# ymartin101/RTS

Hardware: AMD Instinct MI355X
Metric: Mrays/s (primary+bounces) & ms/pulse, 100k-tri scene (higher is better)
Workload: dtype f64

## Files before the change

### include/rts_amd.h

```cpp
#ifndef RTS_AMD_H
#define RTS_AMD_H

#include <stdint.h>
#include "rts_prd.h"

#ifdef __cplusplus
extern "C" {
#endif

typedef struct RtsContext* RtsHandle;

enum {
    RTS_OK = 0,
    RTS_ERR_INVALID = 1,
    RTS_ERR_NO_DEVICE = 2,
    RTS_ERR_HIP = 3,
    RTS_ERR_UNSUPPORTED = 4,
    RTS_ERR_CAPACITY = 5,
    RTS_ERR_IO = 6
};

typedef struct RtsParams {
    uint32_t width;
    uint32_t max_refl;
    uint32_t max_refr;
    uint32_t interpolate_smooth;
    int32_t device;
    uint32_t flags;
} RtsParams;

#define RTS_FLAG_KEEP_ALL_RAYS 1u
#define RTS_FLAG_DEVICE_BUILD 4u
#define RTS_FLAG_HOST_BUILD 16u
#define RTS_FLAG_NO_PREFILTER 8u
#define RTS_FLAG_COUNT_TRAVERSAL 2u

typedef struct RtsMesh {
    const uint32_t* triangles;
    const double* vertices;
    const double* normals;
    uint32_t n_triangles, n_vertices, n_normals;
    uint32_t reserved;
    double refl_coeff;
    double refr_index;
} RtsMesh;

typedef struct RtsTargetMotion {
    double position[3];
    double velocity[3];
    double rotation[9];
    int32_t has_rotation;
    int32_t reserved;
} RtsTargetMotion;

typedef struct RtsReceiverSphere {
    double centre[3];
    double radius;
    double min_theta, max_theta, min_phi, max_phi;
} RtsReceiverSphere;

typedef struct RtsPulse {
    double ray_origin[3];
    double tx_span[3];
    double tx_dir[2];
    uint64_t ray_first;
    uint64_t ray_count;
    const RtsTargetMotion* motion;
    uint32_t interleave_tile, interleave_parts, interleave_part, reserved;
} RtsPulse;
#define RTS_INTERLEAVE_LIST 0xffffffffu

typedef struct RtsStats {
    uint64_t rays;
    uint64_t segments;
    uint64_t shaded;
    uint64_t received;
    uint64_t node_visits;
    uint64_t tri_tests;
    uint32_t n_prims, n_nodes;
    float ms_scene;
    float ms_trace;
    float ms_compact;
    float ms_aggregate;
    uint32_t bvh_rebuilt;
    uint32_t stack_overflows;
    uint64_t walked_segments;
    uint32_t coop_tiles;
    uint32_t cost_records_dropped;
} RtsStats;

typedef struct RtsResponse {
    uint64_t ray;
    int32_t rx;
    uint32_t n;
    double power, delay, doppler, phase;
} RtsResponse;

#define RTS_MAX_DEPTH 16
typedef struct RtsGroup {
    int32_t rx;
    uint32_t direct;
    int32_t path[RTS_MAX_DEPTH];
    uint64_t min_ray;
    double n, sum_sqrt_power, sum_delay, sum_phase, sum_doppler;
} RtsGroup;

int rts_create(const RtsParams* params, RtsHandle* out);
int rts_destroy(RtsHandle h);
const char* rts_last_error(void);
const char* rts_build_id(void);
int rts_bind_host_to_device(int device, int* numa_node);
int rts_device_count(int* n);

int rts_set_scene(RtsHandle h, const RtsMesh* meshes, uint32_t n_targets);
int rts_set_receivers(RtsHandle h, const RtsReceiverSphere* rx, uint32_t n_rx);
int rts_share_scene(RtsHandle dst, RtsHandle src);
typedef struct RtsSceneInfo {
    uint32_t n_targets, n_prims, n_nodes, n_leaves;
    uint32_t handles_sharing;
    uint32_t builder;
    double build_ms;
    uint64_t shared_device_bytes;
    uint64_t handle_device_bytes;
    uint64_t version_bytes;
} RtsSceneInfo;
int rts_scene_info(RtsHandle h, RtsSceneInfo* out);

int rts_trace_pulse(RtsHandle h, const RtsPulse* pulse);

int rts_reserve(RtsHandle h, uint64_t n_rays);
int rts_trace_pulse_begin(RtsHandle h, const RtsPulse* pulse);
int rts_trace_pulse_end(RtsHandle h);
int rts_link_handles(RtsHandle a, RtsHandle b);
int rts_get_stats(RtsHandle h, RtsStats* out);
int rts_get_block_timeline(RtsHandle h, double* out, uint32_t n);

int rts_get_lane_stats(RtsHandle h, uint64_t* out3);
int rts_get_walk_stats(RtsHandle h, uint64_t* out, uint32_t n);
int rts_received_count(RtsHandle h, uint64_t* count);
int rts_get_received(RtsHandle h, struct PerRayData* rays, int32_t* paths, double* rcs_angles, uint64_t* slots,
                     uint64_t capacity);

int rts_received_prefetch(RtsHandle h);
int rts_received_view(RtsHandle h, const struct PerRayData** rays, const int32_t** paths, const double** rcs_angles, const uint64_t** slots,
                      uint64_t* count);
int rts_finalise_values(RtsHandle h, const double* power, const double* doppler, uint64_t count);
int rts_aggregated_view(RtsHandle h, const double** power, const double** doppler, const double** delay, const double** phase,
                        const int32_t** path_match, uint64_t* count);

int rts_get_all_rays(RtsHandle h, struct PerRayData* results, int32_t* targ_intersect, double* rcs_angle,
                     int32_t* hit_prim, float* hit_t, uint64_t capacity);

int rts_finalise_uniform(RtsHandle h, const double* rcs_per_target, double wavelength, double gt, double gr,
                         double carrier, double cspeed);

int rts_trace_pulse_end_uniform(RtsHandle h, const double* rcs_per_target, double wavelength, double gt, double gr,
                                double carrier, double cspeed, int32_t cube_pulse, uint64_t recv_index_base);

#define RTS_PATTERN_CONSTANT 0u
#define RTS_PATTERN_SEPARABLE 1u
#define RTS_PATTERN_GRID 2u
#define RTS_PATTERN_ABS_U 1u
#define RTS_PATTERN_ABS_V 2u
#define RTS_PATTERN_MAX_AXIS 65536u
#define RTS_PATTERN_MAX_GRID 4194304u
typedef struct RtsPattern {
    uint32_t kind;
    uint32_t flags;
    uint32_t n_u, n_v;
    double scale;
    const double* u_samples;
    const double* u_values;
    const double* v_samples;
    const double* v_values;
    double u0, du, v0, dv;
    const double* grid;
    uint64_t reserved[2];
} RtsPattern;
typedef struct RtsPatternPulse {
// ... 429 lines not shown
```

### rts_amd/_lib.py

```python
import ctypes as C
import os
import subprocess

import numpy as np

_HERE = os.path.dirname(os.path.abspath(__file__))
LIB_PATH = os.environ.get("RTS_AMD_LIB", os.path.join(_HERE, "librts_amd.so"))
CSRC = os.path.join(_HERE, "csrc")

RTS_OK, RTS_ERR_INVALID, RTS_ERR_NO_DEVICE, RTS_ERR_HIP, RTS_ERR_UNSUPPORTED, RTS_ERR_CAPACITY, RTS_ERR_IO = range(7)
RTS_FLAG_KEEP_ALL_RAYS = 1
RTS_FLAG_COUNT_TRAVERSAL = 2
RTS_FLAG_DEVICE_BUILD = 4
RTS_FLAG_HOST_BUILD = 16
RTS_FLAG_NO_PREFILTER = 8
RTS_MAX_DEPTH = 16
RTS_BASE_USE_ROWS = 0xffffffffffffffff

PRD_DTYPE = np.dtype({
    "names": ["rayLength", "refrIndex", "reflDepth", "refrDepth", "maxRayIndex", "rayDirection",
              "firstHitPoint", "prevHitPoint", "power", "doppler", "received", "end"],
    "formats": ["<f8", ("<f8", 2), "<u4", "<u4", "<u4", ("<f8", 3), ("<f8", 3), ("<f8", 3), "<f8", "<f8", "<i4", "u1"],
    "offsets": [0, 16, 32, 36, 40, 48, 72, 96, 120, 128, 136, 140],
    "itemsize": 144,
})


class RtsParams(C.Structure):
    _fields_ = [("width", C.c_uint32), ("max_refl", C.c_uint32), ("max_refr", C.c_uint32),
                ("interpolate_smooth", C.c_uint32), ("device", C.c_int32), ("flags", C.c_uint32)]


class RtsMesh(C.Structure):
    _fields_ = [("triangles", C.c_void_p), ("vertices", C.c_void_p), ("normals", C.c_void_p),
                ("n_triangles", C.c_uint32), ("n_vertices", C.c_uint32), ("n_normals", C.c_uint32),
                ("reserved", C.c_uint32), ("refl_coeff", C.c_double), ("refr_index", C.c_double)]


class RtsTargetMotion(C.Structure):
    _fields_ = [("position", C.c_double * 3), ("velocity", C.c_double * 3), ("rotation", C.c_double * 9),
                ("has_rotation", C.c_int32), ("reserved", C.c_int32)]


class RtsReceiverSphere(C.Structure):
    _fields_ = [("centre", C.c_double * 3), ("radius", C.c_double), ("min_theta", C.c_double),
                ("max_theta", C.c_double), ("min_phi", C.c_double), ("max_phi", C.c_double)]


class RtsPulse(C.Structure):
    _fields_ = [("ray_origin", C.c_double * 3), ("tx_span", C.c_double * 3), ("tx_dir", C.c_double * 2),
                ("ray_first", C.c_uint64), ("ray_count", C.c_uint64), ("motion", C.POINTER(RtsTargetMotion)),
                ("interleave_tile", C.c_uint32), ("interleave_parts", C.c_uint32), ("interleave_part", C.c_uint32), ("reserved", C.c_uint32)]


class RtsCubeParams(C.Structure):
    _fields_ = [("n_rx", C.c_uint32), ("n_pulses", C.c_uint32), ("n_bins", C.c_uint32), ("reserved", C.c_uint32),
                ("t0", C.c_double), ("dt", C.c_double)]


class RtsPlanItem(C.Structure):
    _fields_ = [("pulse", C.c_uint32), ("interleave_tile", C.c_uint32), ("interleave_parts", C.c_uint32), ("interleave_part", C.c_uint32),
                ("ray_first", C.c_uint64), ("ray_count", C.c_uint64)]


RTS_SHARD_PULSES, RTS_SHARD_RAYS, RTS_SHARD_PULSES_WHOLE = 0, 1, 2


RTS_PATTERN_CONSTANT, RTS_PATTERN_SEPARABLE, RTS_PATTERN_GRID = 0, 1, 2
# ... 168 lines not shown
class RtsCovParams(C.Structure):
    _fields_ = [("source", C.c_uint32), ("n_rows_in", C.c_uint32), ("first_row", C.c_uint32), ("n_rows", C.c_uint32),
                ("first_bin", C.c_uint32), ("n_bins", C.c_uint32), ("skip_first_bin", C.c_uint32), ("skip_n_bins", C.c_uint32),
                ("device_in", C.c_void_p), ("reserved", C.c_uint64 * 2)]


class RtsMvdrParams(C.Structure):
    _fields_ = [("n_beams", C.c_uint32), ("n_rx", C.c_uint32), ("loading", C.c_double), ("steering", C.c_void_p),
                ("device_cov", C.c_void_p), ("reserved", C.c_uint64 * 2)]


assert C.sizeof(RtsCovParams) == 56 and C.sizeof(RtsMvdrParams) == 48


RTS_ST_MAX_TAPS = 16


class RtsStCovParams(C.Structure):
    _fields_ = [("source", C.c_uint32), ("n_rows_in", C.c_uint32), ("first_row", C.c_uint32), ("n_rows", C.c_uint32),
                ("first_bin", C.c_uint32), ("n_bins", C.c_uint32), ("skip_first_bin", C.c_uint32), ("skip_n_bins", C.c_uint32),
                ("n_taps", C.c_uint32), ("reserved0", C.c_uint32), ("device_in", C.c_void_p), ("reserved", C.c_uint64 * 2)]


class RtsStApplyParams(C.Structure):
    _fields_ = [("n_filters", C.c_uint32), ("source", C.c_uint32), ("first_row", C.c_uint32), ("n_rows", C.c_uint32),
                ("n_rows_in", C.c_uint32), ("flags", C.c_uint32), ("n_taps", C.c_uint32), ("reserved0", C.c_uint32),
                ("weights", C.c_void_p), ("device_in", C.c_void_p), ("reserved", C.c_uint64 * 2)]


assert C.sizeof(RtsStCovParams) == 64 and C.sizeof(RtsStApplyParams) == 64


RTS_EIG_MAX_SWEEPS = 30
RTS_DOA_INVERSE = 1
RTS_DOA_BARTLETT, RTS_DOA_CAPON, RTS_DOA_MUSIC = 0, 1, 2
RTS_DOA_AIC, RTS_DOA_MDL = 0, 1


class RtsEigParams(C.Structure):
    _fields_ = [("n", C.c_uint32), ("reserved0", C.c_uint32), ("device_cov", C.c_void_p), ("reserved", C.c_uint64 * 2)]


class RtsDoaScanParams(C.Structure):
    _fields_ = [("n", C.c_uint32), ("first_vector", C.c_uint32), ("m", C.c_uint32), ("flags", C.c_uint32), ("n_dirs", C.c_uint64),
                ("g", C.c_void_p), ("device_steering", C.c_void_p), ("device_vectors", C.c_void_p), ("reserved", C.c_uint64 * 2)]


assert C.sizeof(RtsEigParams) == 32 and C.sizeof(RtsDoaScanParams) == 64


class RtsSceneInfo(C.Structure):
    _fields_ = [("n_targets", C.c_uint32), ("n_prims", C.c_uint32), ("n_nodes", C.c_uint32), ("n_leaves", C.c_uint32),
                ("handles_sharing", C.c_uint32), ("builder", C.c_uint32), ("build_ms", C.c_double),
                ("shared_device_bytes", C.c_uint64), ("handle_device_bytes", C.c_uint64), ("version_bytes", C.c_uint64)]


class RtsStats(C.Structure):
    _fields_ = [("rays", C.c_uint64), ("segments", C.c_uint64), ("shaded", C.c_uint64), ("received", C.c_uint64),
                ("node_visits", C.c_uint64), ("tri_tests", C.c_uint64), ("n_prims", C.c_uint32), ("n_nodes", C.c_uint32),
                ("ms_scene", C.c_float), ("ms_trace", C.c_float), ("ms_compact", C.c_float), ("ms_aggregate", C.c_float),
                ("bvh_rebuilt", C.c_uint32), ("stack_overflows", C.c_uint32), ("walked_segments", C.c_uint64), ("coop_tiles", C.c_uint32), ("cost_records_dropped", C.c_uint32)]


RESPONSE_DTYPE = np.dtype([("ray", "<u8"), ("rx", "<i4"), ("n", "<u4"), ("power", "<f8"), ("delay", "<f8"),
                           ("doppler", "<f8"), ("phase", "<f8")])
GROUP_DTYPE = np.dtype([("rx", "<i4"), ("direct", "<u4"), ("path", "<i4", (RTS_MAX_DEPTH,)), ("min_ray", "<u8"),
                        ("n", "<f8"), ("sum_sqrt_power", "<f8"), ("sum_delay", "<f8"), ("sum_phase", "<f8"),
                        ("sum_doppler", "<f8")])
assert RESPONSE_DTYPE.itemsize == 48 and GROUP_DTYPE.itemsize == 120


def is_stale():
    if not os.path.exists(LIB_PATH):
        return True
    try:
        return build_id() != source_hash()
    except (OSError, AttributeError):
        return True


def source_hash():
    import hashlib
    names = sorted(f for f in os.listdir(CSRC) if f.endswith((".hip", ".cpp", ".h")) and f != "rts_build_id.h")
    h = hashlib.sha256()
    for path in [os.path.join(CSRC, f) for f in names] + [os.path.join(_HERE, "..", "include", f) for f in ("rts_amd.h", "rts_prd.h")]:
        with open(path, "rb") as f:
            h.update(f.read())
    return h.hexdigest()[:16]


def build_id(path=None):
    L = C.CDLL(path or LIB_PATH)
    L.rts_build_id.restype = C.c_char_p
    return L.rts_build_id().decode()


def require_built():
    if not os.path.exists(LIB_PATH):
        raise SystemExit("librts_amd.so is not built: run `python __graft_entry__.py` (or make -C rts_amd/csrc) first")
    if "RTS_AMD_LIB" not in os.environ:
        have, want = build_id(), source_hash()
        if have != want:
            raise SystemExit("librts_amd.so is stale: built from sources %s, the tree is %s -- run `python __graft_entry__.py` first" % (have, want))


def build(force=False, verbose=False):
    if force or is_stale():
        cmd = ["make", "-C", CSRC, "-j", "5"] + ([] if verbose else ["-s"])
        subprocess.check_call(cmd)
    return LIB_PATH


_lib = None

EXPORTS = ["rts_create", "rts_destroy", "rts_last_error", "rts_device_count", "rts_set_scene", "rts_share_scene", "rts_scene_info", "rts_set_receivers",
           "rts_trace_pulse", "rts_reserve", "rts_trace_pulse_begin", "rts_trace_pulse_end", "rts_link_handles", "rts_get_stats", "rts_get_block_timeline", "rts_received_count", "rts_get_received", "rts_get_all_rays",
           "rts_finalise_uniform", "rts_trace_pulse_end_uniform", "rts_aggregate", "rts_group_count", "rts_get_groups", "rts_get_aggregated",
           "rts_merge_groups", "rts_groups_to_responses", "rts_kernel_wrapper", "rts_vertex_rotation",
           "rts_rotation_matrix", "rts_rect_mesh", "rts_sphere_mesh", "rts_file_mesh", "rts_rx_sphere", "rts_get_bvh",
           "rts_build_id", "rts_bind_host_to_device", "rts_get_lane_stats", "rts_get_walk_stats", "rts_self_test_math", "rts_cube_attach", "rts_cube_accumulate", "rts_cube_get", "rts_cube_accumulate_paths", "rts_cube_doppler", "rts_cube_doppler_get", "rts_plan_cpi", "rts_cube_reduce", "rts_kernel_wrapper_on",
           "rts_received_prefetch", "rts_received_view", "rts_finalise_values", "rts_aggregated_view", "rts_build_hierarchy_host",
           "rts_tile_records_get", "rts_tile_records_set", "rts_deal_tiles", "rts_set_tile_list",
           "rts_set_patterns", "rts_finalise_patterns", "rts_trace_pulse_end_patterns", "rts_pattern_eval",
           "rts_cube_set_waveform", "rts_cube_render", "rts_cube_compress", "rts_waveform_eval",
           "rts_cube_add_noise", "rts_noise_eval", "rts_cube_detect", "rts_cube_detections_get",
           "rts_cube_detect_os", "rts_cfar_os_alpha", "rts_cfar_os_eval",
           "rts_cube_plots", "rts_cube_plots_get", "rts_plots_eval",
           "rts_cube_track", "rts_cube_tracks_get", "rts_cube_tracks_set", "rts_cube_tracks_reset", "rts_cube_track_rounds", "rts_tracks_eval",
           "rts_cube_tbd_step", "rts_cube_tbd_extract", "rts_cube_tbd_tracks_get", "rts_cube_tbd_paths_get", "rts_cube_tbd_merit_get", "rts_cube_tbd_ring_get",
           "rts_cube_tbd_info", "rts_cube_tbd_reset", "rts_tbd_step_eval", "rts_tbd_extract_eval",
           "rts_cube_backproject", "rts_cube_image_get", "rts_backproject_eval",
           "rts_cube_spectrogram", "rts_cube_spectrogram_get", "rts_stft_eval", "rts_window_make",
           "rts_cube_render_beat", "rts_beat_eval", "rts_cube_range_transform", "rts_cube_range_get", "rts_range_eval",
           "rts_cube_beamform", "rts_cube_beam_get", "rts_beamform_eval", "rts_steering_make",
           "rts_cube_covariance", "rts_cube_covariance_get", "rts_covariance_eval", "rts_cube_mvdr", "rts_cube_mvdr_get", "rts_mvdr_eval",
           "rts_cube_st_covariance", "rts_st_covariance_eval", "rts_cube_st_apply", "rts_cube_st_get", "rts_st_apply_eval", "rts_st_steering_make",
           "rts_cube_eig", "rts_cube_eig_get", "rts_eig_eval", "rts_cube_doa_scan", "rts_cube_doa_get", "rts_doa_scan_eval", "rts_doa_weights", "rts_source_count"]


def lib():
    global _lib
    if _lib is not None:
        return _lib
    if not os.path.exists(LIB_PATH):
        raise RuntimeError("librts_amd.so is not built (run `make -C rts_amd/csrc` or __graft_entry__.build()); "
                           "there is no Python/CPU fallback for the RTS hot path")
    L = C.CDLL(LIB_PATH)
    vp, u32, u64, dbl, i32 = C.c_void_p, C.c_uint32, C.c_uint64, C.c_double, C.c_int32
    L.rts_last_error.restype = C.c_char_p
    sig = {
        "rts_create": [C.POINTER(RtsParams), C.POINTER(vp)],
        "rts_destroy": [vp],
        "rts_device_count": [C.POINTER(C.c_int)],
        "rts_set_scene": [vp, C.POINTER(RtsMesh), u32],
        "rts_share_scene": [vp, vp],
        "rts_scene_info": [vp, C.POINTER(RtsSceneInfo)],
        "rts_set_receivers": [vp, C.POINTER(RtsReceiverSphere), u32],
        "rts_trace_pulse": [vp, C.POINTER(RtsPulse)],
        "rts_reserve": [vp, u64],
        "rts_trace_pulse_begin": [vp, C.POINTER(RtsPulse)],
        "rts_get_block_timeline": [vp, vp, u32],
        "rts_trace_pulse_end": [vp],
        "rts_link_handles": [vp, vp],
        "rts_get_stats": [vp, C.POINTER(RtsStats)],
        "rts_received_count": [vp, C.POINTER(u64)],
        "rts_get_received": [vp, vp, vp, vp, vp, u64],
        "rts_get_all_rays": [vp, vp, vp, vp, vp, vp, u64],
        "rts_finalise_uniform": [vp, vp, dbl, dbl, dbl, dbl, dbl],
        "rts_build_hierarchy_host": [vp, vp, u32, dbl, vp, u32, vp, u32, C.POINTER(u32), C.POINTER(u32), C.POINTER(C.c_int32)],
        "rts_received_prefetch": [vp],
        "rts_received_view": [vp, C.POINTER(vp), C.POINTER(vp), C.POINTER(vp), C.POINTER(vp), C.POINTER(u64)],
        "rts_finalise_values": [vp, vp, vp, u64],
        "rts_aggregated_view": [vp, C.POINTER(vp), C.POINTER(vp), C.POINTER(vp), C.POINTER(vp), C.POINTER(vp), C.POINTER(u64)],
        "rts_aggregate": [vp, dbl, dbl, u64],
        "rts_trace_pulse_end_uniform": [vp, vp, dbl, dbl, dbl, dbl, dbl, C.c_int32, u64],
        "rts_group_count": [vp, C.POINTER(u32)],
        "rts_get_groups": [vp, vp, u32],
        "rts_get_aggregated": [vp, vp, vp, vp, vp, u64],
        "rts_merge_groups": [vp, u32, u32, vp, C.POINTER(u32)],
        "rts_groups_to_responses": [vp, u32, vp, u32, C.POINTER(u32)],
        "rts_kernel_wrapper": [vp, vp, C.c_uint, C.c_uint, C.c_uint, C.c_uint, dbl, dbl, vp, vp, vp, vp, vp, vp],
        "rts_kernel_wrapper_on": [vp, vp, vp, C.c_uint, C.c_uint, C.c_uint, C.c_uint, dbl, dbl, vp, vp, vp, vp, vp, vp],
        "rts_vertex_rotation": [vp, u32, C.c_float, C.c_float, C.c_float],
        "rts_rotation_matrix": [C.c_float, C.c_float, C.c_float, vp],
        "rts_rect_mesh": [C.c_float] * 6 + [vp, vp, vp],
        "rts_sphere_mesh": [u32, C.c_float, C.c_float, C.c_float, C.c_float, vp, C.POINTER(u32), vp, C.POINTER(u32), vp],
        "rts_file_mesh": [C.c_char_p, C.c_char_p, C.c_float, C.c_float, C.c_float, vp, vp, vp, C.POINTER(u32)],
        "rts_rx_sphere": [vp, dbl, dbl, dbl, dbl, dbl, C.POINTER(RtsReceiverSphere)],
        "rts_get_bvh": [vp, vp, vp, vp, u32, u32, vp],
        "rts_cube_attach": [vp, C.POINTER(RtsCubeParams), vp],
        "rts_cube_accumulate": [vp, u32, dbl, dbl],
        "rts_cube_get": [vp, vp, u64], "rts_get_lane_stats": [vp, vp], "rts_get_walk_stats": [vp, vp, C.c_uint32], "rts_bind_host_to_device": [C.c_int, C.POINTER(C.c_int)],
        "rts_cube_accumulate_paths": [vp, u32], "rts_cube_doppler": [vp, u32, vp], "rts_cube_doppler_get": [vp, vp, u64],
        "rts_plan_cpi": [u64, u32, u32, u32, u32, u32, u32, vp, u32, C.POINTER(u32)],
        "rts_cube_reduce": [vp, u32, C.c_int],
        "rts_tile_records_get": [vp, vp, u32], "rts_tile_records_set": [vp, vp, u32], "rts_deal_tiles": [vp, u32, u64, u32, u32, vp, vp], "rts_set_tile_list": [vp, u32, vp, u32],
        "rts_self_test_math": [vp, vp, vp, vp, vp, vp, vp, vp, u32],
        "rts_set_patterns": [vp, C.POINTER(RtsPattern), C.POINTER(RtsPattern), u32, C.POINTER(RtsPattern), u32],
        "rts_finalise_patterns": [vp, C.POINTER(RtsPatternPulse)],
        "rts_trace_pulse_end_patterns": [vp, C.POINTER(RtsPatternPulse), C.c_int32, u64],
        "rts_pattern_eval": [C.POINTER(RtsPattern), vp, vp, u32, vp],
        "rts_cube_set_waveform": [vp, C.POINTER(RtsWaveform)],
        "rts_cube_render": [vp, u32, u32, u32, C.c_double, C.c_double],
        "rts_cube_compress": [vp, u32, u32],
        "rts_waveform_eval": [C.POINTER(RtsWaveform), vp, u32, vp],
        "rts_cube_add_noise": [vp, u32, u32, C.c_double, u64],
        "rts_noise_eval": [u64, vp, u32, C.c_double, vp],
        "rts_cube_detect": [vp, C.POINTER(RtsCfarParams), vp, u32],
        "rts_cube_detections_get": [vp, vp, u32, C.POINTER(u32)],
        "rts_cube_detect_os": [vp, C.POINTER(RtsCfarOsParams), vp, u32],
        "rts_cfar_os_alpha": [u32, u32, C.c_double, C.POINTER(C.c_double)],
        "rts_cfar_os_eval": [C.POINTER(RtsCubeParams), vp, u32, C.POINTER(RtsCfarOsParams), vp, u32, C.POINTER(u32)],
        "rts_cube_plots": [vp, C.POINTER(RtsPlotParams)],
        "rts_cube_plots_get": [vp, vp, u32, C.POINTER(u32)],
        "rts_plots_eval": [C.POINTER(RtsCubeParams), vp, u32, u32, C.POINTER(RtsPlotParams), vp, u32, C.POINTER(u32)],
        "rts_cube_track": [vp, C.POINTER(RtsTrackParams), C.c_double],
        "rts_cube_tracks_get": [vp, vp, u32, C.POINTER(u32), C.POINTER(u64)],
        "rts_cube_tracks_set": [vp, vp, u32, u64, C.c_double],
        "rts_cube_tracks_reset": [vp],
        "rts_cube_track_rounds": [vp, C.POINTER(u32)],
        "rts_tracks_eval": [C.POINTER(RtsTrackParams), vp, u32, u64, C.c_double, vp, u32, vp, u32, C.POINTER(u32), C.POINTER(u64)],
        "rts_cube_tbd_step": [vp, C.POINTER(RtsTbdParams), C.c_double, vp, u32],
        "rts_cube_tbd_extract": [vp, C.POINTER(RtsTbdExtractParams)],
        "rts_cube_tbd_tracks_get": [vp, vp, u32, C.POINTER(u32)],
        "rts_cube_tbd_paths_get": [vp, vp, u32],
        "rts_cube_tbd_merit_get": [vp, vp, u64],
        "rts_cube_tbd_ring_get": [vp, vp, vp, u32, C.POINTER(u32)],
        "rts_cube_tbd_info": [vp, C.POINTER(u32 * 4), C.POINTER(u64)],
        "rts_cube_tbd_reset": [vp],
        "rts_tbd_step_eval": [C.POINTER(RtsCubeParams), vp, u32, vp, C.POINTER(RtsTbdParams), C.c_double, vp, vp, vp],
        "rts_tbd_extract_eval": [C.POINTER(RtsCubeParams), u32, C.POINTER(RtsTbdParams), vp, vp, vp, u32, C.POINTER(RtsTbdExtractParams), vp, vp, u32, C.POINTER(u32)],
        "rts_cube_backproject": [vp, C.POINTER(RtsImageParams), vp],
        "rts_cube_image_get": [vp, vp, u64],
        "rts_backproject_eval": [C.POINTER(RtsCubeParams), vp, C.POINTER(RtsImageParams), vp],
        "rts_cube_spectrogram": [vp, C.POINTER(RtsStftParams), vp, C.POINTER(u32)],
        "rts_cube_spectrogram_get": [vp, vp, u64],
        "rts_stft_eval": [C.POINTER(RtsCubeParams), vp, C.POINTER(RtsStftParams), vp, C.POINTER(u32)],
        "rts_window_make": [u32, u32, vp],
        "rts_cube_render_beat": [vp, u32, C.POINTER(RtsBeatParams), C.c_double, C.c_double],
        "rts_beat_eval": [C.POINTER(RtsCubeParams), C.POINTER(RtsBeatParams), vp, u32, u32, vp],
        "rts_cube_range_transform": [vp, C.POINTER(RtsRangeParams), vp],
        "rts_cube_range_get": [vp, vp, u64],
        "rts_range_eval": [C.POINTER(RtsCubeParams), vp, C.POINTER(RtsRangeParams), vp],
        "rts_cube_beamform": [vp, C.POINTER(RtsBeamParams), vp],
        "rts_cube_beam_get": [vp, vp, u64],
# ... 47 lines not shown
```

### rts_amd/api.py

```python
import ctypes as C

import numpy as np

from . import _lib as L
from ._lib import PRD_DTYPE, RESPONSE_DTYPE, GROUP_DTYPE, check, ptr


def rect_mesh(w, h, d, yaw=0.0, pitch=0.0, roll=0.0):
    v = np.zeros((8, 3)); t = np.zeros((12, 3), np.uint32); n = np.zeros((12, 3))
    check(L.lib().rts_rect_mesh(w, h, d, yaw, pitch, roll, ptr(v), ptr(t), ptr(n)))
    return v, t, n


def sphere_mesh(subdivisions, radius, yaw=0.0, pitch=0.0, roll=0.0):
    nv = C.c_uint32(); nt = C.c_uint32()
    check(L.lib().rts_sphere_mesh(subdivisions, radius, yaw, pitch, roll, None, C.byref(nv), None, C.byref(nt), None))
    v = np.zeros((nv.value, 3)); t = np.zeros((nt.value, 3), np.uint32); n = np.zeros((nv.value, 3))
    check(L.lib().rts_sphere_mesh(subdivisions, radius, yaw, pitch, roll, ptr(v), C.byref(nv), ptr(t), C.byref(nt), ptr(n)))
    return v, t, n


def file_mesh(v_file, n_file, yaw=0.0, pitch=0.0, roll=0.0):
    nt = C.c_uint32(0)
    check(L.lib().rts_file_mesh(v_file.encode(), n_file.encode(), yaw, pitch, roll, None, None, None, C.byref(nt)))
# ... 599 lines not shown
    p = _st_cov_params(taps, "cube", first, count, first_bin, n_bins, skip, None, 0)
    D = n_rx * max(int(taps), 0)
    out = np.zeros((D, D), np.complex128)
    check(L.lib().rts_st_covariance_eval(C.byref(q), ptr(inp.view(np.float64)), rows, C.byref(p), ptr(out.view(np.float64))))
    return out


def _st_apply_params(weights, taps, n_rx, source, first, count, power, device_in, n_rows_in):
    w = np.ascontiguousarray(np.asarray(weights, np.complex128))
    if w.ndim != 2 or w.shape[1] != int(taps) * n_rx:
        raise ValueError("st_apply: weights of shape %s for %d taps of %d receivers ([n_filters][taps n_rx])" % (w.shape, taps, n_rx))
    p = L.RtsStApplyParams()
    p.n_filters, p.source, p.n_taps = w.shape[0], _BEAM_SOURCES.get(source, source), int(taps)
    p.first_row, p.n_rows, p.n_rows_in = int(first), int(count or 0), int(n_rows_in)
    p.flags = L.RTS_BEAM_POWER if power else 0
    p.weights = ptr(w.view(np.float64))
    p.device_in = device_in if device_in else None
    return p, w


def st_apply_eval(inp, weights, taps, first=0, count=None, power=False):
    inp = np.ascontiguousarray(np.asarray(inp, np.complex128))
    n_rx, rows, nb = inp.shape
    q = L.RtsCubeParams(n_rx, rows, nb, 0, 0.0, 1.0)
    p, keep = _st_apply_params(weights, taps, n_rx, "cube", first, count, power, None, 0)
    out = _beam_out(p.n_filters, (p.n_rows if p.n_rows else rows - p.first_row) - p.n_taps + 1, nb, power, False)
    check(L.lib().rts_st_apply_eval(C.byref(q), ptr(inp.view(np.float64)), rows, C.byref(p), ptr(out.view(np.float64))))
    return out


def st_steering(spatial, dopplers, taps, tap_taper=None):
    a = np.ascontiguousarray(np.atleast_2d(np.asarray(spatial, np.complex128)))
    f = np.ascontiguousarray(np.asarray(dopplers, np.float64).ravel())
    t = None if tap_taper is None else np.ascontiguousarray(np.asarray(tap_taper, np.float64).ravel())
    if t is not None and len(t) != int(taps):
        raise ValueError("st_steering: a taper of %d values for %d taps" % (len(t), taps))
    out = np.zeros((a.shape[0] * len(f), max(int(taps), 0) * a.shape[1]), np.complex128)
    check(L.lib().rts_st_steering_make(ptr(a.view(np.float64)), a.shape[1], a.shape[0], ptr(f), len(f), int(taps), ptr(t), ptr(out.view(np.float64))))
    return out


def device_count():
    n = C.c_int(0)
    rc = L.lib().rts_device_count(C.byref(n))
    return n.value if rc == 0 else 0


import os as _os
_PY_LAP = {} if _os.environ.get("RTS_PY_LAP") == "1" else None


class Tracer:

    def __init__(self, width, max_refl, max_refr=0, smooth=True, device=0, keep_all=False, count_traversal=False, device_build=None, pre_filter=True):
        p = L.RtsParams(width, max_refl, max_refr, 1 if smooth else 0, device,
                        (L.RTS_FLAG_KEEP_ALL_RAYS if keep_all else 0) | (L.RTS_FLAG_COUNT_TRAVERSAL if count_traversal else 0) |
                        (0 if device_build is None else (L.RTS_FLAG_DEVICE_BUILD if device_build else L.RTS_FLAG_HOST_BUILD)) |
                         (0 if pre_filter else L.RTS_FLAG_NO_PREFILTER))
        self.h = C.c_void_p()
        check(L.lib().rts_create(C.byref(p), C.byref(self.h)))
        self.width = width; self.max_refl = max_refl; self.depth = max_refl + (2 if max_refr else 0)
        self.n_targets = 0; self.keep_all = keep_all; self.device = device
        self._keep = []

    def close(self):
        if self.h:
            L.lib().rts_destroy(self.h); self.h = C.c_void_p()

    def __del__(self):
        try:
            self.close()
        except Exception:
            pass

    def set_scene(self, meshes):
        arr = (L.RtsMesh * max(len(meshes), 1))()
        keep = []
        for i, m in enumerate(meshes):
            t = np.ascontiguousarray(m["tris"], np.uint32); v = np.ascontiguousarray(m["verts"], np.float64)
            n = np.ascontiguousarray(m["normals"], np.float64)
            keep += [t, v, n]
            arr[i] = L.RtsMesh(t.ctypes.data, v.ctypes.data, n.ctypes.data, t.shape[0], v.shape[0], n.shape[0], 0,
                               float(m.get("refl_coeff", 1.0)), float(m.get("refr_index", 1.0)))
        check(L.lib().rts_set_scene(self.h, arr, len(meshes)))
        self.n_targets = len(meshes)

    def share_scene(self, other):
        check(L.lib().rts_share_scene(self.h, other.h))
        self.n_targets = other.n_targets

    def scene_info(self):
        s = L.RtsSceneInfo()
        check(L.lib().rts_scene_info(self.h, C.byref(s)))
        return {k: getattr(s, k) for k, _ in L.RtsSceneInfo._fields_}

    def set_receivers(self, spheres):
        arr = (L.RtsReceiverSphere * max(len(spheres), 1))()
        for i, s in enumerate(spheres):
            arr[i] = L.RtsReceiverSphere((C.c_double * 3)(*s["centre"]), s["radius"], s["minTheta"], s["maxTheta"],
                                         s["minPhi"], s["maxPhi"])
        check(L.lib().rts_set_receivers(self.h, arr, len(spheres)))

    def trace(self, origin, tx_span, tx_dir, motion=None, ray_first=0, ray_count=0, want_stats=True, interleave=None):
        check(L.lib().rts_trace_pulse(self.h, C.byref(self._pulse(origin, tx_span, tx_dir, motion, ray_first, ray_count, interleave))))
        return self.stats() if want_stats else None

    def reserve(self, n_rays=0):
        check(L.lib().rts_reserve(self.h, n_rays))

    def trace_begin(self, origin, tx_span, tx_dir, motion=None, ray_first=0, ray_count=0, interleave=None):
        if _PY_LAP is None:
            check(L.lib().rts_trace_pulse_begin(self.h, C.byref(self._pulse(origin, tx_span, tx_dir, motion, ray_first, ray_count, interleave))))
            return
        import time
        t0 = time.perf_counter(); p = self._pulse(origin, tx_span, tx_dir, motion, ray_first, ray_count, interleave)
        t1 = time.perf_counter(); f = L.lib().rts_trace_pulse_begin
        t2 = time.perf_counter(); rc = f(self.h, C.byref(p))
        t3 = time.perf_counter(); check(rc)
        t4 = time.perf_counter()
        for k, v in zip(("marshal", "lookup", "call", "check"), (t1 - t0, t2 - t1, t3 - t2, t4 - t3)):
            _PY_LAP[k] = _PY_LAP.get(k, 0.0) + v
        _PY_LAP["n"] = _PY_LAP.get("n", 0) + 1

    def block_timeline(self):
        out = np.zeros(9, np.float64)
        check(L.lib().rts_get_block_timeline(self.h, ptr(out), 9))
        return dict(zip(("start_first", "start_p50", "start_last", "end_first", "end_p10", "end_p50", "end_p90", "end_last", "blocks"), out.tolist()))

    def trace_end(self):
        check(L.lib().rts_trace_pulse_end(self.h))

    def tile_records_get(self):
        n = (self.width ** 3 + 63) // 64
        out = np.zeros(n, np.uint32)
        check(L.lib().rts_tile_records_get(self.h, ptr(out), n))
        return out

    def tile_records_set(self, records):
# ... 493 lines not shown
```

### rts_amd/csrc/rts_api.hip

```cpp
#include <cmath>
#include <cstdarg>
#include <cstdio>
#include <cstring>
#include <cstdlib>
#include <dlfcn.h>
#include <algorithm>
#include <chrono>
#include <map>
#include <mutex>
#include <stdexcept>
#include <string>
#include "rts_internal.h"
#include "rts_raygen.h"
#include <atomic>

static thread_local char g_err[1024] = "";
void rts_set_error(const char* fmt, ...) { va_list ap; va_start(ap, fmt); vsnprintf(g_err, sizeof(g_err), fmt, ap); va_end(ap); }
extern "C" const char* rts_last_error(void) { return g_err; }
#include "rts_build_id.h"
extern "C" const char* rts_build_id(void) { return RTS_SOURCE_HASH; }

#include <dirent.h>
#include <sched.h>
extern "C" int rts_bind_host_to_device(int device, int* numa_node)
// ... 240 lines not shown
    for (int i = 0; i < 3; i++) for (int j = 0; j < 3; j++) a.rot1[3*i + j] = Rot1[i][j];
}

static void fill_mask_frame(RtsLaunchConsts& a, bool enable)
{
    RtsMaskFrame& f = a.mask; memset(&f, 0, sizeof(f));
    if (!enable || a.W < 2) return;
    dvec3 c[8]; dvec3 sum = mk3(0, 0, 0);
    for (int k = 0; k < 8; k++) {
        c[k] = rts_lattice_dir(a, (k & 1) ? a.W - 1 : 0, (k & 2) ? a.W - 1 : 0, (k & 4) ? a.W - 1 : 0);
        const double n = len3(c[k]); if (!(n > 0) || !std::isfinite(n)) return;
        c[k] = mk3(c[k].x / n, c[k].y / n, c[k].z / n); sum = add3(sum, c[k]);
    }
    const double sn = len3(sum); if (!(sn > 1e-6)) return;
    const dvec3 b = mk3(sum.x / sn, sum.y / sn, sum.z / sn);
    dvec3 ref = std::fabs(b.z) < 0.9 ? mk3(0, 0, 1) : mk3(1, 0, 0);
    dvec3 u = cross3(ref, b); const double un = len3(u); u = mk3(u.x / un, u.y / un, u.z / un);
    const dvec3 v = cross3(b, u);
    double u0 = 1e300, u1 = -1e300, v0 = 1e300, v1 = -1e300;
    for (int k = 0; k < 8; k++) {
        const double w = dot3(c[k], b); if (!(w > 0.5)) return;
        const double uu = dot3(c[k], u) / w, vv = dot3(c[k], v) / w;
        u0 = std::min(u0, uu); u1 = std::max(u1, uu); v0 = std::min(v0, vv); v1 = std::max(v1, vv);
    }
    const double du = std::max(u1 - u0, 1e-9), dv = std::max(v1 - v0, 1e-9);
    u0 -= 0.002 * du; u1 += 0.002 * du; v0 -= 0.002 * dv; v1 += 0.002 * dv;
    f.bx = (float)b.x; f.by = (float)b.y; f.bz = (float)b.z; f.ux = (float)u.x; f.uy = (float)u.y; f.uz = (float)u.z; f.vx = (float)v.x; f.vy = (float)v.y; f.vz = (float)v.z;
    const double n_fit = std::floor(std::min(u1 - u0, v1 - v0) / RTS_MASK_MIN_CELL);
    if (!(n_fit >= 32.0)) return;
    const uint32_t n = (uint32_t)std::min<double>(RTS_MASK_N, n_fit) & ~31u;
    f.u0 = (float)u0; f.v0 = (float)v0; f.inv_du = (float)(n / (u1 - u0)); f.inv_dv = (float)(n / (v1 - v0));
    f.n = n;
}

static int fill_target_placement(const RtsContext* c, uint32_t t, RtsTargetDev& td)
{
    const RtsTargetMotion& m = c->motion[t]; const RtsBlasInfo& b = c->scene->blas[t];
    double R[9] = {1, 0, 0, 0, 1, 0, 0, 0, 1};
    if (m.has_rotation) for (int k = 0; k < 9; k++) R[k] = m.rotation[k];
    for (int k = 0; k < 9; k++) if (!std::isfinite(R[k])) { rts_set_error("rts_trace_pulse: target %u has a non-finite rotation", t); return RTS_ERR_INVALID; }
    double dev = 0;
    for (int i = 0; i < 3; i++) for (int j = 0; j < 3; j++) {
        double g = 0; for (int k = 0; k < 3; k++) g += R[3*k + i] * R[3*k + j];
        dev = std::max(dev, std::fabs(g - (i == j ? 1.0 : 0.0)));
    }
    if (!(dev < 1e-3)) { rts_set_error("rts_trace_pulse: target %u: rotation is not orthonormal (|R^T R - I| = %.3g); only rigid placements are supported", t, dev); return RTS_ERR_UNSUPPORTED; }
    const double det = R[0]*(R[4]*R[8] - R[5]*R[7]) - R[1]*(R[3]*R[8] - R[5]*R[6]) + R[2]*(R[3]*R[7] - R[4]*R[6]);
    const double id = 1.0 / det;
    td.rinv[0] = (R[4]*R[8] - R[5]*R[7]) * id; td.rinv[1] = (R[2]*R[7] - R[1]*R[8]) * id; td.rinv[2] = (R[1]*R[5] - R[2]*R[4]) * id;
    td.rinv[3] = (R[5]*R[6] - R[3]*R[8]) * id; td.rinv[4] = (R[0]*R[8] - R[2]*R[6]) * id; td.rinv[5] = (R[2]*R[3] - R[0]*R[5]) * id;
    td.rinv[6] = (R[3]*R[7] - R[4]*R[6]) * id; td.rinv[7] = (R[1]*R[6] - R[0]*R[7]) * id; td.rinv[8] = (R[0]*R[4] - R[1]*R[3]) * id;
    td.px = m.position[0]; td.py = m.position[1]; td.pz = m.position[2];
    td.root = b.root;
    double cl[3], half2 = 0, wc[3], wmax = 0;
    for (int i = 0; i < 3; i++) { cl[i] = 0.5 * b.lo[i] + 0.5 * b.hi[i]; const double h = 0.5 * (b.hi[i] - b.lo[i]); half2 += h * h; }
    for (int i = 0; i < 3; i++) { wc[i] = R[3*i]*cl[0] + R[3*i + 1]*cl[1] + R[3*i + 2]*cl[2] + m.position[i]; wmax = std::max(wmax, std::fabs(wc[i])); }
    double rad = std::sqrt(half2) * (1.0 + 2.0 * dev); wmax += rad;
    rad = rad * (1.0 + 1e-6) + wmax * 1e-6 + 1e-30;
    td.cx = wc[0]; td.cy = wc[1]; td.cz = wc[2]; td.r2 = rad * rad;
    td.ew = (float)(wmax * c->tune.ew_rel) + 1.0e-30f;
    if (b.root < 0 || !std::isfinite(td.cx + td.cy + td.cz + td.r2)) td.root = -1;
    return RTS_OK;
}

static int rts_hist_ensure(RtsContext* c, uint32_t n_hist)
{
    if (c->hist->n == n_hist) return RTS_OK;
    std::lock_guard<std::mutex> lk(g_hist_mu);
    RTS_HIP(hipDeviceSynchronize()); RTS_HIP(c->hist->d.reserve(n_hist)); RTS_HIP(hipMemset(c->hist->d.p, 0, sizeof(uint32_t) * n_hist));
    c->hist->n = n_hist; c->hist->any = false; c->tile_cost_pending = false;
    return RTS_OK;
}

static int rts_zero_block_reserve(RtsContext* c)
{
    RTS_HIP(c->d_tile_ctr.reserve(RTS_ZERO_WORDS + RTS_MASK_WORDS + 64));
    c->p_counters = reinterpret_cast<unsigned long long*>(c->d_tile_ctr.p + RTS_OFF_COUNTERS);
    return RTS_OK;
}

static int rts_launch_buffers_reserve(RtsContext* c, const RtsLaunchSizes& s)
{
    RTS_HIP(c->d_recv.reserve(s.recv)); RTS_HIP(c->d_dir_hist.reserve(s.dir_hist)); RTS_HIP(c->d_child.reserve(s.child));
    RTS_HIP(c->d_stack_ovf.reserve(s.stack_ovf)); RTS_HIP(c->d_block_counters.reserve(s.block_counters));
    RTS_HIP(c->d_all.reserve(s.all)); RTS_HIP(c->d_hit_prim.reserve(s.hit_prim)); RTS_HIP(c->d_hit_t.reserve(s.hit_t));
    return RTS_OK;
}

static uint32_t rts_coop_threads(const RtsContext* c) { return c->tune.coop_frac > 0.0 ? c->tune.coop_grid_max * RTS_BLOCK : 0u; }

extern "C" int rts_reserve(RtsHandle c, uint64_t n_rays)
{
    CHECK_HANDLE(c);
    const uint64_t W3 = rts_lattice_size(c->params.width);
    const uint64_t n = std::min<uint64_t>(n_rays ? n_rays : W3, W3);
    if (n * rts_chains(c->params.max_refr) > 0xfffffff0ULL) { rts_set_error("rts_reserve: rays x chains exceeds 2^32"); return RTS_ERR_UNSUPPORTED; }
    const RtsLaunchSizes sz = rts_launch_sizes(n, (uint64_t)c->n_cu * 64 * RTS_BLOCK, (uint64_t)c->n_cu * 1024, rts_coop_threads(c), (uint64_t)c->n_cu * 64 + c->tune.coop_grid_max,
                                               c->params.max_refl, c->params.max_refr, (c->params.flags & RTS_FLAG_KEEP_ALL_RAYS) != 0);
    { int rc = rts_launch_buffers_reserve(c, sz); if (rc != RTS_OK) return rc; }
    { int rc = rts_zero_block_reserve(c); if (rc != RTS_OK) return rc; }
    const size_t n_tiles = (size_t)rts_wave_tiles(n);
    RTS_HIP(c->d_tile_cost.reserve(n_tiles)); RTS_HIP(c->d_tile_key.reserve(n_tiles)); RTS_HIP(c->d_tile_order.reserve(n_tiles));
    { int rc = rts_hist_ensure(c, (uint32_t)rts_wave_tiles(W3)); if (rc != RTS_OK) return rc; }
    RTS_HIP(hipMemsetAsync(c->d_recv.p, 0, sizeof(RtsEndRecord) * sz.recv, c->stream));
    RTS_HIP(hipMemsetAsync(c->d_dir_hist.p, 0, sizeof(float) * c->d_dir_hist.cap, c->stream));
    RTS_HIP(hipStreamSynchronize(c->stream));
// ... 76 lines not shown
    lc.ray_first = r.first; lc.W = W; lc.il_tile = r.il_tile; lc.il_parts = r.il_parts; lc.il_part = r.il_part; lc.il_list = r.il_list ? c->d_il_list.p : nullptr;
    const RtsDivMagic d = rts_div_magic(W); lc.w_magic = d.magic; lc.w_more = d.more;
    fill_mask_frame(lc, pre_filter && c->scene->n_prims > 0);
    for (int k = 0; k < 3; k++) { lc.f_bs[k] = (float)(&lc.bsx)[k]; lc.f_st[k] = (float)(&lc.stx)[k]; }
    for (int i = 0; i < 3; i++) for (int j = 0; j < 3; j++) lc.f_m[3 * i + j] = (float)(lc.rot1[3 * i] * lc.rot[j] + lc.rot1[3 * i + 1] * lc.rot[3 + j] + lc.rot1[3 * i + 2] * lc.rot[6 + j]);
}

static uint32_t* pulse_mask_words(const RtsContext* c) { return c->d_tile_ctr.p + RTS_ZERO_WORDS; }

static int pulse_upload_and_fill(RtsContext* c, bool moved)
{
    const uint32_t n_targets = (uint32_t)c->scene->meshes.size(); const RtsMaskFrame& mask = c->last_lc.mask;
    c->pin.p->lc = c->last_lc;
    RTS_HIP(hipMemcpyAsync(c->d_params.p, &c->pin.p->lc, moved && n_targets ? offsetof(RtsPinned, td) + sizeof(RtsTargetDev) * n_targets : sizeof(RtsLaunchConsts), hipMemcpyHostToDevice, c->stream));
    { int rc = rts_zero_block_reserve(c); if (rc != RTS_OK) return rc; }
    RTS_HIP(hipMemsetAsync(c->d_tile_ctr.p, 0, sizeof(uint32_t) * (((RTS_ZERO_WORDS + (mask.n ? (size_t)mask.n * mask.n / 32u + 1u : 0u)) + 63u) & ~(size_t)63u), c->stream));
    return RTS_OK;
}

static int pulse_scene_place(RtsContext* c, bool moved)
{
    { int rc = rts_scene_place(c, c->last_lc, moved, pulse_mask_words(c)); if (rc != RTS_OK) return rc; }
    if (moved) { RTS_STAGE(c, "scene_place"); c->bvh_valid = true; c->stats.bvh_rebuilt = 1; }
    RTS_HIP(hipEventRecord(c->ev[1], c->stream));
    return RTS_OK;
}

static int pulse_args_and_buffers(RtsContext* c, RtsPulseLaunch& L)
{
    RtsTraceArgs& a = L.a; memset(&a, 0, sizeof(a));
    const uint32_t n = L.n; const RtsLaunchConsts& lc = c->last_lc; hipStream_t st = c->stream;
    a.lc = c->p_lc;
    a.ray_first = L.r.first; a.n_rays = n; a.W = c->params.width; a.max_refl = c->params.max_refl; a.smooth = c->params.interpolate_smooth ? 1u : 0u;
    a.n_prims = c->scene->n_prims; a.n_targets = (uint32_t)c->scene->meshes.size(); a.n_rx = c->n_rx; a.keep_all = L.keep_all ? 1u : 0u;
    a.max_refr = c->params.max_refr; a.rows = a.max_refr ? c->params.max_refl + 3 : 1;
    if ((uint64_t)n * rts_chains(a.max_refr) > 0xfffffff0ULL) { rts_set_error("rts_trace_pulse: rays x chains exceeds 2^32"); return RTS_ERR_UNSUPPORTED; }
    a.total_threads = L.grid * RTS_BLOCK;
    a.coop_spread = c->tune.coop_spread;
    a.coop_walk_steps_lo = std::min(c->tune.coop_walk_steps_lo, c->tune.coop_walk_steps);
    a.coop_walk_steps = c->tune.coop_walk_steps; a.coop_min_cost = c->tune.coop_walk_steps ? std::min<uint32_t>(c->tune.coop_floor, 1875u) : 0u;
    a.slab_threads = a.total_threads + rts_coop_threads(c);
    const RtsLaunchSizes sz = rts_launch_sizes(n, a.total_threads, a.total_threads, rts_coop_threads(c), (uint64_t)L.grid + c->tune.coop_grid_max, a.max_refl, a.max_refr, L.keep_all);
    { int rc = rts_launch_buffers_reserve(c, sz); if (rc != RTS_OK) return rc; }
    if (L.keep_all) {
        rts_fill_i32(st, c->d_hit_prim.p, -2, sz.hit_prim - 1);
        RTS_HIP(hipMemsetAsync(c->d_hit_t.p, 0, sizeof(float) * (sz.hit_t - 1), st));
    }
    a.pmask = lc.mask.n ? pulse_mask_words(c) : nullptr; a.pre_filter = L.pre_filter ? 1u : 0u;
    a.nodes4 = c->scene->d_nodes4.p; a.nodes4v = c->tune.node_versions ? c->scene->d_nodes4v.p : nullptr; a.stack_lds = c->tune.stack_lds; a.leaves = c->d_leaves.p; a.tri_nidx = c->scene->d_tri_nidx.p; a.normals = c->d_normals_world.p;
    a.targets = c->p_targets; a.rx = c->d_rx.p;
    a.recv_records = c->d_recv.p; a.all_records = c->d_all.p; a.counters = c->p_counters; a.block_counters = c->d_block_counters.p; a.dir_hist = c->d_dir_hist.p;
    a.hit_prim = c->d_hit_prim.p; a.hit_t = c->d_hit_t.p; a.stack_ovf = c->d_stack_ovf.p; a.child = c->d_child.p;
    a.rx_window_screen = c->tune.rx_window_screen ? 1u : 0u;
    a.coop_versions = c->tune.coop_versions ? 1u : 0u;
    a.tile_ctr = c->d_tile_ctr.p;
    return RTS_OK;
}

static int pulse_tile_order(RtsContext* c, RtsPulseLaunch& L)
{
    RtsTraceArgs& a = L.a;
    const RtsLaunchShape s = rts_launch_shape(L.n, L.r.first, L.r.il_tile, L.r.il_parts, L.r.il_part, rts_lattice_size(c->params.width));
    const uint32_t n_tiles = s.n_tiles, resident_waves = L.grid * (RTS_BLOCK / RTS_WTILE);
    a.batch_dead = s.aligned ? (uint32_t)c->tune.batch_dead : 0u;
    if (!(c->tune.tile_lpt && s.aligned && n_tiles > resident_waves)) { c->tile_cost_pending = false; c->tile_last_valid = false; return RTS_OK; }
    { int rc = rts_hist_ensure(c, s.n_hist); if (rc != RTS_OK) return rc; }
    if (c->tile_cost_pending || c->hist->any) {
        c->coop_big_now = (L.r.il_parts > 1 && !L.shared_gpu && c->tune.coop_big_part > c->tune.coop_big) ? c->tune.coop_big_part : c->tune.coop_big;
        int rc = rts_tile_order_build(c, c->tile_cost_sig, c->tile_cost_pending, s.sig, n_tiles, resident_waves); if (rc != RTS_OK) return rc;
        a.tile_order = c->d_tile_order.p; a.tile_head = c->tune.coop_frac > 0.0 ? c->d_tile_ctr.p + RTS_OFF_HEAD + 2 : nullptr; a.tile_head_all = a.tile_head; c->hist->any = true;
        a.tile_live = c->d_tile_ctr.p + RTS_OFF_LIVE;
    }
    const bool merged_all = c->tile_cost_pending && rts_wave_tiles(c->tile_cost_sig[0]) >= n_tiles && c->d_tile_cost.cap >= n_tiles;
    RTS_HIP(c->d_tile_cost.reserve(n_tiles));
    if (!merged_all) RTS_HIP(hipMemsetAsync(c->d_tile_cost.p, 0, sizeof(uint32_t) * n_tiles, c->stream));
    a.tile_cost = c->d_tile_cost.p;
    c->tile_cost_pending = true; memcpy(c->tile_cost_sig, s.sig, sizeof(s.sig)); memcpy(c->tile_last_sig, s.sig, sizeof(s.sig)); c->tile_last_valid = true;
    return RTS_OK;
}

static int pulse_timelines(RtsContext* c, RtsPulseLaunch& L)
{
    const size_t blocks2 = (size_t)L.grid * 2;
    RtsLaunchTuning lt; if (L.count_trav) rts_tuning_read(&lt, rts_env);
    L.tl_path = lt.timeline;
    L.cnt_tl = blocks2 + 2 * (size_t)rts_wave_tiles(L.n);
    c->tl_blocks = 0;
    const size_t words = L.tl_path ? L.cnt_tl + 1 : (!L.count_trav && c->tune.timeline_blocks) ? blocks2 + 1 : 0;
    if (!words) return RTS_OK;
    RTS_HIP(c->d_timeline.reserve(words)); RTS_HIP(hipMemsetAsync(c->d_timeline.p, 0, sizeof(unsigned long long) * words, c->stream)); L.a.timeline = c->d_timeline.p;
    if (!L.tl_path) c->tl_blocks = L.grid;
    return RTS_OK;
}

static int pulse_launch(RtsContext* c, RtsPulseLaunch& L)
{
    RtsTraceArgs& a = L.a; hipStream_t st = c->stream;
    RTS_STAGE(c, "pre-trace");
    c->tstream_now = (c->tune.trace_own_stream && !L.shared_gpu && c->gate->refs.load() == 1) ? st : c->tstream;
    if (c->tstream_now != st) {
        RTS_HIP(hipEventRecord(c->ev[8], st));
        RTS_HIP(hipStreamWaitEvent(c->tstream_now, c->ev[8], 0));
    }
    RTS_HIP(hipEventRecord(c->ev[2], c->tstream_now));
    unsigned coop_grid = 0;
    if (a.tile_head) {
// ... 811 lines not shown
```

### rts_amd/csrc/rts_bvh.hip

```cpp
#include <cstring>
#include <hip/hip_runtime.h>
#include "rts_internal.h"
#include "rts_ray_ops.h"

__device__ __forceinline__ void place_one(const double* __restrict__ local, double* __restrict__ world, const uint32_t* __restrict__ targ_of,
                                          const RtsTargetMotion* __restrict__ motion, uint32_t i, bool add_position)
{
    const RtsTargetMotion m = motion[targ_of[i]];
    double x = local[3*i], y = local[3*i+1], z = local[3*i+2];
    if (m.has_rotation) {
        double rx = 0.0, ry = 0.0, rz = 0.0;
        rx += m.rotation[0] * x; rx += m.rotation[1] * y; rx += m.rotation[2] * z;
        ry += m.rotation[3] * x; ry += m.rotation[4] * y; ry += m.rotation[5] * z;
        rz += m.rotation[6] * x; rz += m.rotation[7] * y; rz += m.rotation[8] * z;
        x = rx; y = ry; z = rz;
    }
    if (add_position) { x += m.position[0]; y += m.position[1]; z += m.position[2]; }
    world[3*i] = x; world[3*i+1] = y; world[3*i+2] = z;
}
__global__ void k_place(const double* __restrict__ v_local, double* __restrict__ v_world, const uint32_t* __restrict__ v_targ, uint32_t n_verts,
                        const double* __restrict__ n_local, double* __restrict__ n_world, const uint32_t* __restrict__ n_targ, uint32_t n_normals,
                        const RtsTargetMotion* __restrict__ motion)
{
    const uint32_t i = blockIdx.x * blockDim.x + threadIdx.x;
// ... 34 lines not shown
    }
    const bool any = iu1 >= iu0 && iv1 >= iv0;
    {
        int b0 = any ? iu0 : 0x7fffffff, b1 = any ? iv0 : 0x7fffffff, b2 = any ? iu1 : -1, b3 = any ? iv1 : -1;
        for (int d = warpSize / 2; d > 0; d >>= 1) {
            b0 = min(b0, __shfl_xor(b0, d)); b1 = min(b1, __shfl_xor(b1, d)); b2 = max(b2, __shfl_xor(b2, d)); b3 = max(b3, __shfl_xor(b3, d));
        }
        if ((threadIdx.x & (warpSize - 1)) == 0 && b2 >= 0) { atomicMin(&S.box[0], b0); atomicMin(&S.box[1], b1); atomicMax(&S.box[2], b2); atomicMax(&S.box[3], b3); }
    }
    __syncthreads();
    if (S.box[2] < 0) return;
    const int W0 = S.box[0] >> 5, V0 = S.box[1], TW = (S.box[2] >> 5) - W0 + 1, TH = S.box[3] - V0 + 1;
    const int band = RTS_MASK_TILE_WORDS / TW;
    for (int b0 = 0; b0 < TH; b0 += band) {
        const int B0 = V0 + b0, bh = min(band, TH - b0), nw = TW * bh;
        if (b0) __syncthreads();
        for (int w = threadIdx.x; w < nw; w += blockDim.x) S.tile[w] = 0u;
        __syncthreads();
        if (any) {
            for (int iv = max(iv0, B0); iv <= min(iv1, B0 + bh - 1); iv++) {
                for (int w0 = iu0 >> 5; w0 <= (iu1 >> 5); w0++) {
                    const int lo = max(iu0, w0 << 5) & 31, hi = min(iu1, (w0 << 5) + 31) & 31;
                    const uint32_t bits = (hi == 31 ? 0xffffffffu : ((1u << (hi + 1)) - 1u)) & ~((1u << lo) - 1u);
                    atomicOr(&S.tile[(iv - B0) * TW + (w0 - W0)], bits);
                }
            }
        }
        __syncthreads();
        for (int w = threadIdx.x; w < nw; w += blockDim.x) {
            const uint32_t bits = S.tile[w];
            if (bits) atomicOr(&mask[((size_t)(B0 + w / TW) * f.n >> 5) + (size_t)(W0 + w % TW)], bits);
        }
    }
}

__device__ __forceinline__ void place_vertex(const double* __restrict__ local, const RtsTargetMotion& m, uint32_t i, double* __restrict__ out3)
{
    double x = local[3*(size_t)i], y = local[3*(size_t)i+1], z = local[3*(size_t)i+2];
    if (m.has_rotation) {
        double rx = 0.0, ry = 0.0, rz = 0.0;
        rx += m.rotation[0] * x; rx += m.rotation[1] * y; rx += m.rotation[2] * z;
        ry += m.rotation[3] * x; ry += m.rotation[4] * y; ry += m.rotation[5] * z;
        rz += m.rotation[6] * x; rz += m.rotation[7] * y; rz += m.rotation[8] * z;
        x = rx; y = ry; z = rz;
    }
    x += m.position[0]; y += m.position[1]; z += m.position[2];
    out3[0] = x; out3[1] = y; out3[2] = z;
}
template <bool LEAVES, bool MASK, bool PLACE = false>
__global__ void __launch_bounds__(256) k_leaves(const uint32_t* __restrict__ order, const uint32_t* __restrict__ tri_vidx, const double* __restrict__ verts,
                                                const uint32_t* __restrict__ prim_targ, RtsLeafTri* __restrict__ leaves, uint32_t n,
                                                double ox, double oy, double oz, RtsMaskFrame f, uint32_t* __restrict__ mask,
                                                const RtsTargetMotion* __restrict__ motion = nullptr, uint32_t prim_blocks = 0, const double* __restrict__ n_local = nullptr,
                                                double* __restrict__ n_world = nullptr, const uint32_t* __restrict__ n_targ = nullptr, uint32_t n_normals = 0)
{
    __shared__ __attribute__((aligned(16))) uint32_t s_raw[MASK ? sizeof(RtsMaskLds) / 4 : 1];
    if (PLACE && blockIdx.x >= prim_blocks) {
        const uint32_t q = (blockIdx.x - prim_blocks) * blockDim.x + threadIdx.x;
        if (q < n_normals) place_one(n_local, n_world, n_targ, motion, q, false);
        return;
    }
    const uint32_t i = blockIdx.x * blockDim.x + threadIdx.x;
    double p[9] = {0, 0, 0, 0, 0, 0, 0, 0, 0};
    if (i < n) {
        const uint32_t g = order[i];
        const uint32_t a = tri_vidx[3*(size_t)g], b = tri_vidx[3*(size_t)g+1], c = tri_vidx[3*(size_t)g+2];
        if (PLACE) {
            const RtsTargetMotion m = motion[prim_targ[g]];
            place_vertex(verts, m, a, p); place_vertex(verts, m, b, p + 3); place_vertex(verts, m, c, p + 6);
        } else {
        p[0] = verts[3*(size_t)a]; p[1] = verts[3*(size_t)a+1]; p[2] = verts[3*(size_t)a+2];
        p[3] = verts[3*(size_t)b]; p[4] = verts[3*(size_t)b+1]; p[5] = verts[3*(size_t)b+2];
        p[6] = verts[3*(size_t)c]; p[7] = verts[3*(size_t)c+1]; p[8] = verts[3*(size_t)c+2];
        }
        if (LEAVES) {
            dvec3 e0, e1, nn;
            tri_terms(mk3(p[0], p[1], p[2]), mk3(p[3], p[4], p[5]), mk3(p[6], p[7], p[8]), e0, e1, nn);
            RtsLeafTri L;
            L.p0x = p[0]; L.p0y = p[1]; L.p0z = p[2]; L.e0x = e0.x; L.e0y = e0.y; L.e0z = e0.z; L.e1x = e1.x; L.e1y = e1.y; L.e1z = e1.z;
            L.nx = nn.x; L.ny = nn.y; L.nz = nn.z;
            L.prim = g; L.targ = prim_targ[g]; L.pad[0] = 0u; L.pad[1] = 0u;
            leaves[g] = L;
        }
    }
    if (MASK) rts_mask_mark(*reinterpret_cast<RtsMaskLds*>(s_raw), i < n, p, ox, oy, oz, f, mask);
}

static inline unsigned blocks_for(size_t n, unsigned bs) { return (unsigned)((n + bs - 1) / bs); }

int rts_scene_place(RtsContext* c, const RtsLaunchConsts& lc, bool place, uint32_t* pmask)
{
    hipStream_t st = c->stream;
    const RtsMaskFrame& f = lc.mask;
    const bool mask = f.n != 0;
    const RtsScene* sc = c->scene;
    if (place && sc->n_prims) {
        const unsigned gp = blocks_for(sc->n_prims, 256), gn = blocks_for(sc->n_normals, 256);
        if (mask) k_leaves<true, true, true><<<gp + gn, 256, 0, st>>>(sc->d_prim_order.p, sc->d_tri_vidx.p, sc->d_verts_local.p, sc->d_prim_targ.p, c->d_leaves.p, sc->n_prims, lc.ox, lc.oy, lc.oz, f, pmask,
                                                                     c->p_motion, gp, sc->d_normals_local.p, c->d_normals_world.p, sc->d_norm_targ.p, sc->n_normals);
        else k_leaves<true, false, true><<<gp + gn, 256, 0, st>>>(sc->d_prim_order.p, sc->d_tri_vidx.p, sc->d_verts_local.p, sc->d_prim_targ.p, c->d_leaves.p, sc->n_prims, lc.ox, lc.oy, lc.oz, f, nullptr,
                                                                  c->p_motion, gp, sc->d_normals_local.p, c->d_normals_world.p, sc->d_norm_targ.p, sc->n_normals);
        c->verts_world_valid = false;
        RTS_HIP(hipGetLastError());
        return RTS_OK;
    }
    if (place) {
        if (sc->n_verts + sc->n_normals) k_place<<<blocks_for((size_t)sc->n_verts + sc->n_normals, 256), 256, 0, st>>>(sc->d_verts_local.p, c->d_verts_world.p, sc->d_vert_targ.p, sc->n_verts,
                                                                                                                         sc->d_normals_local.p, c->d_normals_world.p, sc->d_norm_targ.p, sc->n_normals, c->p_motion);
        c->verts_world_valid = true;
    } else if (mask) {
        if (!c->verts_world_valid && sc->n_verts) {
            k_place<<<blocks_for((size_t)sc->n_verts, 256), 256, 0, st>>>(sc->d_verts_local.p, c->d_verts_world.p, sc->d_vert_targ.p, sc->n_verts, sc->d_normals_local.p, c->d_normals_world.p, sc->d_norm_targ.p, 0u, c->p_motion);
            c->verts_world_valid = true;
        }
        if (sc->n_prims) k_leaves<false, true><<<blocks_for(sc->n_prims, 256), 256, 0, st>>>(sc->d_prim_order.p, sc->d_tri_vidx.p, c->d_verts_world.p, sc->d_prim_targ.p, nullptr, sc->n_prims, lc.ox, lc.oy, lc.oz, f, pmask);
    }
    RTS_HIP(hipGetLastError());
    return RTS_OK;
}
```

### rts_amd/csrc/rts_internal.h

```cpp
#pragma once
#include <hip/hip_runtime.h>
#include <stdint.h>
#include <stddef.h>
#include <atomic>
#include <string>
#include <vector>
#include "../../include/rts_amd.h"
#include "rts_device_math.h"
#include "rts_pattern.h"
#include "rts_waveform.h"
#include "rts_noise.h"
#include "rts_image.h"
#include "rts_cube_source.h"
#include "rts_stft.h"
#include "rts_beat.h"
#include "rts_beam.h"
#include "rts_adapt.h"
#include "rts_stap.h"
#include "rts_doa.h"
#include "rts_cfar_os.h"
#include "rts_track.h"
#include "rts_tbd.h"
#include "rts_plot.h"
#include "rts_owned.h"
#include "rts_launch_plan.h"
#include "rts_post_plan.h"
#include "rts_pulse_state.h"
#include "rts_scene_host.h"
#include "rts_tuning.h"
static_assert(RtsTuning().img_split_below == RTS_IMAGE_SPLIT_BELOW, "the default of RTS_IMAGE_SPLIT_BELOW is rts_image.h's");


struct __attribute__((aligned(16))) RtsLeafTri {
    double p0x, p0y, p0z, e0x, e0y, e0z, e1x, e1y, e1z, nx, ny, nz;
    uint32_t prim;
    uint32_t targ;
    uint32_t pad[2];
};
static_assert(sizeof(RtsLeafTri) == 112, "leaf size");
static_assert(offsetof(RtsLeafTri, p0x) == 0 && offsetof(RtsLeafTri, p0z) == 16 && offsetof(RtsLeafTri, e0y) == 32 && offsetof(RtsLeafTri, e1x) == 48 &&
              offsetof(RtsLeafTri, e1z) == 64 && offsetof(RtsLeafTri, ny) == 80 && offsetof(RtsLeafTri, prim) == 96 && offsetof(RtsLeafTri, targ) == 100,
              "leaf record offsets of the walk step's decode");

struct RtsTargetDev {
    double reflCoeff;
    double refrIndex;
    double vx, vy, vz;
    uint32_t tri_base;
    uint32_t perface_normals;
    double rinv[9];
    double px, py, pz;
    double cx, cy, cz, r2;
    float ew;
    int32_t root;
};

struct RtsRxDev { double cx, cy, cz, radius, minTheta, maxTheta, minPhi, maxPhi; };

struct __attribute__((aligned(16))) RtsEndRecord {
    double rayLength, power, doppler;
    double prevx, prevy, prevz;
    double firstx, firsty, firstz;
    uint64_t path_lo, path_hi;
    uint32_t slot;
    int32_t received;
    uint32_t reflDepth;
    uint32_t pad;
};
static_assert(sizeof(RtsEndRecord) == 112, "end record size");
static_assert(sizeof(RtsDetection) == 72 && sizeof(RtsCfarParams) == 72 && sizeof(RtsCfarOsParams) == 72, "CFAR ABI sizes (rts_amd/_lib.py mirrors them)");
static_assert(sizeof(RtsPlot) == 104 && sizeof(RtsPlotParams) == 56, "plot ABI sizes (rts_amd/_lib.py mirrors them)");
static_assert(sizeof(RtsTrack) == 88 && sizeof(RtsTrackParams) == 96, "track ABI sizes (rts_amd/_lib.py mirrors them)");
static_assert(sizeof(RtsTbdParams) == 72 && sizeof(RtsTbdExtractParams) == 40 && sizeof(RtsTbdTrack) == 48, "track-before-detect ABI sizes (rts_amd/_lib.py mirrors them)");
struct RtsTrackMeta { uint64_t next_id; uint32_t n, total, rounds, reserved; };

struct __attribute__((aligned(16))) RtsChildState {
    double prevx, prevy, prevz, firstx, firsty, firstz;
    double rayLength, power, doppler, refx, refy;
    float dx, dy, dz;
    uint32_t refrDepth, refr_code, end, pad0, pad1;
};
static_assert(sizeof(RtsChildState) == 128, "child state size");

#ifndef RTS_TILE_CTRS
#define RTS_TILE_CTRS 64
#endif
#define RTS_TILE_BUCKETS 1024
#define RTS_TILE_CTR_STRIDE 32
#define RTS_XCD 8
#define RTS_SEG_STRIPES 8
#define RTS_TILE_CTRS_LAYOUT ((RTS_XCD + 1) * RTS_SEG_STRIPES + 8)
#define RTS_OFF_CTR_COOP (RTS_TILE_CTRS_LAYOUT * RTS_TILE_CTR_STRIDE)
#define RTS_OFF_HEAD (2 * RTS_TILE_CTRS_LAYOUT * RTS_TILE_CTR_STRIDE)
#define RTS_OFF_LIVE (RTS_OFF_HEAD + 4)
#define RTS_OFF_COUNTERS (RTS_OFF_HEAD + 8)
#define RTS_OFF_BINS (RTS_OFF_COUNTERS + 32)
#define RTS_OFF_TAKEN (RTS_OFF_BINS + RTS_TILE_BUCKETS)
#define RTS_ZERO_WORDS (RTS_OFF_TAKEN + RTS_TILE_BUCKETS)
#ifndef RTS_RX_LDS
#define RTS_RX_LDS 16
#endif

#define RTS_MASK_MIN_CELL 1.0e-5
#define RTS_MASK_N 1024u
#define RTS_MASK_WORDS (RTS_MASK_N * RTS_MASK_N / 32u + 1u)
#define RTS_MASK_MAX_CELLS 4096
struct RtsMaskFrame { float bx, by, bz, ux, uy, uz, vx, vy, vz; float u0, v0, inv_du, inv_dv; uint32_t n, pad0, pad1; };

struct RtsLaunchConsts {
    double ox, oy, oz;
    double bsx, bsy, bsz;
    double stx, sty, stz;
    double rot[9];
    double rot1[9];
    double w1x, w1y, w1z;
    uint64_t ray_first;
    uint32_t W, pad;
    uint32_t w_magic, w_more;
    uint32_t il_tile, il_parts, il_part, pad2;
    const uint32_t* il_list;
    RtsMaskFrame mask;
    float f_bs[3], f_st[3], f_m[9], f_pad;
};
static_assert(sizeof(RtsLaunchConsts) % 8 == 0, "launch constants are copied to LDS dword by dword");

struct RtsTraceArgs {
    const RtsLaunchConsts* lc;
    uint64_t ray_first;
    uint32_t n_rays, W;
    uint32_t max_refl, smooth;
    uint32_t n_prims, n_targets, n_rx, keep_all;
    uint32_t max_refr, rows;
    RtsChildState* child;
    const RtsNode4* nodes4;
    const RtsNode4* nodes4v;
    const RtsLeafTri* leaves;
    const uint32_t* tri_nidx;
    const double* normals;
    const RtsTargetDev* targets;
    const RtsRxDev* rx;
    RtsEndRecord* recv_records;
    RtsEndRecord* all_records;
    unsigned long long* counters;
    unsigned long long* block_counters;
    float* dir_hist;
    int32_t* hit_prim;
    float* hit_t;
    int32_t* stack_ovf;
    uint32_t total_threads;
    uint32_t slab_threads;
    const uint32_t* tile_order;
    uint32_t* tile_cost;
    uint32_t* tile_ctr;
    uint32_t coop_spread;
    const uint32_t* tile_head;
    const uint32_t* tile_head_all;
    const uint32_t* tile_live;
    uint32_t rx_window_screen;
    uint32_t coop_versions;
    uint32_t batch_dead;
    uint32_t coop_walk_steps_lo;
    uint32_t coop_min_cost, coop_walk_steps;
    unsigned long long* timeline;
    uint32_t pre_filter;
    const uint32_t* pmask;
    uint32_t stack_lds;
};

#define RTS_PIN_GROUPS 4096
static inline uint32_t rts_agg_spec(uint32_t R) { return R < RTS_PIN_GROUPS ? R : RTS_PIN_GROUPS; }
struct RtsPinned {
    RtsLaunchConsts lc;
    RtsTargetMotion motion[256];
    RtsTargetDev td[256];
    unsigned long long cnt[16];
    uint32_t G, pad;
    double rcs[256];
    double gsum[5 * RTS_PIN_GROUPS]; uint64_t gkey[RTS_PIN_GROUPS]; uint64_t grow[RTS_PIN_GROUPS]; uint32_t gmin[RTS_PIN_GROUPS];
};

struct RtsGate { hipStream_t tstream = nullptr; std::atomic<int> refs{0}; int device = 0; };

struct RtsScene {
    std::atomic<int> refs{1}; int device = 0;
    std::vector<RtsMeshHost> meshes;
    uint32_t n_prims = 0, n_verts = 0, n_normals = 0;
    DevBuf<uint32_t> d_tri_vidx, d_tri_nidx, d_vert_targ, d_norm_targ, d_prim_targ;
    DevBuf<double> d_verts_local, d_normals_local;
    std::vector<RtsBlasInfo> blas; uint32_t n_nodes = 0, n_leaves = 0;
    DevBuf<RtsNode4> d_nodes4; DevBuf<uint32_t> d_leaf_prim;
    DevBuf<uint32_t> d_prim_order;
    DevBuf<RtsNode4> d_nodes4v;
    double build_ms = 0; uint32_t builder = 0;
    size_t device_bytes() const {
        return d_tri_vidx.cap * 4 + d_tri_nidx.cap * 4 + d_vert_targ.cap * 4 + d_norm_targ.cap * 4 + d_prim_targ.cap * 4 + d_verts_local.cap * 8 +
               d_normals_local.cap * 8 + (d_nodes4.cap + d_nodes4v.cap) * sizeof(RtsNode4) + d_leaf_prim.cap * 4 + d_prim_order.cap * 4;
    }
};

struct RtsTileHist { std::atomic<int> refs{1}; DevBuf<uint32_t> d; uint32_t n = 0; bool any = false; uint32_t head_hint = 0; bool head_hint_valid = false; };

struct RtsSpecParams { std::vector<double> rcs; double wl = 0, gt = 0, gr = 0, carrier = 0, cspeed = 0; int32_t cube_pulse = -1; uint64_t base = 0;
                       int mode = 0;
                       int fin = 0;
                       std::vector<double> pat_rx; double pat_org[3] = {0, 0, 0}, pat_dir[2] = {0, 0};
};
struct RtsPatArgs { const RtsPatView* pats; const double* rx; uint32_t n_rx, n_targets; double ox, oy, oz, tx_az, tx_el, wl, carrier, cspeed; };
struct RtsHostMirror {
    PinBuf<char> buf; uint32_t cap = 0, D = 0;
    size_t o_rays = 0, o_paths = 0, o_angles = 0, o_slots = 0, o_apower = 0, o_adoppler = 0, o_adelay = 0, o_aphase = 0, o_apm = 0, o_vpower = 0, o_vdoppler = 0;
    bool recv_valid = false, agg_valid = false;
    bool want = false;
};
struct RtsAggPending { bool valid = false, rows = false; uint32_t R = 0, D = 0, spec = 0; RtsKeyPlan key = {}; uint64_t base = 0; double* gsum = nullptr; };

struct RtsCubeProduct {
    DevBuf<double> own; double* p = nullptr; size_t doubles = 0; bool valid = false;
    hipError_t place(void* device_out, size_t n, double** out)
    {
        *out = (double*)device_out; if (*out) return hipSuccess;
        if (n > own.cap) { p = nullptr; doubles = 0; valid = false; }
        const hipError_t e = own.reserve(n); *out = own.p; return e;
    }
    void record(double* out, size_t n) { p = out; doubles = n; valid = true; }
};

struct RtsCubeState {
    RtsCubeParams params = {}; double* p = nullptr; DevBuf<double> own; bool set = false;
    DevBuf<double> d_wave; uint32_t wave_M = 0, wave_L = 0; bool wave_set = false;
    RtsCubeProduct doppler; uint32_t doppler_n = 0;
    DevBuf<uint32_t> d_det_cnt, d_det_off; DevBuf<uint8_t> d_det_tmp; DevBuf<RtsDetection> d_det; uint32_t det_nseg = 0, det_max = 0; bool det_valid = false;
    uint32_t det_nd = 0;
    DevBuf<uint64_t> d_plot_key; DevBuf<uint32_t> d_plot_parent, d_plot_idx, d_plot_lab_s, d_plot_idx_s, d_plot_len, d_plot_flag, d_plot_off; DevBuf<uint8_t> d_plot_tmp;
    DevBuf<RtsPlot> d_plot; uint32_t plot_cap = 0, plot_max = 0; bool plot_valid = false, plot_own_list = false;
    DevBuf<RtsTrack> d_trk[2]; DevBuf<RtsTrackMeta> d_trk_meta; DevBuf<RtsTrackPred> d_trk_pred;
    DevBuf<double> d_trk_zd, d_trk_zf, d_trk_pw, d_trk_cd, d_trk_md2; DevBuf<uint64_t> d_trk_best_d;
    DevBuf<uint32_t> d_trk_zrx, d_trk_cj, d_trk_cn, d_trk_of_track, d_trk_of_plot, d_trk_best_t, d_trk_rounds, d_trk_flag, d_trk_off; DevBuf<uint8_t> d_trk_tmp;
    uint32_t trk_cur = 0, trk_max = 0, trk_loaded = 0; bool trk_live = false; double trk_time = 0.0;
    DevBuf<double> d_tbd_merit[2]; DevBuf<uint8_t> d_tbd_ptr, d_tbd_tmp; DevBuf<int32_t> d_tbd_shift;
    DevBuf<uint32_t> d_tbd_cnt, d_tbd_off, d_tbd_paths; DevBuf<RtsTbdTrack> d_tbd_out;
    uint32_t tbd_rx = 0, tbd_nd = 0, tbd_nb = 0, tbd_depth = 0, tbd_hd = 0, tbd_hr = 0, tbd_cur = 0; uint64_t tbd_frames = 0;
    double tbd_time = 0.0, tbd_t0 = 0.0, tbd_dt = 0.0;
    uint32_t tbd_ext_nseg = 0, tbd_ext_max = 0, tbd_ext_depth = 0; bool tbd_ext_valid = false;
    StagedUpload<double> os_alpha; std::vector<double> os_tab; uint32_t os_tab_key[5] = {0, 0, 0, 0, 0}; double os_tab_pfa = 0.0; bool os_tab_sent = false;
    RtsCubeProduct image; uint32_t img_nx = 0, img_ny = 0;
    StagedUpload<double> img_geo; DevBuf<double> d_img_scratch;
    RtsCubeProduct stft;
    StagedUpload<double> stft_win; DevBuf<double> d_stft_part;
    DevBuf<double> d_beat_part;
// ... 51 lines not shown
    DevBuf<uint32_t> d_tile_cost, d_tile_key, d_tile_order, d_tile_ctr;
    RtsTileHist* hist = nullptr;
    double coop_big_now = 0.0;
    bool tile_cost_pending = false; uint64_t tile_cost_sig[4] = {0, 0, 0, 0};
    DevBuf<uint32_t> d_il_list; uint32_t il_list_n = 0, il_list_tile = 0, il_list_gen = 0; uint32_t il_list_last = 0;
    uint64_t tile_last_sig[4] = {0, 0, 0, 0}; bool tile_last_valid = false; DevBuf<uint32_t> d_rec_tmp;
    DevBuf<float> d_dir_hist; DevBuf<uint32_t> d_pmask; bool pre_dense = false;
    DevBuf<int32_t> d_hit_prim; DevBuf<float> d_hit_t; DevBuf<int32_t> d_stack_ovf; DevBuf<RtsChildState> d_child;
    DevBuf<uint64_t> d_rk64, d_rk64_sorted;
    RtsTraceArgs last_args; RtsLaunchConsts last_lc;
    DevBuf<uint32_t> d_rk, d_rk_sorted, d_ri, d_ri_sorted;
    DevBuf<PerRayData> d_rx_rays; DevBuf<int32_t> d_rx_paths; DevBuf<double> d_rx_angles; DevBuf<uint64_t> d_rx_slots;
    DevBuf<PerRayData> d_all_rays; DevBuf<int32_t> d_all_paths; DevBuf<double> d_all_angles;
    DevBuf<uint64_t> d_akeys, d_akeys_sorted; DevBuf<uint32_t> d_aidx, d_aidx_sorted; DevBuf<uint32_t> d_ghead, d_gid;
    DevBuf<double> d_gsum; DevBuf<uint32_t> d_gmin; DevBuf<uint64_t> d_gkey; DevBuf<uint32_t> d_gcount; DevBuf<uint64_t> d_grow; DevBuf<int32_t> d_gpath;
    DevBuf<double> d_delay, d_phase; DevBuf<int32_t> d_pathmatch; DevBuf<double> d_rcs;
    double tl_summary[9] = {0, 0, 0, 0, 0, 0, 0, 0, 0};
    uint32_t tl_blocks = 0;
    bool order_sum_valid = false; DevBuf<unsigned long long> d_order_sum;
    bool verts_world_valid = false;
    hipStream_t tstream_now = nullptr;
    uint32_t spec_cap = RTS_SMALL_CAP64;
    RtsSpecParams spec;
    uint64_t recv_hint = 0; bool recv_hint_valid = false;
    RtsPulseResults res;
    PinBuf<RtsRxDev> pin_rx; std::vector<RtsRxDev> rx_host;
    RtsCubeState cube;
    PinBuf<RtsPinned> pin;
    bool rcs_uploaded = false; DevBuf<double> d_rcsval; int n_cu = 0; bool stats_pending = false;
    RtsStats stats;
    DevBuf<char> d_pat; uint32_t pat_n_rx = 0, pat_n_targets = 0; bool pat_set = false;
    StagedUpload<double> pat_rx;
    double pulse_org[3] = {0, 0, 0}, pulse_dir[2] = {0, 0}; bool pulse_traced = false;
    double lap_s[8] = {0, 0, 0, 0, 0, 0, 0, 0}; uint64_t lap_n[8] = {0, 0, 0, 0, 0, 0, 0, 0};
    RtsGate* gate = nullptr;
    RtsPulseState pulse;
    ~RtsContext();
};
static inline RtsKeyPlan rts_key_plan_for(uint32_t D, uint32_t n_targets, uint32_t n_rx) { return rts_key_plan(D, (int64_t)n_targets - 1, (int64_t)(n_rx ? n_rx : 1u) - 1); }
static inline RtsKeyPlan rts_handle_key_plan(const RtsContext* c) { return rts_key_plan_for(c->depth, (uint32_t)c->scene->meshes.size(), c->n_rx); }
static inline RtsCubeSource rts_cube_source(const RtsContext* c, bool paths, double cspeed, double carrier, int64_t base)
{
    RtsCubeSource s;
    s.rays = c->d_rx_rays.p; s.delay = c->d_delay.p; s.phase = c->d_phase.p; s.pm = c->d_pathmatch.p; s.base = base;
    s.R = (uint32_t)c->res.n_recv; s.paths = paths ? 1 : 0; s.cspeed = cspeed; s.carrier = carrier;
    return s;
}
void rts_scene_unref(RtsScene* s);
void rts_hist_unref(RtsTileHist* h);
void rts_gate_unref(RtsGate* g);

int rts_sah_build(const double* verts, const uint32_t* tris, uint32_t n_tris, double split_budget, std::vector<RtsNode4>& nodes, std::vector<uint32_t>& leaf_prim, RtsBlasInfo& out);
int rts_lbvh_build_device(RtsContext* c, RtsScene* ns, const RtsSceneFlat& flat, const RtsSceneTuning& tune);
int rts_scene_place(RtsContext* c, const RtsLaunchConsts& lc, bool place, uint32_t* pmask);
int rts_tile_costs_flush(RtsContext* c);
int rts_tile_records_masked(RtsContext* c, uint32_t* d_out, uint32_t n);
int rts_tile_order_build(RtsContext* c, const uint64_t* prev_sig, bool prev_valid, const uint64_t* cur_sig, uint32_t n_tiles_cur, uint32_t resident_waves);
int rts_trace_launch(RtsContext* c, const RtsTraceArgs& a, bool count_traversal, unsigned coop_grid);
void rts_trace_preload();
int rts_post_order_and_expand(RtsContext* c);
int rts_mirror_reserve(RtsContext* c, uint32_t rows);
int rts_post_mirror_received(RtsContext* c);
int rts_post_mirror_aggregated(RtsContext* c);
int rts_post_set_values(RtsContext* c, const double* power, const double* doppler);
int rts_post_expand_all(RtsContext* c);
int rts_post_all_small(RtsContext* c, uint32_t cap, const RtsSpecParams& sp, bool want_groups);
int rts_cube_accumulate_device(RtsContext* c, uint32_t pulse_index, double cspeed, double carrier);
int rts_cube_accumulate_paths_device(RtsContext* c, uint32_t pulse_index, int64_t base);
int rts_cube_render_device(RtsContext* c, uint32_t pulse_index, bool paths, bool doppler, double cspeed, double carrier, int64_t base);
int rts_cube_compress_device(RtsContext* c, uint32_t first_pulse, uint32_t n_pulses);
int rts_cube_noise_device(RtsContext* c, uint32_t first_pulse, uint32_t n_pulses, double sigma, uint64_t seed);
int rts_cube_detect_device(RtsContext* c, const RtsCfarParams& p, const double* map, uint32_t n_doppler, uint32_t max_det);
int rts_cube_detect_os_device(RtsContext* c, const RtsCfarOsParams& p, const double* alpha_tab, const double* map, uint32_t n_doppler, uint32_t max_det);
int rts_cube_plots_device(RtsContext* c, const RtsPlotParams& p, const RtsDetection* list, const uint32_t* n_dev, uint32_t n_cap, uint32_t n_doppler, uint32_t max_plots);
int rts_cube_track_tables(RtsContext* c);
int rts_cube_track_device(RtsContext* c, const RtsTrackParams& p, double T, const RtsPlot* list, const uint32_t* n_dev, uint32_t pcap, uint32_t tcap);
int rts_cube_tbd_step_device(RtsContext* c, const RtsTbdParams& p, const double* map, bool first, double T, double dt, uint32_t slot);
int rts_cube_tbd_extract_device(RtsContext* c, const RtsTbdExtractParams& e, uint32_t max_tracks);
int rts_cube_doppler_device(RtsContext* c, uint32_t n_fft, double* out);
int rts_cube_stft_device(RtsContext* c, const RtsStftParams& p, const RtsStftPlan& plan, const double* window, double* out);
int rts_cube_beat_device(RtsContext* c, uint32_t pulse_index, const RtsBeatParams& p, const RtsBeatPlan& plan, double cspeed, double carrier, int64_t base);
int rts_cube_range_device(RtsContext* c, const RtsRangeParams& p, const RtsRangePlan& plan, const double* window, double* out);
int rts_cube_beam_device(RtsContext* c, const RtsBeamParams& p, const RtsBeamPlan& plan, const double* in, uint64_t rx_stride, const double* weights, void* out);
int rts_cube_cov_device(RtsContext* c, const RtsCovSet& set, const RtsCovPlan& plan, uint32_t n_taps, const double* in, uint64_t rx_stride, double* part, double* out);
int rts_cube_mvdr_device(RtsContext* c, const RtsMvdrPlan& plan, uint32_t n_rx, uint32_t n_beams, double loading, const double* cov, const double* steering, uint32_t* status, double* out);
int rts_cube_st_apply_device(RtsContext* c, const RtsStApplyParams& p, const RtsStApplyPlan& plan, const double* in, uint64_t rx_stride, const double* weights, void* out);
int rts_cube_eig_device(RtsContext* c, const RtsEigPlan& plan, uint32_t n, const double* cov, uint32_t* status, double* values, double* vectors);
int rts_cube_doa_scan_device(RtsContext* c, const RtsDoaScanPlan& plan, uint32_t n, uint32_t m, uint64_t n_dirs, uint32_t flags, const double* steering, const double* vectors,
                             const double* g, double* out);
int rts_cube_backproject_device(RtsContext* c, const RtsImageParams& p, const RtsImagePlan& plan, const double* geo, double* out);
int rts_post_finalise(RtsContext* c, const double* rcs_host, double wl, double gt, double gr, double carrier, double cspeed);
int rts_pattern_pulse_upload(RtsContext* c, const RtsSpecParams& q, RtsPatArgs* out);
int rts_post_finalise_patterns(RtsContext* c, const RtsSpecParams& q);
hipError_t rts_stream_wait(RtsContext* c, hipStream_t st);
int rts_aggregate_fetch(RtsContext* c, std::vector<RtsGroup>* groups);
int rts_aggregate_device(RtsContext* c, int32_t max_path, int32_t max_rx, const int32_t* d_paths, uint64_t R, uint32_t D,
                         double cspeed, double carrier, uint64_t base, PerRayData* d_rays, double* d_delay,
                         double* d_phase, int32_t* d_pm, std::vector<RtsGroup>* groups, double* d_npath,
                         double* d_power_sum, double* d_doppler_sum, int32_t pm_init, const uint64_t* d_rows);
const char* rts_env(const char* name);
int check_key_width(uint32_t depth, uint32_t n_targets, uint32_t n_rx, const char* who);
int rts_attach_scene(RtsContext* c);
int rts_debug_stage(RtsContext* c, const char* name);
#define RTS_STAGE(c, name) do { int rc_ = rts_debug_stage((c), (name)); if (rc_ != RTS_OK) return rc_; } while (0)

#define RTS_HIP(call) do { hipError_t e_ = (call); if (e_ != hipSuccess) { \
// ... 15 lines not shown
```

### rts_amd/csrc/rts_results_api.hip

```cpp
#include <cstring>
#include "rts_internal.h"

template <class T> static hipError_t rts_copy_home(T* dst, const T* src, size_t n) { return dst && n ? hipMemcpy(dst, src, sizeof(T) * n, hipMemcpyDeviceToHost) : hipSuccess; }

template <class T> static hipError_t rts_view_fill(RtsPulseResults& r, unsigned bit, std::vector<T>& v, const T* src, size_t n, const T** out)
{
    if (!(r.v_recv_have & bit)) { v.resize(n); const hipError_t e = hipMemcpy(v.data(), src, sizeof(T) * n, hipMemcpyDeviceToHost); if (e != hipSuccess) return e; r.v_recv_have |= bit; }
    if (out) *out = v.data();
    return hipSuccess;
}

extern "C" int rts_get_stats(RtsHandle c, RtsStats* out)
{
    if (!c || !out) { rts_set_error("rts_get_stats: null argument"); return RTS_ERR_INVALID; }
    CHECK_CLOSED(c);
    if (c->stats_pending) {
        RTS_HIP(hipSetDevice(c->device));
        RTS_HIP(hipStreamSynchronize(c->stream));
        RtsStats& s = c->stats; float ms = 0;
        RTS_HIP(hipEventElapsedTime(&s.ms_scene, c->ev[0], c->ev[1]));
        RTS_HIP(hipEventElapsedTime(&s.ms_trace, c->ev[2], c->ev[3]));
        RTS_HIP(hipEventElapsedTime(&s.ms_compact, c->ev[4], c->ev[5]));
        s.ms_aggregate = 0;
        if (c->res.fin_timed || c->res.agg_timed) { RTS_HIP(hipEventElapsedTime(&ms, c->ev[6], c->ev[7])); s.ms_aggregate = ms; }
        c->stats_pending = false;
    }
    *out = c->stats; return RTS_OK;
}

extern "C" int rts_get_block_timeline(RtsHandle c, double* out, uint32_t n)
{
    if (!c || !out) { rts_set_error("rts_get_block_timeline: null argument"); return RTS_ERR_INVALID; }
    CHECK_CLOSED(c);
    if (!c->tune.timeline_blocks || c->tl_summary[8] == 0.0) { rts_set_error("rts_get_block_timeline: the handle records no block timeline (create it with RTS_TIMELINE_BLOCKS=1, product build) or has not traced yet"); return RTS_ERR_INVALID; }
    for (uint32_t k = 0; k < n && k < 9; k++) out[k] = c->tl_summary[k];
    return RTS_OK;
}

static int rts_walk_counters(RtsContext* c, const char* who, uint64_t* out, uint32_t n)
{
    if (!c || !out) { rts_set_error("%s: null argument", who); return RTS_ERR_INVALID; }
    CHECK_CLOSED(c);
    const int src[5] = {8, 9, 10, 11, 15};
    for (uint32_t k = 0; k < n && k < 5u; k++) out[k] = c->pin.p->cnt[src[k]];
    return RTS_OK;
}
extern "C" int rts_get_lane_stats(RtsHandle c, uint64_t* out3) { return rts_walk_counters(c, "rts_get_lane_stats", out3, 3); }
extern "C" int rts_get_walk_stats(RtsHandle c, uint64_t* out, uint32_t n) { return rts_walk_counters(c, "rts_get_walk_stats", out, n); }

extern "C" int rts_received_count(RtsHandle c, uint64_t* count)
{
    if (!c || !count) { rts_set_error("rts_received_count: null argument"); return RTS_ERR_INVALID; }
    CHECK_CLOSED(c);
    *count = c->res.n_recv; return RTS_OK;
}

extern "C" int rts_get_received(RtsHandle c, PerRayData* rays, int32_t* paths, double* rcs_angles, uint64_t* slots, uint64_t capacity)
{
    CHECK_HANDLE(c);
    CHECK_CLOSED(c);
    const uint64_t R = c->res.n_recv; const uint32_t D = c->depth;
    if (capacity < R) { rts_set_error("rts_get_received: capacity %llu < %llu received rays", (unsigned long long)capacity, (unsigned long long)R); return RTS_ERR_CAPACITY; }
    if (R == 0) return RTS_OK;
    RTS_HIP(hipStreamSynchronize(c->stream));
    RTS_HIP(rts_copy_home(rays, c->d_rx_rays.p, R)); RTS_HIP(rts_copy_home(paths, c->d_rx_paths.p, R * D));
    RTS_HIP(rts_copy_home(rcs_angles, c->d_rx_angles.p, 2 * R * D)); RTS_HIP(rts_copy_home(slots, c->d_rx_slots.p, R));
    return RTS_OK;
}

extern "C" int rts_get_all_rays(RtsHandle c, PerRayData* results, int32_t* targ_intersect, double* rcs_angle, int32_t* hit_prim, float* hit_t, uint64_t capacity)
{
    CHECK_HANDLE(c);
    CHECK_CLOSED(c);
    if (!(c->params.flags & RTS_FLAG_KEEP_ALL_RAYS)) { rts_set_error("rts_get_all_rays: handle was not created with RTS_FLAG_KEEP_ALL_RAYS"); return RTS_ERR_INVALID; }
    const uint64_t n1 = c->n_rays, n = n1 * c->last_args.rows; const uint32_t D = c->depth, H = rts_hit_rows(c->params.max_refl);
    if (capacity < n) { rts_set_error("rts_get_all_rays: capacity too small (%llu rows)", (unsigned long long)n); return RTS_ERR_CAPACITY; }
    if (n == 0) return RTS_OK;
    RTS_HIP(hipStreamSynchronize(c->stream));
    RTS_HIP(rts_copy_home(results, c->d_all_rays.p, n)); RTS_HIP(rts_copy_home(targ_intersect, c->d_all_paths.p, n * D)); RTS_HIP(rts_copy_home(rcs_angle, c->d_all_angles.p, 2 * n * D));
    RTS_HIP(rts_copy_home(hit_prim, c->d_hit_prim.p, n1 * H)); RTS_HIP(rts_copy_home(hit_t, c->d_hit_t.p, n1 * H));
    return RTS_OK;
}

extern "C" int rts_received_view(RtsHandle c, const PerRayData** rays, const int32_t** paths, const double** rcs_angles, const uint64_t** slots, uint64_t* count)
{
    CHECK_HANDLE(c);
    if (!count) { rts_set_error("rts_received_view: null count"); return RTS_ERR_INVALID; }
    CHECK_CLOSED(c);
    RtsPulseResults& r = c->res; const uint64_t R = r.n_recv; const uint32_t D = c->depth;
    *count = R;
    if (rays) *rays = nullptr; if (paths) *paths = nullptr; if (rcs_angles) *rcs_angles = nullptr; if (slots) *slots = nullptr;
    if (R == 0) return RTS_OK;
    RTS_HIP(rts_stream_wait(c, c->stream));
    const RtsHostMirror& m = r.mirror;
    if (m.recv_valid && R <= m.cap) {
        if (rays) *rays = (const PerRayData*)(m.buf.p + m.o_rays); if (paths) *paths = (const int32_t*)(m.buf.p + m.o_paths);
        if (rcs_angles) *rcs_angles = (const double*)(m.buf.p + m.o_angles); if (slots) *slots = (const uint64_t*)(m.buf.p + m.o_slots);
// ... 94 lines not shown
```

### rts_amd/csrc/rts_scene.hip

```cpp
#include <cstdio>
#include <cstring>
#include <algorithm>
#include <chrono>
#include <memory>
#include <thread>
#include "rts_internal.h"
#include "rts_prim_order.h"

__global__ void k_children_to_prims(RtsNode4* __restrict__ nodes, uint32_t n, const uint32_t* __restrict__ leaf_prim)
{
    const uint32_t i = blockIdx.x * blockDim.x + threadIdx.x;
    if (i >= n) return;
    for (int k = 0; k < 4; k++) { const int32_t ch = nodes[i].child[k]; nodes[i].pad[k] = ch; if (ch < 0) nodes[i].child[k] = ~(int32_t)leaf_prim[~ch]; }
}

__global__ void k_node_versions(const RtsNode4* __restrict__ nodes, uint32_t n, RtsNode4* __restrict__ out, int key_mode)
{
    const uint32_t g = blockIdx.x * blockDim.x + threadIdx.x;
    if (g >= n * 8u) return;
    const uint32_t i = g >> 3, o = g & 7u;
    const RtsNode4 nd = nodes[i];
    const bool mx = (o & 1u) != 0u, my = (o & 2u) != 0u, mz = (o & 4u) != 0u;
    float key[4]; int ord[4];
    for (int k = 0; k < 4; k++) {
// ... 88 lines not shown
    const bool want = st.node_versions;
    const int key_mode = st.version_key_centre ? 1 : 0;
    size_t free_b = 0, total_b = 0; (void)hipMemGetInfo(&free_b, &total_b);
    const size_t need = (size_t)ns->n_nodes * 8 * sizeof(RtsNode4);
    if (want && ns->n_nodes && ns->n_nodes < (1u << 28) && need < free_b / 4) {
        if (ns->d_nodes4v.reserve((size_t)ns->n_nodes * 8) == hipSuccess) {
            k_node_versions<<<(ns->n_nodes * 8u + 255u) / 256u, 256, 0, c->stream>>>(ns->d_nodes4.p, ns->n_nodes, ns->d_nodes4v.p, key_mode);
            RTS_HIP(hipGetLastError()); RTS_HIP(hipStreamSynchronize(c->stream));
        } else (void)hipGetLastError();
    }
    return RTS_OK;
}

int rts_attach_scene(RtsContext* c)
{
    const RtsScene* sc = c->scene; const uint32_t n_targets = (uint32_t)sc->meshes.size();
    RTS_HIP(c->d_leaves.reserve((size_t)sc->n_prims + 1));
    RTS_HIP(c->d_verts_world.reserve(3*(size_t)sc->n_verts + 1)); RTS_HIP(c->d_normals_world.reserve(3*(size_t)sc->n_normals + 1));
    {
        const size_t span = offsetof(RtsPinned, cnt);
        RTS_HIP(c->d_params.reserve(span));
        c->p_lc = reinterpret_cast<RtsLaunchConsts*>(c->d_params.p + offsetof(RtsPinned, lc));
        c->p_motion = reinterpret_cast<RtsTargetMotion*>(c->d_params.p + offsetof(RtsPinned, motion));
        c->p_targets = reinterpret_cast<RtsTargetDev*>(c->d_params.p + offsetof(RtsPinned, td));
        c->rcs_uploaded = false;
    }
    c->verts_world_valid = false; c->order_sum_valid = false;
    if (c->hist->refs.load() > 1) { rts_hist_unref(c->hist); c->hist = new RtsTileHist(); }
    c->motion.assign(n_targets, RtsTargetMotion{}); c->motion_valid = false; c->bvh_valid = false; c->hist->n = 0; c->hist->any = false; c->hist->head_hint_valid = false; c->tile_cost_pending = false; c->tile_last_valid = false;
    return RTS_OK;
}

static int scene_swap(RtsContext* c, RtsScene* ns)
{
    rts_scene_unref(c->scene);
    c->scene = ns;
    return rts_attach_scene(c);
}

extern "C" int rts_set_scene(RtsHandle c, const RtsMesh* meshes, uint32_t n_targets)
{
    CHECK_HANDLE(c);
    CHECK_CLOSED(c);
    { int rc = check_key_width(c->depth, n_targets, c->n_rx, "rts_set_scene"); if (rc != RTS_OK) return rc; }
    RtsSceneFlat flat;
    { int rc = rts_scene_flatten(meshes, n_targets, c->params.interpolate_smooth, &flat); if (rc != RTS_OK) return rc; }
    std::unique_ptr<RtsScene> ns(new RtsScene()); ns->device = c->device;
    { int rc = scene_upload(c, ns.get(), flat); if (rc != RTS_OK) return rc; }
    const auto t_build0 = std::chrono::steady_clock::now();
    RtsSceneTuning st; st.device_build = (c->params.flags & RTS_FLAG_HOST_BUILD) == 0;
    rts_tuning_read(&st, rts_env);
    { int rc = scene_build(c, ns.get(), meshes, flat, st); if (rc != RTS_OK) return rc; }
    { int rc = scene_finish(c, ns.get(), st); if (rc != RTS_OK) return rc; }
    ns->build_ms = std::chrono::duration<double, std::milli>(std::chrono::steady_clock::now() - t_build0).count();
    return scene_swap(c, ns.release());
}

extern "C" int rts_share_scene(RtsHandle dst, RtsHandle src)
{
    if (!dst || !src || dst == src) { rts_set_error("rts_share_scene: needs two distinct handles"); return RTS_ERR_INVALID; }
    if (dst->device != src->device) { rts_set_error("rts_share_scene: handles live on different devices (%d, %d)", dst->device, src->device); return RTS_ERR_INVALID; }
    if (dst->params.interpolate_smooth && !src->params.interpolate_smooth) {
        for (const RtsMeshHost& m : src->scene->meshes) if (m.n_tris && m.n_normals == 0) { rts_set_error("rts_share_scene: the scene has a mesh without normals but the receiving handle interpolates normals"); return RTS_ERR_INVALID; }
    }
    RtsContext* c = dst;
    CHECK_HANDLE(c);
    CHECK_CLOSED(c);
    RTS_HIP(hipStreamSynchronize(c->stream));
    if (dst->scene == src->scene) return RTS_OK;
    rts_scene_unref(dst->scene);
    dst->scene = src->scene; dst->scene->refs++;
    { int rc = rts_attach_scene(dst); if (rc != RTS_OK) return rc; }
    if (dst->tune.share_history && src->tune.share_history && dst->params.width == src->params.width) {
        rts_hist_unref(dst->hist);
        dst->hist = src->hist; dst->hist->refs++;
    }
    return RTS_OK;
}

extern "C" int rts_scene_info(RtsHandle c, RtsSceneInfo* out)
{
    if (!c || !out) { rts_set_error("rts_scene_info: null argument"); return RTS_ERR_INVALID; }
    const RtsScene* sc = c->scene;
    memset(out, 0, sizeof(*out));
    out->n_targets = (uint32_t)sc->meshes.size(); out->n_prims = sc->n_prims; out->n_nodes = sc->n_nodes; out->n_leaves = sc->n_leaves;
    out->handles_sharing = (uint32_t)sc->refs.load(); out->builder = sc->builder; out->build_ms = sc->build_ms;
    out->shared_device_bytes = sc->device_bytes(); out->version_bytes = sc->d_nodes4v.cap * sizeof(RtsNode4);
    out->handle_device_bytes = c->d_leaves.cap * sizeof(RtsLeafTri) + c->d_verts_world.cap * 8 + c->d_normals_world.cap * 8 + c->d_params.cap;
    return RTS_OK;
}

extern "C" int rts_get_bvh(RtsHandle c, void* nodes128, uint32_t* leaf_prim, int32_t* roots, uint32_t node_capacity, uint32_t leaf_capacity, uint32_t* n_leaves)
{
    CHECK_HANDLE(c);
    if (n_leaves) *n_leaves = c->scene->n_leaves;
    if ((nodes128 && node_capacity < c->scene->n_nodes) || (leaf_prim && leaf_capacity < c->scene->n_leaves)) { rts_set_error("rts_get_bvh: capacity too small (%u nodes, %u leaves)", c->scene->n_nodes, c->scene->n_leaves); return RTS_ERR_CAPACITY; }
    RTS_HIP(hipStreamSynchronize(c->stream));
    if (nodes128 && c->scene->n_nodes) {
        RTS_HIP(hipMemcpy(nodes128, c->scene->d_nodes4.p, sizeof(RtsNode4)*c->scene->n_nodes, hipMemcpyDeviceToHost));
        RtsNode4* nd = static_cast<RtsNode4*>(nodes128);
        for (uint32_t i = 0; i < c->scene->n_nodes; i++) for (int k = 0; k < 4; k++) { nd[i].child[k] = nd[i].pad[k]; nd[i].pad[k] = 0; }
    }
    if (leaf_prim && c->scene->n_leaves) RTS_HIP(hipMemcpy(leaf_prim, c->scene->d_leaf_prim.p, sizeof(uint32_t)*c->scene->n_leaves, hipMemcpyDeviceToHost));
    if (roots) for (size_t t = 0; t < c->scene->blas.size(); t++) roots[t] = c->scene->blas[t].root;
    return RTS_OK;
}
```

### rts_amd/csrc/rts_trace.hip

```cpp
#include "rts_internal.h"
#include "rts_raygen.h"
#include "rts_ray_ops.h"

struct RtsSlabRay { float iNx, cNx, iFx, cFx, iNy, cNy, iFy, cFy, iNz, cNz, iFz, cFz; };
__device__ __forceinline__ void rts_slab_axis(float o, float d, float E, float& iN_, float& cN_, float& iF_, float& cF_)
{
    const float iv = 1.0f / d;
    const bool pos = !(iv < 0.0f);
    const float oN = o + (pos ? E : -E), oF = o - (pos ? E : -E);
    const float iN = iv * 0.9999994f, iF = iv * 1.0000006f;
    const float cN = -(oN * iN), cF = -(oF * iF);
    const bool drop = !(fabsf(iv) < 1.0e30f);
    const float NINF = -__builtin_inff(), PINF = __builtin_inff();
    iN_ = drop ? 0.0f : iN; cN_ = drop ? NINF : cN;
    iF_ = drop ? 0.0f : iF; cF_ = drop ? PINF : cF;
}
__device__ __forceinline__ RtsSlabRay rts_slab_setup(const dvec3& o, const dvec3& d, float extra)
{
    RtsSlabRay r;
    const float ox = (float)o.x, oy = (float)o.y, oz = (float)o.z;
    const float E = fmaxf(fmaxf(fabsf(ox), fabsf(oy)), fabsf(oz)) * 4.5e-7f + extra + 1.0e-30f;
    rts_slab_axis(ox, (float)d.x, E, r.iNx, r.cNx, r.iFx, r.cFx);
    rts_slab_axis(oy, (float)d.y, E, r.iNy, r.cNy, r.iFy, r.cFy);
    rts_slab_axis(oz, (float)d.z, E, r.iNz, r.cNz, r.iFz, r.cFz);
// ... 208 lines not shown
        const bool busy = node != SENTINEL;
        const unsigned long long busy_m = __ballot(busy);
        if (busy_m == 0ULL) break;
        if (++steps > (1u << 24)) { hard_overflow = true; break; }
        const unsigned long long idle_m = __ballot(true) & ~busy_m;
        if (idle_m != 0ULL) {
            const bool can = busy && sp > bot && bot < lds_cap;
            const unsigned long long can_m = __ballot(can);
            if (can_m != 0ULL) {
                const unsigned long long idle_g = idle_m & gmask, can_g = can_m & gmask;
                const uint32_t n_give = min((uint32_t)__popcll(idle_g), (uint32_t)__popcll(can_g));
                const uint32_t r_can = (uint32_t)__popcll(can_g & below_me), r_idle = (uint32_t)__popcll(idle_g & below_me);
                if (can && r_can < n_give) { row[r_can] = s_stack[bot * RTS_BLOCK + tid]; s_stack[bot * RTS_BLOCK + tid] = SENTINEL; bot++; }
                __builtin_amdgcn_wave_barrier();
                if (!busy && r_idle < n_give) { node = row[r_idle]; sp = 1; bot = 1; }
                __builtin_amdgcn_wave_barrier();
            }
        }
        bool improved = false;
        if (node != SENTINEL) {
            const float before = t_prune;
            rts_walk_step<COUNT, VERS ? RTS_WALK_VERSIONS : RTS_WALK_PLANES>(a, s_stack, tid, gtid, lds_cap, n_spill_lds, node, sp, lp, prev, dir, tmin, best_t, best_leaf, best_prim, t_prune, n_nodes, n_tris, hard_overflow);
            improved = t_prune != before;
        }
        if (__any(improved)) { for (int o = (int)CG / 2; o > 0; o >>= 1) t_prune = fminf(t_prune, __shfl_xor(t_prune, o)); }
    }
    const unsigned long long key = best_leaf >= 0 ? (((unsigned long long)__float_as_uint(best_t) << 32) | best_prim) : ~0ULL;
    unsigned long long kmin = key;
    for (int o = (int)CG / 2; o > 0; o >>= 1) { const unsigned long long w = __shfl_xor(kmin, o); kmin = w < kmin ? w : kmin; }
    const unsigned long long has_m = __ballot(key == kmin) & gmask;
    const int win = has_m ? __ffsll((long long)has_m) - 1 : (int)lane;
    const int leaf_w = __shfl(best_leaf, win);
    if (kmin != ~0ULL) {
        best_leaf = leaf_w; best_t = __uint_as_float((uint32_t)(kmin >> 32)); best_prim = (uint32_t)kmin;
        t_prune = f32_next_up_pos(best_t);
    }
}

#define RTS_RXP_QQW 3
#define RTS_RXP_R2W 4
#define RTS_RXP_QN 5
#define RTS_RXP_QQ 6
#define RTS_RXP_R2 7
#define RTS_RXP_E2 8
#define RTS_RXP_CT 9
#define RTS_RXP_ST 10
#define RTS_RXP_CH 11
#define RTS_RXP_SLO 12
#define RTS_RXP_SHI 13
#define RTS_RXP_OK 14
#define RTS_RXP_RW 15
#define RTS_RXP_N 16
struct RtsUnitLds { int32_t* stack; int32_t* exch; double* first; unsigned long long* path; uint32_t* n; const RtsRxDev* rx; const float (*rxp)[RTS_RXP_N]; uint32_t* lane_scratch; uint32_t* walk; };
struct RtsRay { dvec3 dir, prev; double rayLength, power, doppler, refx, refy; uint32_t reflDepth, refrDepth; int received; bool end, chain_start; };

template <bool KEEP_ALL, bool REFR, bool COOP, uint32_t CG = 64u>
__device__ __forceinline__ bool rts_shade(const RtsTraceArgs& a, const RtsUnitLds& L_, const uint32_t tid, const uint32_t gtid, const uint32_t lane, const uint32_t slot,
                                          const uint32_t chain, const uint32_t D, const uint32_t max_refr, const dvec3& origin, const bool primary, const bool may_rx,
                                          const float best_t, const int best_leaf, const uint32_t best_prim, const float tmin, RtsRay& S, uint32_t& pending, uint32_t& refr_code0)
{
    double* const s_first = L_.first; unsigned long long* const s_path = L_.path; uint32_t* const s_n = L_.n; const RtsRxDev* const s_rx = L_.rx;
    dvec3& dir = S.dir; dvec3& prev = S.prev;
    double& rayLength = S.rayLength; double& power = S.power; double& doppler = S.doppler; double& refx = S.refx; double& refy = S.refy;
    uint32_t& reflDepth = S.reflDepth; uint32_t& refrDepth = S.refrDepth; int& received = S.received; bool& end = S.end; bool& chain_start = S.chain_start;
        if (KEEP_ALL && chain == 0 && (!COOP || (lane & (CG - 1u)) == 0u)) {
            const size_t hidx = (size_t)slot * (a.max_refl + 1) + reflDepth;
            a.hit_prim[hidx] = (best_leaf >= 0) ? (int32_t)best_prim : -1;
            a.hit_t[hidx] = (best_leaf >= 0) ? best_t : 0.0f;
        }

        if (best_leaf < 0) {
            if (end == false && (!primary || may_rx)) {
                for (uint32_t Rx_i = 0; Rx_i < a.n_rx; Rx_i++) {
                    const RtsRxDev rx = Rx_i < RTS_RX_LDS ? s_rx[Rx_i] : a.rx[Rx_i];
                    double t[2] = {0, 0};
                    const double A = (dir.x)*(dir.x) + (dir.y)*(dir.y) + (dir.z)*(dir.z);
                    const double B = 2*(((prev.x - rx.cx)*dir.x) + ((prev.y - rx.cy)*dir.y) + ((prev.z - rx.cz)*dir.z));
                    const double C = prev.x*prev.x + prev.y*prev.y + prev.z*prev.z + (rx.cx*rx.cx) + (rx.cy*rx.cy) + (rx.cz*rx.cz) -
                                     2*((rx.cx*prev.x) + (rx.cy*prev.y) + (rx.cz*prev.z)) - rx.radius*rx.radius;
                    double discriminant = B*B - 4*A*C;
                    if (discriminant > 0.f) {
                        discriminant = sqrt(discriminant);
                        t[0] = (-B - discriminant)/(2*A);
                        t[1] = (-B + discriminant)/(2*A);
                        unsigned int received_root = 2;
    #pragma unroll
                        for (int i = 0; i < 2; i++) {
                            if ((t[i] >= 0) && ((rayLength + t[i]) > SCENE_EPS) && ((rayLength + t[i]) > SCENE_EPS_R)) {
                                const dvec3 ep = mk3(prev.x + t[i]*dir.x, prev.y + t[i]*dir.y, prev.z + t[i]*dir.z);
                                double theta = rts_atan2f((float)(ep.y - rx.cy), (float)(ep.x - rx.cx));
                                double phi = rts_atan2f((float)(ep.z - rx.cz), (float)sqrt(((ep.y - rx.cy) * (ep.y - rx.cy)) + ((ep.x - rx.cx) * (ep.x - rx.cx))));
                                if ((phi < -RTS_PI/2)) { theta += RTS_PI; phi = -RTS_PI - phi; }
                                if ((phi > RTS_PI/2)) { theta += RTS_PI; phi = RTS_PI - phi; }
                                double maxTheta1 = rx.maxTheta, minTheta1 = rx.minTheta, maxTheta2 = maxTheta1, minTheta2 = minTheta1;
                                double maxPhi1 = rx.maxPhi, minPhi1 = rx.minPhi, maxPhi2 = maxPhi1, minPhi2 = minPhi1;
                                if ((minPhi1 < -RTS_PI/2)) { maxTheta2 += RTS_PI; minTheta2 += RTS_PI; maxPhi2 = -RTS_PI - minPhi1; minPhi2 = -RTS_PI/2; minPhi1 = -RTS_PI/2; }
                                if ((maxPhi1 > RTS_PI/2)) { maxTheta2 += RTS_PI; minTheta2 += RTS_PI; minPhi2 = RTS_PI - maxPhi1; maxPhi2 = RTS_PI/2; maxPhi1 = RTS_PI/2; }
                                if (((rts_angle_in_range(theta, minTheta1, maxTheta1)) && (rts_angle_in_range(phi, minPhi1, maxPhi1))) ||
                                    ((rts_angle_in_range(theta, minTheta2, maxTheta2)) && (rts_angle_in_range(phi, minPhi2, maxPhi2)))) {
                                    if (received_root == 2) received_root = i;
                                    else if (t[received_root] > t[i]) received_root = i;
                                }
                            }
                        }
                        if (received_root < 2) {
                            end = true;
// ... 71 lines not shown
                normal = mk3(n[0], n[1], n[2]);
            } else {
                const double* n0 = a.normals + 3*(size_t)ni[0]; const double* n1 = a.normals + 3*(size_t)ni[1]; const double* n2 = a.normals + 3*(size_t)ni[2];
                const double w = 1.0f - h.beta - h.gamma;
                normal = mk3(n1[0]*h.beta + n2[0]*h.gamma + n0[0]*w, n1[1]*h.beta + n2[1]*h.gamma + n0[1]*w, n1[2]*h.beta + n2[2]*h.gamma + n0[2]*w);
            }
            normal = unit3(normal);
        } else {
            normal = unit3(h.n);
        }
        const fvec3 dirf = (chain == 0 && chain_start) ? unit3_to_f32(dir) : mk3f((float)dir.x, (float)dir.y, (float)dir.z);
        const fvec3 nf = unit3_to_f32(normal);

        const double rrefx = refy;
        if (REFR) {
            if ((fabs(T.reflCoeff) != 1.00000f) && (refrDepth < max_refr) && (reflDepth == 0)) {
                const double rrefy = (rrefx == 1) ? T.refrIndex : 1.0;
                const float ratio = (float)(rrefy / rrefx);
                fvec3 rd;
                if (refract3f(rd, dirf, nf, ratio)) {
                    RtsChildState cs;
                    cs.prevx = prev.x; cs.prevy = prev.y; cs.prevz = prev.z; cs.firstx = s_first[tid]; cs.firsty = s_first[RTS_BLOCK + tid]; cs.firstz = s_first[2 * RTS_BLOCK + tid];
                    cs.rayLength = rayLength; cs.refx = rrefx; cs.refy = rrefy; cs.end = end ? 1u : 0u;
                    double cpower = power;
                    if ((reflDepth + 1) < (a.max_refl + 1)) cpower *= (1 - fabs(T.reflCoeff));
                    cs.power = cpower;
                    cs.refrDepth = refrDepth + 1;
                    const dvec3 k0 = unit3(dir);
                    const dvec3 nd3 = widen3(rd);
                    const dvec3 k1 = unit3(nd3);
                    cs.doppler = doppler + dot3(mk3(T.vx, T.vy, T.vz), sub3(k1, k0));
                    cs.dx = rd.x; cs.dy = rd.y; cs.dz = rd.z;
                    cs.refr_code = (chain == 0) ? (L.targ + 1) : (uint32_t)(s_path[tid] & 0xff);
                    if (chain == 0) refr_code0 = L.targ + 1;
                    a.child[(size_t)chain * a.slab_threads + gtid] = cs;
                    pending |= 1u << (chain + 1);
                    float* dh = a.dir_hist + (size_t)((chain + 1) * (a.max_refl + 1)) * 3 * a.n_rays;
                    if (!COOP || (lane & (CG - 1u)) == 0u) { dh[slot] = rd.x; dh[(size_t)a.n_rays + slot] = rd.y; dh[2*(size_t)a.n_rays + slot] = rd.z; }
                }
            }
        }
        reflDepth++;
        refy = rrefx; refx = rrefx;
        chain_start = false;
        if (!(reflDepth < a.max_refl + 1)) return false;
        const fvec3 nd = reflect3f(dirf, nf);
        power *= T.reflCoeff;
        if (KEEP_ALL || REFR) {
            const dvec3 k0 = unit3(dir);
            const dvec3 k1 = unit3(widen3(nd));
            doppler += dot3(mk3(T.vx, T.vy, T.vz), sub3(k1, k0));
        }
        dir = widen3(nd);
        {
            const size_t plane = REFR ? (size_t)chain * (a.max_refl + 1) + reflDepth : (size_t)(reflDepth - 1);
            float* dh = a.dir_hist + plane * 3 * a.n_rays;
            if (!COOP || (lane & (CG - 1u)) == 0u) { dh[slot] = nd.x; dh[(size_t)a.n_rays + slot] = nd.y; dh[2*(size_t)a.n_rays + slot] = nd.z; }
        }
    return true;
}


template <bool KEEP_ALL, bool REFR, bool COOP, uint32_t CG = 64u>
__device__ __forceinline__ void rts_write_back(const RtsTraceArgs& a, const RtsUnitLds& L_, const uint32_t tid, const uint32_t lane, const uint32_t slot, const uint32_t chain,
                                               const RtsRay& S, const uint32_t pending, const uint32_t refr_code0)
{
    const double* const s_first = L_.first; const unsigned long long* const s_path = L_.path;
    const dvec3& prev = S.prev; const double rayLength = S.rayLength, power = S.power, doppler = S.doppler;
    const uint32_t reflDepth = S.reflDepth, refrDepth = S.refrDepth; const int received = S.received;
    const bool recv = received >= 0;
    if ((recv || KEEP_ALL) && (!COOP || (lane & (CG - 1u)) == 0u)) {
        RtsEndRecord r;
        r.rayLength = rayLength; r.power = power; r.doppler = (KEEP_ALL || REFR) ? doppler : 0.0;
        r.prevx = prev.x; r.prevy = prev.y; r.prevz = prev.z;
        r.firstx = s_first[tid]; r.firsty = s_first[RTS_BLOCK + tid]; r.firstz = s_first[2 * RTS_BLOCK + tid];
        r.path_lo = s_path[tid]; r.path_hi = s_path[RTS_BLOCK + tid]; r.slot = slot; r.received = received; r.reflDepth = reflDepth;
        r.pad = chain | (refrDepth << 2) | ((chain == 0 ? refr_code0 : 0u) << 8) | ((pending & 6u) << 15);
        if (KEEP_ALL) a.all_records[(size_t)chain * a.n_rays + slot] = r;
        if (recv) {
            unsigned long long idx = atomicAdd(&a.counters[0], 1ULL);
            a.recv_records[idx] = r;
        }
    }
}

__device__ __forceinline__ bool rts_rx_maybe(const float* K, const float dx, const float dy, const float dz, const float dd, const float delta)
{
    const float qx = K[0], qy = K[1], qz = K[2], qn = K[RTS_RXP_QN];
    const float b = qx*dx + qy*dy + qz*dz;
    const float R = K[RTS_RXP_RW] + qn * delta, r2w = delta > 0.0f ? R * R : K[RTS_RXP_R2W];
    const bool inside = K[RTS_RXP_QQW] <= K[RTS_RXP_R2W] * 1.01f;
    const bool ahead = b > -(1.0e-3f + delta) * qn && (b*b - (K[RTS_RXP_QQW] - r2w) * dd) >= 0.0f;
    if (!(inside || ahead)) return false;
    if (K[RTS_RXP_OK] == 0.0f) return true;
    const float e2 = K[RTS_RXP_E2], s2 = b*b - (K[RTS_RXP_QQ] - K[RTS_RXP_R2]);
    if (!(s2 >= 16.0f * e2)) return true;
    const float s = __builtin_sqrtf(s2);
    float dt = 0.0f;
    if (delta > 0.0f) {
        const float qd = qn * delta;
        if (!(s2 - qd * (2.2f * fabsf(b) + qd) >= 0.5f * s2)) return true;
        dt = qd * (1.0f + (2.0f * fabsf(b) + qd) / (1.7f * s));
    }
    const float et = 0.75f * e2 / s + 1.0e-6f * qn;
    const float tl_min = fabsf(b >= 0.0f ? b + s : b - s) - et - dt;
    const bool small_gone = tl_min > 0.0f && (fabsf(K[RTS_RXP_QQ] - K[RTS_RXP_R2]) + e2) / tl_min + et < 0.004999f;
// ... 52 lines not shown
        const float iwa = __builtin_amdgcn_rcpf(wa), iwb = __builtin_amdgcn_rcpf(wb);
        const float fua = ((ax * mf.ux + ay * mf.uy + az * mf.uz) * iwa - mf.u0) * mf.inv_du, fva = ((ax * mf.vx + ay * mf.vy + az * mf.vz) * iwa - mf.v0) * mf.inv_dv;
        const float fub = ((bx * mf.ux + by * mf.uy + bz * mf.uz) * iwb - mf.u0) * mf.inv_du, fvb = ((bx * mf.vx + by * mf.vy + bz * mf.vz) * iwb - mf.v0) * mf.inv_dv;
        const float ulo = fminf(fua, fub), uhi = fmaxf(fua, fub), vlo = fminf(fva, fvb), vhi = fmaxf(fva, fvb);
        if (!(ulo >= 0.0f && vlo >= 0.0f && uhi < (float)mf.n && vhi < (float)mf.n)) return true;
        const bool major_u = (uhi - ulo) >= (vhi - vlo);
        float a0 = major_u ? fua : fva, a1 = major_u ? fub : fvb, b0 = major_u ? fva : fua, b1 = major_u ? fvb : fub;
        if (a0 > a1) { const float t0 = a0; a0 = a1; a1 = t0; const float t1 = b0; b0 = b1; b1 = t1; }
        const uint32_t c0 = (uint32_t)a0, c1 = (uint32_t)a1;
        if (c1 - c0 > 96u) return true;
        const float slope = (a1 - a0) > 1.0e-6f ? (b1 - b0) / (a1 - a0) : 0.0f;
        const float nmax = (float)(mf.n - 1u);
        uint32_t found = 0u;
        for (uint32_t c = c0; c <= c1; c++) {
            const float la = fmaxf(a0, (float)c), ha = fminf(a1, (float)(c + 1u));
            const float bl = b0 + slope * (la - a0), bh = b0 + slope * (ha - a0);
            const uint32_t r0 = (uint32_t)fminf(fmaxf(fminf(bl, bh) - 0.03125f, 0.0f), nmax), r1 = (uint32_t)fminf(fmaxf(fmaxf(bl, bh) + 0.03125f, 0.0f), nmax);
            for (uint32_t r = r0; r <= r1; r++) { const uint32_t cell = major_u ? r * mf.n + c : c * mf.n + r; found |= pmask[cell >> 5] >> (cell & 31u); }
        }
        if (found & 1u) return true;
    }
    const float ex = ax - bx, ey = ay - by, ez = az - bz;
    const float delta = 1.6f * __builtin_sqrtf(ex*ex + ey*ey + ez*ez) + 4.0e-6f;
    const float dd = ax*ax + ay*ay + az*az;
    for (uint32_t Rx_i = 0; Rx_i < n_rx; Rx_i++) if (rts_rx_maybe(rxp[Rx_i], ax, ay, az, dd, delta)) return true;
    return false;
}
__device__ __forceinline__ bool rts_tile_maybe(const RtsLaunchConsts& lc, const uint32_t tile, const uint32_t n_rays, const bool has_prims, const bool mask_on, const uint32_t* __restrict__ pmask,
                                               const uint32_t n_rx, const float (*rxp)[RTS_RXP_N])
{
    const uint32_t s0 = tile * 64u, s1 = min(s0 + 63u, n_rays - 1u);
    uint32_t lx, ly, lz;
    rts_lattice_coords(lc, s0, lx, ly, lz);
    uint32_t left = s1 - s0 + 1u;
    bool maybe = false;
    while (left != 0u && !maybe) {
        const uint32_t n = min(left, lc.W - lx);
        maybe = rts_segment_maybe(lc, lx, lx + n - 1u, ly, lz, has_prims, mask_on, pmask, n_rx, rxp);
        left -= n; lx = 0u;
        if (++ly == lc.W) { ly = 0u; lz++; }
    }
    return maybe;
}

__device__ __forceinline__ void rts_primary_setup(const RtsTraceArgs& a, const RtsLaunchConsts& lc, const RtsUnitLds& L_, const uint32_t tid, const uint32_t slot, const bool pre_on,
                                                  const bool mask_on, const dvec3& origin, RtsRay& S, bool& may_target, bool& may_rx, const bool pre_done = false)
{
    double* const s_first = L_.first; unsigned long long* const s_path = L_.path; const float (*const s_rxp)[RTS_RXP_N] = L_.rxp;
    dvec3& dir = S.dir; dvec3& prev = S.prev; double& rayLength = S.rayLength; double& power = S.power; double& doppler = S.doppler;
    if (pre_on && !pre_done) rts_prefilter(lc, slot, mask_on, a.pmask, a.n_rx, s_rxp, may_target, may_rx);
    dir = (may_target || may_rx) ? rts_primary_dir(lc, slot) : mk3(0.0, 0.0, 0.0);
    prev = origin;
    s_first[tid] = 0.0; s_first[RTS_BLOCK + tid] = 0.0; s_first[2 * RTS_BLOCK + tid] = 0.0;
    s_path[tid] = 0ULL; s_path[RTS_BLOCK + tid] = 0ULL;
    rayLength = 0; power = 0; doppler = 0;
}

template <bool COUNT, bool KEEP_ALL, bool REFR, bool COOP, bool VERS = false>
__device__ __forceinline__ void rts_trace_unit(const RtsTraceArgs& a, const RtsLaunchConsts& lc, const RtsUnitLds& L_, const uint32_t tid, const uint32_t gtid, const uint32_t lane,
                                               const uint32_t slot, const bool pre_on, const bool mask_on, const uint32_t D, const uint32_t max_refr, const dvec3& origin,
                                               uint32_t& n_nodes, uint32_t& n_tris, bool& hard_overflow, unsigned long long (&lane_stats)[5],
                                               const uint32_t pre = 0u)
{
      int32_t* const s_stack = L_.stack; int32_t* const s_exch = L_.exch; double* const s_first = L_.first; unsigned long long* const s_path = L_.path; uint32_t* const s_n = L_.n;
      constexpr uint32_t CG = (COOP && VERS) ? (uint32_t)RTS_COOP_GROUP : 64u;

      uint32_t pending = 0;
      uint32_t refr_code0 = 0;
      for (uint32_t chain = 0; chain < (REFR ? 3u : 1u); chain++) {
        RtsRay S;
        dvec3& dir = S.dir; dvec3& prev = S.prev;
        double& rayLength = S.rayLength; double& power = S.power; double& doppler = S.doppler; double& refx = S.refx; double& refy = S.refy;
        uint32_t& reflDepth = S.reflDepth; uint32_t& refrDepth = S.refrDepth; bool& end = S.end; bool& chain_start = S.chain_start;
        refx = 1; refy = 1; reflDepth = 0; refrDepth = 0; S.received = -1; end = false;
        bool may_target = a.n_prims > 0, may_rx = a.n_rx > 0;
        if (pre & 1u) { may_target = (pre & 2u) != 0u; may_rx = (pre & 4u) != 0u; }
        if (chain == 0) {
            rts_primary_setup(a, lc, L_, tid, slot, pre_on, mask_on, origin, S, may_target, may_rx, (pre & 1u) != 0u);
        } else {
            if (!REFR || !(pending & (1u << chain))) continue;
            const RtsChildState cs = a.child[(size_t)(chain - 1) * a.slab_threads + gtid];
            dir = mk3((double)cs.dx, (double)cs.dy, (double)cs.dz);
            prev = mk3(cs.prevx, cs.prevy, cs.prevz);
            s_first[tid] = cs.firstx; s_first[RTS_BLOCK + tid] = cs.firsty; s_first[2 * RTS_BLOCK + tid] = cs.firstz;
            rayLength = cs.rayLength; power = cs.power; doppler = cs.doppler; refx = cs.refx; refy = cs.refy;
            refrDepth = cs.refrDepth; end = cs.end != 0;
            const uint64_t code = cs.refr_code;
            uint64_t path_lo = 0, path_hi = 0;
            for (uint32_t col = 0; col < (chain == 1 ? D : 2u); col++) { if (col < 8) path_lo |= code << (8 * col); else path_hi |= code << (8 * (col - 8)); }
            s_path[tid] = path_lo; s_path[RTS_BLOCK + tid] = path_hi;
        }
        chain_start = true;

        for (;;) {
            if (!COOP || (lane & (CG - 1u)) == 0u) atomicAdd(&s_n[tid], RTS_SEG_ONE);
            if (!COOP) { const unsigned long long ex_ = __ballot(true);
                         if (__builtin_amdgcn_mbcnt_hi((uint32_t)(ex_ >> 32), __builtin_amdgcn_mbcnt_lo((uint32_t)ex_, 0u)) == 0u) atomicAdd(&L_.walk[2u * __builtin_amdgcn_readfirstlane(tid >> 6) + 1u], 1u); }
            const float tmin = chain_start ? SCENE_EPS : SCENE_EPS_R;
            float best_t = RTS_DEFAULT_TMAX;
            int best_leaf = -1; uint32_t best_prim = 0xffffffffu;
            const bool primary = chain == 0 && chain_start;
            const bool may_hit = primary ? may_target : a.n_prims > 0;
            uint32_t steps = 0;
            if (may_hit) {
                float t_prune = RTS_DEFAULT_TMAX;
                for (uint32_t targ = 0; targ < a.n_targets; targ++) {
                    const RtsTargetDev& TG = a.targets[targ];
                    if (TG.root < 0) continue;
                    {
                        const dvec3 q = mk3(TG.cx - prev.x, TG.cy - prev.y, TG.cz - prev.z);
                        const double qq = q.x*q.x + q.y*q.y + q.z*q.z, b = q.x*dir.x + q.y*dir.y + q.z*dir.z;
                        if (qq > TG.r2) {
                            const double dd = dir.x*dir.x + dir.y*dir.y + dir.z*dir.z;
                            if (!(b > 0.0) || !(b*b >= (qq - TG.r2) * dd * 0.999999)) continue;
                        }
                    }
                    const dvec3 q = mk3(prev.x - TG.px, prev.y - TG.py, prev.z - TG.pz);
                    const dvec3 ol = mk3(TG.rinv[0]*q.x + TG.rinv[1]*q.y + TG.rinv[2]*q.z, TG.rinv[3]*q.x + TG.rinv[4]*q.y + TG.rinv[5]*q.z, TG.rinv[6]*q.x + TG.rinv[7]*q.y + TG.rinv[8]*q.z);
                    const dvec3 dl = mk3(TG.rinv[0]*dir.x + TG.rinv[1]*dir.y + TG.rinv[2]*dir.z, TG.rinv[3]*dir.x + TG.rinv[4]*dir.y + TG.rinv[5]*dir.z, TG.rinv[6]*dir.x + TG.rinv[7]*dir.y + TG.rinv[8]*dir.z);
                    const RtsSlabRay lr = rts_slab_setup(ol, dl, TG.ew);
                    const uint32_t oct = VERS ? ((__float_as_uint(lr.iNx) >> 31) | ((__float_as_uint(lr.iNy) >> 31) << 1) | ((__float_as_uint(lr.iNz) >> 31) << 2)) : 0u;
                    const int SENTINEL = RTS_STACK_SENTINEL;
                    const int lds_cap = (int)a.stack_lds;
                    if (COOP) {
                        rts_walk_coop<COUNT, VERS, CG>(a, s_stack, s_exch, tid, gtid, lane, lds_cap, &s_n[2 * RTS_BLOCK + tid], VERS ? (int)(((uint32_t)TG.root << 3) | oct) : TG.root, lr, prev, dir, tmin, best_t, best_leaf, best_prim, t_prune,
                                             n_nodes, n_tris, hard_overflow);
                        if (COUNT) steps = 1u;
                    } else {
                        s_stack[tid] = SENTINEL;
                        int sp = 1;
                        int node = VERS ? (int)(((uint32_t)TG.root << 3) | oct) : TG.root;
                        uint32_t wave_steps = 0;
                        while (node != SENTINEL) {
                            wave_steps = __builtin_amdgcn_readfirstlane(wave_steps) + 1u;
                            if (wave_steps > (1u << 24)) { hard_overflow = true; break; }
                            if (COUNT) steps++;
                            rts_walk_step<COUNT, VERS ? RTS_WALK_VERSIONS : RTS_WALK_ROLES>(a, s_stack, tid, gtid, lds_cap, &s_n[2 * RTS_BLOCK + tid], node, sp, lr, prev, dir, tmin, best_t, best_leaf, best_prim, t_prune,
                                                 n_nodes, n_tris, hard_overflow);
                        }
                        { const unsigned long long ex_ = __ballot(true);
                          if (__builtin_amdgcn_mbcnt_hi((uint32_t)(ex_ >> 32), __builtin_amdgcn_mbcnt_lo((uint32_t)ex_, 0u)) == 0u) { atomicAdd(&L_.walk[2u * __builtin_amdgcn_readfirstlane(tid >> 6)], wave_steps); } }
                    }
                }
            }
            if (COUNT && !COOP) {
                uint32_t* ls = L_.lane_scratch + 2u * (tid >> 6);
                const unsigned long long act = __ballot(true);
                if (lane == (uint32_t)(__ffsll((long long)act) - 1)) { ls[0] = 0u; ls[1] = 0u; }
                atomicMax(&ls[0], steps); atomicAdd(&ls[1], steps);
                const uint32_t smax = ls[0], ssum = ls[1];
                lane_stats[0] += 64ull * smax; lane_stats[1] += (unsigned long long)__popcll(act) * smax; lane_stats[2] += ssum;
                lane_stats[3] += (unsigned long long)__popcll(__ballot(steps > 0u));
                lane_stats[4] += (unsigned long long)__popcll(__ballot(steps == 0u)) * smax;
            }
            if (COUNT && COOP && steps) lane_stats[3] += 1ull;
            {
                const bool go_on_ = rts_shade<KEEP_ALL, REFR, COOP, CG>(a, L_, tid, gtid, lane, slot, chain, D, max_refr, origin, primary, may_rx, best_t, best_leaf, best_prim, tmin, S, pending, refr_code0);
                if (!go_on_) break;
            }
        }

        rts_write_back<KEEP_ALL, REFR, COOP, CG>(a, L_, tid, lane, slot, chain, S, pending, refr_code0);
      }
}

#define RTS_COST_UNITS(ticks) (((unsigned long long)(ticks) * 3ULL) >> 3)

template <bool COUNT, bool KEEP_ALL, bool REFR, bool COOP, bool VERS = false>
__global__ void __launch_bounds__(RTS_BLOCK, (REFR && COOP) ? 2 : ((REFR || COOP) ? 3 : 4)) k_trace(const RtsTraceArgs a)
{
    __shared__ __attribute__((aligned(16))) int32_t s_stack[RTS_STACK_LDS * RTS_BLOCK];
    const uint32_t tid = threadIdx.x;
    const uint32_t gtid = (COOP ? a.total_threads : 0u) + blockIdx.x * RTS_BLOCK + tid;
    __shared__ __attribute__((aligned(16))) RtsLaunchConsts s_lc;
    __shared__ __attribute__((aligned(16))) RtsRxDev s_rx[RTS_RX_LDS];
    __shared__ __attribute__((aligned(16))) double s_first[3 * RTS_BLOCK];
    __shared__ __attribute__((aligned(16))) unsigned long long s_path[2 * RTS_BLOCK];
    __shared__ uint32_t s_n[3 * RTS_BLOCK];
    s_n[threadIdx.x] = 0; s_n[RTS_BLOCK + threadIdx.x] = 0; s_n[2 * RTS_BLOCK + threadIdx.x] = 0;
    {
        const uint32_t* src = reinterpret_cast<const uint32_t*>(a.lc); uint32_t* dst = reinterpret_cast<uint32_t*>(&s_lc);
        for (uint32_t i = threadIdx.x; i < sizeof(RtsLaunchConsts) / 4; i += RTS_BLOCK) dst[i] = src[i];
        const uint32_t n_rx_lds = a.n_rx < RTS_RX_LDS ? a.n_rx : RTS_RX_LDS;
        const uint32_t* rsrc = reinterpret_cast<const uint32_t*>(a.rx); uint32_t* rdst = reinterpret_cast<uint32_t*>(s_rx);
        for (uint32_t i = threadIdx.x; i < n_rx_lds * (sizeof(RtsRxDev) / 4); i += RTS_BLOCK) rdst[i] = rsrc[i];
    }
    __syncthreads();
    const RtsLaunchConsts& lc = s_lc;
    const dvec3 origin = mk3(lc.ox, lc.oy, lc.oz);
    __shared__ float s_rxp[RTS_RX_LDS][RTS_RXP_N];
    if (tid < RTS_RX_LDS && tid < a.n_rx) {
        const RtsRxDev r = s_rx[tid];
        const double qx = r.cx - lc.ox, qy = r.cy - lc.oy, qz = r.cz - lc.oz, qq = qx*qx + qy*qy + qz*qz;
        const double w2 = lc.ox*lc.ox + lc.oy*lc.oy + lc.oz*lc.oz + r.cx*r.cx + r.cy*r.cy + r.cz*r.cz;
        const double r2wd = r.radius * r.radius * 1.001 + 1.0e-5 * qq + 1.0e-6 + 1.0e-14 * w2;
        s_rxp[tid][0] = (float)qx; s_rxp[tid][1] = (float)qy; s_rxp[tid][2] = (float)qz; s_rxp[tid][RTS_RXP_QQW] = (float)qq * 1.000001f;
        s_rxp[tid][RTS_RXP_R2W] = (float)r2wd;
        s_rxp[tid][RTS_RXP_QN] = (float)sqrt(qq);
        const double th_c = 0.5 * (r.minTheta + r.maxTheta), th_h = 0.5 * (r.maxTheta - r.minTheta);
        const bool ok = r.minPhi >= -RTS_PI / 2 && r.maxPhi <= RTS_PI / 2 && r.minPhi < r.maxPhi && th_h > 0.0 && th_h < 1.5 && r.radius > 0.0 && isfinite(th_c) && isfinite(qq);
        s_rxp[tid][RTS_RXP_QQ] = (float)qq; s_rxp[tid][RTS_RXP_R2] = (float)(r.radius * r.radius);
        s_rxp[tid][RTS_RXP_E2] = (float)(2.0e-6 * qq + 1.0e-6 * r.radius * r.radius + 1.0e-14 * w2 + 1.0e-12);
        s_rxp[tid][RTS_RXP_CT] = (float)cos(th_c); s_rxp[tid][RTS_RXP_ST] = (float)sin(th_c); s_rxp[tid][RTS_RXP_CH] = (float)cos(th_h);
        s_rxp[tid][RTS_RXP_SLO] = (float)(r.radius * sin(r.minPhi)); s_rxp[tid][RTS_RXP_SHI] = (float)(r.radius * sin(r.maxPhi));
        s_rxp[tid][RTS_RXP_OK] = (ok && a.rx_window_screen) ? 1.0f : 0.0f;
        s_rxp[tid][RTS_RXP_RW] = (float)(sqrt(r2wd) * 1.000001);
    }
    __syncthreads();
    uint32_t n_nodes = 0, n_tris = 0;
    bool hard_overflow = false;
    const bool mask_on = a.pmask != nullptr && lc.mask.n != 0 && a.pmask[(size_t)lc.mask.n * lc.mask.n / 32u] == 0u;
    const bool pre_on = lc.W > 1 && a.n_rx <= RTS_RX_LDS && (mask_on || a.n_prims == 0) && a.pre_filter;
    const uint32_t max_refr = REFR ? 2u : 0u;
    const uint32_t D = a.max_refl + max_refr;

    unsigned long long tl_t0 = 0;
    if (!COOP && a.timeline && tid == 0) { tl_t0 = wall_clock64(); a.timeline[(size_t)blockIdx.x * 2] = tl_t0; }
    const uint32_t n_tiles = (a.n_rays + 63u) / 64u;
    const uint32_t lane = tid & 63u;
    const uint32_t wave_u = __builtin_amdgcn_readfirstlane(tid >> 6);
    const uint32_t stripe = __builtin_amdgcn_readfirstlane((blockIdx.x * (RTS_BLOCK / 64u) + (tid >> 6)) % RTS_TILE_CTRS);
    const uint32_t n_head = (a.tile_head && a.tile_order) ? min(min(__builtin_amdgcn_readfirstlane(a.tile_head[0]), n_tiles), 16384u) : 0u;
    constexpr uint32_t CG = (COOP && VERS) ? (uint32_t)RTS_COOP_GROUP : 64u;
    constexpr uint32_t RPU = 64u / CG;
    const uint32_t n_units = COOP ? CG * n_head : n_tiles - n_head;
    __shared__ int32_t s_exch[COOP ? RTS_BLOCK : 1];
    __shared__ uint32_t s_lane_scratch[COUNT ? 2 * (RTS_BLOCK / 64) : 1];
    __shared__ uint32_t s_walk[2 * (RTS_BLOCK / 64)];
    const RtsUnitLds ul = {s_stack, s_exch, s_first, s_path, s_n, s_rx, s_rxp, s_lane_scratch, s_walk};
    unsigned long long lane_stats[5] = {0ull, 0ull, 0ull, 0ull, 0ull};
#define RTS_OPAQUE_S(x) ({ uint32_t o_ = (x); asm volatile("" : "+s"(o_)); o_; })
    uint32_t coop_x = 0, coop_sweep = 0, coop_len = 0;
    const uint32_t coop_P = COOP ? a.coop_spread : 1u, coop_G = RTS_XCD / coop_P;
#define RTS_COOP_LEN(x) (n_head > ((x) % coop_G) ? (n_head - ((x) % coop_G) + coop_G - 1u) / coop_G : 0u)
    if (COOP) {
        asm volatile("s_getreg_b32 %0, hwreg(HW_REG_XCC_ID)" : "=s"(coop_x));
        coop_x &= (RTS_XCD - 1u);
        coop_len = RTS_COOP_LEN(coop_x);
    }
    const uint32_t S = COOP ? (uint32_t)RTS_SEG_STRIPES : (uint32_t)RTS_TILE_CTRS;
#define RTS_LSTRIPE (COOP ? (stripe & (RTS_SEG_STRIPES - 1u)) : RTS_OPAQUE_S(stripe))
    const uint32_t per_stripe_all = (n_units + RTS_TILE_CTRS - 1u) / RTS_TILE_CTRS;
    constexpr bool BATCHABLE = !COOP && !KEEP_ALL;
    __shared__ uint32_t s_sched[(RTS_BLOCK / 64) * 8];
#define RTS_SCHED(k) s_sched[RTS_OPAQUE_S(wave_u) * 8u + (k)]
    const uint32_t single_draws_nobatch = per_stripe_all >= 1024u ? per_stripe_all / 4u : per_stripe_all;
    if (BATCHABLE) {
        uint32_t k_dead = per_stripe_all;
        if (a.batch_dead != 0u && pre_on) {
            if (a.batch_dead == 2u) k_dead = 0u;
            else if (a.tile_live && a.tile_order) {
                const uint32_t lv = __builtin_amdgcn_readfirstlane(a.tile_live[0]);
                if (lv) { const uint32_t v_dead = lv - 1u > n_head ? lv - 1u - n_head : 0u; k_dead = min(per_stripe_all, v_dead > stripe ? (v_dead - stripe + RTS_TILE_CTRS - 1u) / RTS_TILE_CTRS : 0u); }
            }
        }
        const uint32_t s1 = min(single_draws_nobatch, k_dead);
        if (lane == 0) { RTS_SCHED(0) = s1; RTS_SCHED(1) = (k_dead - s1 + 3u) / 4u; RTS_SCHED(2) = k_dead; }
    }
    const uint32_t single_draws_all = single_draws_nobatch;
    __shared__ uint32_t s_draw[RTS_BLOCK / 64];
    uint32_t draw_next = 0;
#define RTS_DRAW() { const uint32_t dv_ = atomicAdd(&a.tile_ctr[(COOP ? RTS_OFF_CTR_COOP : 0) + ((COOP ? coop_x * S : 0u) + RTS_LSTRIPE) * RTS_TILE_CTR_STRIDE], 1u); if (COUNT || KEEP_ALL) s_draw[wave_u] = dv_; else draw_next = dv_; }
    if (lane == 0) RTS_DRAW()
    for (;;) {
      const uint32_t draw = __builtin_amdgcn_readfirstlane((COUNT || KEEP_ALL) ? s_draw[wave_u] : draw_next);
      const uint32_t per_stripe = COOP ? (coop_len * (CG / coop_P) + RTS_SEG_STRIPES - 1u) / RTS_SEG_STRIPES : per_stripe_all;
      const uint32_t single_draws = COOP ? per_stripe : (BATCHABLE ? __builtin_amdgcn_readfirstlane(RTS_SCHED(0)) : single_draws_all);
      const uint32_t four_draws = BATCHABLE ? __builtin_amdgcn_readfirstlane(RTS_SCHED(1)) : 0u, k_dead = BATCHABLE ? __builtin_amdgcn_readfirstlane(RTS_SCHED(2)) : 0u;
      const bool batch = BATCHABLE && draw >= single_draws + four_draws;
      const uint32_t k0 = draw < single_draws ? draw : (batch ? k_dead + 64u * (draw - single_draws - four_draws) : single_draws + 4u * (draw - single_draws));
      const uint32_t kn = draw < single_draws ? 1u : (batch ? 64u : (BATCHABLE ? min(4u, k_dead - k0) : 4u));
      if (k0 >= per_stripe) {
          if (COOP) {
              if (++coop_sweep >= RTS_XCD) break;
              coop_x = (coop_x + 1u) & (RTS_XCD - 1u);
              coop_len = RTS_COOP_LEN(coop_x);
              if (lane == 0) RTS_DRAW()
              continue;
          }
          break;
      }
      const uint32_t seg_len = COOP ? coop_len * (CG / coop_P) : n_units;
      const bool ahead = draw >= single_draws;
// ... 29 lines not shown
          const uint32_t per = CG / coop_P, j = (uint32_t)vloc64 / per, i = (uint32_t)vloc64 - j * per, h = (coop_x % coop_G) + coop_G * j;
          vpos = (h << 6) | ((((coop_x - h) & (RTS_XCD - 1u)) / coop_G) + coop_P * i);
      }
      const bool coop_unit = COOP;
      const uint32_t tpos = COOP ? (vpos >> 6) : vpos + n_head;
      const uint32_t tile = a.tile_order ? a.tile_order[tpos] : ((tpos & 1u) ? (n_tiles - 1u) / 2u + (tpos + 1u) / 2u : (n_tiles - 1u) / 2u - tpos / 2u);
      const uint32_t slot = coop_unit ? tile * 64u + (vpos & 63u) * RPU + lane / CG : tile * 64u + lane;
      uint32_t pre = 0u;
      if (!COOP && !KEEP_ALL && pre_on) {
          bool pre_target = a.n_prims > 0, pre_rx = a.n_rx > 0;
          if (slot < a.n_rays) rts_prefilter(lc, slot, mask_on, a.pmask, a.n_rx, s_rxp, pre_target, pre_rx);
          if (!__any(slot < a.n_rays && (pre_target || pre_rx))) {
              if (slot < a.n_rays) atomicAdd(&s_n[tid], 1u);
              if (lane == 0 && a.tile_cost) a.tile_cost[tile] = 1u;
              continue;
          }
          pre = 1u | (pre_target ? 2u : 0u) | (pre_rx ? 4u : 0u);
      }
      const long long tile_t0 = wall_clock64();
      const long long tile_s0 = COUNT ? clock64() : 0;
      if (!COOP) atomicAnd(&s_n[tid], 0x003fffffu);
      if (!COOP && lane == 0) { const uint32_t z_ = RTS_OPAQUE_S(0u); s_walk[2u * wave_u] = z_; s_walk[2u * wave_u + 1u] = z_; }
      const unsigned long long tl_tile = (COUNT && a.timeline && lane == 0) ? wall_clock64() : 0ULL;
      if (slot < a.n_rays) {
          rts_trace_unit<COUNT, KEEP_ALL, REFR, COOP, VERS>(a, lc, ul, tid, gtid, lane, slot, pre_on, mask_on, D, max_refr, origin, n_nodes, n_tris, hard_overflow, lane_stats, pre);
      }
      const unsigned long long dt = RTS_COST_UNITS(wall_clock64() - tile_t0);
      if (COUNT && !COOP && lane == 0 && clock64() - tile_s0 < 0) {
          uint32_t xcc; asm volatile("s_getreg_b32 %0, hwreg(HW_REG_XCC_ID)" : "=s"(xcc));
          atomicAdd(&a.counters[14], 1ULL); atomicOr(&a.counters[14], 1ULL << (56u + (xcc & 7u)));
      }
      bool long_walks = false, longish_walks = false;
      if (!COOP && a.tile_cost && dt >= a.coop_min_cost) {
          const uint32_t wsteps = __builtin_amdgcn_readfirstlane(s_walk[2u * wave_u]), walks = __builtin_amdgcn_readfirstlane(s_walk[2u * wave_u + 1u]);
          long_walks = walks != 0u && (unsigned long long)wsteps >= (unsigned long long)a.coop_walk_steps * walks;
          longish_walks = walks != 0u && (unsigned long long)wsteps >= (unsigned long long)a.coop_walk_steps_lo * walks;
      }
      if (lane == 0) {
          if (a.tile_cost && dt >= (1ULL << 26)) atomicAdd(&a.counters[12], 1ULL);
          if (a.tile_cost && dt < (1ULL << 26)) {
              if (COOP) { atomicAdd(&a.tile_cost[tile], ((unsigned int)(dt > 0x00fffffeULL ? 0x00fffffeULL : dt) + 1u) * RPU); if ((vpos & 63u) == 0u) atomicOr(&a.tile_cost[tile], 0x80000000u); }
              else a.tile_cost[tile] = ((unsigned int)(dt > 0x3ffffffeULL ? 0x3ffffffeULL : dt) + 1u) | (long_walks ? 0x80000000u : 0u) | (longish_walks ? 0x40000000u : 0u);
          }
          if (COUNT && a.timeline && !coop_unit) { a.timeline[(size_t)gridDim.x * 2 + tile] = wall_clock64() - tl_tile; a.timeline[(size_t)gridDim.x * 2 + n_tiles + tile] = tl_tile; }
      }
     }
      if (!ahead && lane == 0) RTS_DRAW()
    }
    if (!COOP && a.timeline && tid == 0) a.timeline[(size_t)blockIdx.x * 2 + 1] = wall_clock64();

    if (COUNT && !COOP && lane == 0 && lane_stats[0]) { atomicAdd(&a.counters[8], lane_stats[0]); atomicAdd(&a.counters[9], lane_stats[1]); atomicAdd(&a.counters[10], lane_stats[2]); }
    if (COUNT && (lane & (CG - 1u)) == 0u && lane_stats[3]) atomicAdd(&a.counters[11], lane_stats[3]);
    if (COUNT && !COOP && lane == 0 && lane_stats[4]) atomicAdd(&a.counters[15], lane_stats[4]);
    const uint32_t tid_e = (wave_u << 6) | __builtin_amdgcn_mbcnt_hi(~0u, __builtin_amdgcn_mbcnt_lo(~0u, 0u));
    unsigned long long n_seg = s_n[tid_e] & 0x003fffffu, n_shaded = s_n[RTS_BLOCK + tid_e], n_spill = s_n[2 * RTS_BLOCK + tid_e], n_nodes_w = n_nodes, n_tris_w = n_tris;
    for (int off = 32; off > 0; off >>= 1) {
        n_seg += __shfl_down(n_seg, off); n_shaded += __shfl_down(n_shaded, off);
        if (COUNT) { n_nodes_w += __shfl_down(n_nodes_w, off); n_tris_w += __shfl_down(n_tris_w, off); }
        n_spill += __shfl_down(n_spill, off);
    }
    __syncthreads();
    unsigned long long* s_cnt = reinterpret_cast<unsigned long long*>(s_stack);
    const int wave = (int)wave_u;
    if ((tid_e & 63) == 0) {
        s_cnt[wave * 8 + 1] = n_seg; s_cnt[wave * 8 + 2] = n_shaded; s_cnt[wave * 8 + 3] = COUNT ? n_nodes_w : 0ULL;
        s_cnt[wave * 8 + 4] = COUNT ? n_tris_w : 0ULL; s_cnt[wave * 8 + 5] = n_spill;
    }
    const bool any_overflow = __syncthreads_or(hard_overflow ? 1 : 0) != 0;
    if (tid_e >= 1 && tid_e <= 6) {
        unsigned long long v = 0;
        if (tid_e <= 5) { for (int w = 0; w < RTS_BLOCK / 64; w++) v += s_cnt[w * 8 + tid_e]; }
        else v = any_overflow ? 1ULL : 0ULL;
        a.block_counters[((size_t)(COOP ? a.total_threads / RTS_BLOCK : 0u) + blockIdx.x) * 8 + tid_e] = v;
    }
}

__global__ void k_sum_counters(const unsigned long long* __restrict__ block_counters, unsigned int n_blocks, unsigned long long* __restrict__ counters, const uint32_t* __restrict__ head_count,
                               unsigned long long* __restrict__ host_cnt)
{
    __shared__ unsigned long long s[256];
    const uint32_t t = threadIdx.x;
#define RTS_LD64(p) __hip_atomic_load((p), __ATOMIC_RELAXED, __HIP_MEMORY_SCOPE_AGENT)
    if (t == 7) { const unsigned long long h = head_count ? (unsigned long long)__hip_atomic_load(head_count, __ATOMIC_RELAXED, __HIP_MEMORY_SCOPE_AGENT) : 0ULL; counters[7] = h; host_cnt[7] = h; }
    if (t == 0) host_cnt[0] = RTS_LD64(&counters[0]);
    if ((t >= 8 && t <= 12) || t == 14 || t == 15) host_cnt[t] = RTS_LD64(&counters[t]);
    const unsigned int k = t & 7u, lane = t >> 3;
    unsigned long long v = 0;
    unsigned long long poisoned = 0;
    if (k >= 1 && k <= 6) for (unsigned int b = lane; b < n_blocks; b += 32) { const unsigned long long x = RTS_LD64(&block_counters[(size_t)b * 8 + k]); if (x == ~0ULL) poisoned++; else v += x; }
    s[t] = v;
    if (k == 1 && poisoned) { atomicAdd(&counters[13], poisoned); __threadfence(); }
    __syncthreads();
    if (t >= 1 && t <= 6) {
        unsigned long long sum = 0;
        for (unsigned int l = 0; l < 32; l++) sum += s[l * 8 + t];
        counters[t] = sum; host_cnt[t] = sum;
    }
    if (t == 13) host_cnt[13] = RTS_LD64(&counters[13]);
#undef RTS_LD64
}

template <bool COOP>
static void rts_trace_dispatch(const RtsTraceArgs& a, bool count_traversal, unsigned grid, hipStream_t st)
{
    const int sel = (a.max_refr ? 4 : 0) | (a.keep_all ? 2 : 0) | (count_traversal ? 1 : 0);
    if (!COOP && a.nodes4v) {
        switch (sel) {
            case 0: k_trace<false, false, false, false, true><<<grid, RTS_BLOCK, 0, st>>>(a); break;
            case 1: k_trace<true, false, false, false, true><<<grid, RTS_BLOCK, 0, st>>>(a); break;
            case 2: k_trace<false, true, false, false, true><<<grid, RTS_BLOCK, 0, st>>>(a); break;
            case 3: k_trace<true, true, false, false, true><<<grid, RTS_BLOCK, 0, st>>>(a); break;
            case 4: k_trace<false, false, true, false, true><<<grid, RTS_BLOCK, 0, st>>>(a); break;
            case 5: k_trace<true, false, true, false, true><<<grid, RTS_BLOCK, 0, st>>>(a); break;
            case 6: k_trace<false, true, true, false, true><<<grid, RTS_BLOCK, 0, st>>>(a); break;
            default: k_trace<true, true, true, false, true><<<grid, RTS_BLOCK, 0, st>>>(a); break;
        }
        return;
    }
    if (COOP && a.nodes4v && a.coop_versions && sel < 2) {
        if (sel == 0) k_trace<false, false, false, true, true><<<grid, RTS_BLOCK, 0, st>>>(a);
        else k_trace<true, false, false, true, true><<<grid, RTS_BLOCK, 0, st>>>(a);
        return;
    }
    switch (sel) {
        case 0: k_trace<false, false, false, COOP><<<grid, RTS_BLOCK, 0, st>>>(a); break;
        case 1: k_trace<true, false, false, COOP><<<grid, RTS_BLOCK, 0, st>>>(a); break;
        case 2: k_trace<false, true, false, COOP><<<grid, RTS_BLOCK, 0, st>>>(a); break;
        case 3: k_trace<true, true, false, COOP><<<grid, RTS_BLOCK, 0, st>>>(a); break;
        case 4: k_trace<false, false, true, COOP><<<grid, RTS_BLOCK, 0, st>>>(a); break;
        case 5: k_trace<true, false, true, COOP><<<grid, RTS_BLOCK, 0, st>>>(a); break;
        case 6: k_trace<false, true, true, COOP><<<grid, RTS_BLOCK, 0, st>>>(a); break;
        default: k_trace<true, true, true, COOP><<<grid, RTS_BLOCK, 0, st>>>(a); break;
    }
}

int rts_trace_launch(RtsContext* c, const RtsTraceArgs& a, bool count_traversal, unsigned coop_grid)
{
    if (a.n_rays == 0) {
// ... 28 lines not shown
```

Baseline: 24720.

## Skip self-target traversal after reflection using precomputed per-triangle horizon bounds

```diff
diff --git a/include/rts_amd.h b/include/rts_amd.h
--- a/include/rts_amd.h
+++ b/include/rts_amd.h
@@ -33,6 +33,7 @@
 #define RTS_FLAG_DEVICE_BUILD 4u
 #define RTS_FLAG_HOST_BUILD 16u
 #define RTS_FLAG_NO_PREFILTER 8u
+#define RTS_FLAG_NO_HORIZON 32u
 #define RTS_FLAG_COUNT_TRAVERSAL 2u
 
 typedef struct RtsMesh {
@@ -123,8 +124,10 @@
     uint64_t shared_device_bytes;
     uint64_t handle_device_bytes;
     uint64_t version_bytes;
+    uint64_t horizon_bytes;
 } RtsSceneInfo;
 int rts_scene_info(RtsHandle h, RtsSceneInfo* out);
+int rts_get_horizon(RtsHandle h, float* out, uint32_t capacity_prims);
 
 int rts_trace_pulse(RtsHandle h, const RtsPulse* pulse);
 
diff --git a/rts_amd/_lib.py b/rts_amd/_lib.py
--- a/rts_amd/_lib.py
+++ b/rts_amd/_lib.py
@@ -14,6 +14,7 @@
 RTS_FLAG_DEVICE_BUILD = 4
 RTS_FLAG_HOST_BUILD = 16
 RTS_FLAG_NO_PREFILTER = 8
+RTS_FLAG_NO_HORIZON = 32
 RTS_MAX_DEPTH = 16
 RTS_BASE_USE_ROWS = 0xffffffffffffffff
 
@@ -288,7 +289,8 @@
 class RtsSceneInfo(C.Structure):
     _fields_ = [("n_targets", C.c_uint32), ("n_prims", C.c_uint32), ("n_nodes", C.c_uint32), ("n_leaves", C.c_uint32),
                 ("handles_sharing", C.c_uint32), ("builder", C.c_uint32), ("build_ms", C.c_double),
-                ("shared_device_bytes", C.c_uint64), ("handle_device_bytes", C.c_uint64), ("version_bytes", C.c_uint64)]
+                ("shared_device_bytes", C.c_uint64), ("handle_device_bytes", C.c_uint64), ("version_bytes", C.c_uint64),
+                ("horizon_bytes", C.c_uint64)]
 
 
 class RtsStats(C.Structure):
@@ -354,7 +356,7 @@
            "rts_finalise_uniform", "rts_trace_pulse_end_uniform", "rts_aggregate", "rts_group_count", "rts_get_groups", "rts_get_aggregated",
            "rts_merge_groups", "rts_groups_to_responses", "rts_kernel_wrapper", "rts_vertex_rotation",
            "rts_rotation_matrix", "rts_rect_mesh", "rts_sphere_mesh", "rts_file_mesh", "rts_rx_sphere", "rts_get_bvh",
-           "rts_build_id", "rts_bind_host_to_device", "rts_get_lane_stats", "rts_get_walk_stats", "rts_self_test_math", "rts_cube_attach", "rts_cube_accumulate", "rts_cube_get", "rts_cube_accumulate_paths", "rts_cube_doppler", "rts_cube_doppler_get", "rts_plan_cpi", "rts_cube_reduce", "rts_kernel_wrapper_on",
+           "rts_build_id", "rts_bind_host_to_device", "rts_get_lane_stats", "rts_get_walk_stats", "rts_get_horizon", "rts_self_test_math", "rts_cube_attach", "rts_cube_accumulate", "rts_cube_get", "rts_cube_accumulate_paths", "rts_cube_doppler", "rts_cube_doppler_get", "rts_plan_cpi", "rts_cube_reduce", "rts_kernel_wrapper_on",
            "rts_received_prefetch", "rts_received_view", "rts_finalise_values", "rts_aggregated_view", "rts_build_hierarchy_host",
            "rts_tile_records_get", "rts_tile_records_set", "rts_deal_tiles", "rts_set_tile_list",
            "rts_set_patterns", "rts_finalise_patterns", "rts_trace_pulse_end_patterns", "rts_pattern_eval",
@@ -426,7 +428,7 @@
         "rts_get_bvh": [vp, vp, vp, vp, u32, u32, vp],
         "rts_cube_attach": [vp, C.POINTER(RtsCubeParams), vp],
         "rts_cube_accumulate": [vp, u32, dbl, dbl],
-        "rts_cube_get": [vp, vp, u64], "rts_get_lane_stats": [vp, vp], "rts_get_walk_stats": [vp, vp, C.c_uint32], "rts_bind_host_to_device": [C.c_int, C.POINTER(C.c_int)],
+        "rts_cube_get": [vp, vp, u64], "rts_get_lane_stats": [vp, vp], "rts_get_walk_stats": [vp, vp, C.c_uint32], "rts_get_horizon": [vp, vp, u32], "rts_bind_host_to_device": [C.c_int, C.POINTER(C.c_int)],
         "rts_cube_accumulate_paths": [vp, u32], "rts_cube_doppler": [vp, u32, vp], "rts_cube_doppler_get": [vp, vp, u64],
         "rts_plan_cpi": [u64, u32, u32, u32, u32, u32, u32, vp, u32, C.POINTER(u32)],
         "rts_cube_reduce": [vp, u32, C.c_int],
diff --git a/rts_amd/api.py b/rts_amd/api.py
--- a/rts_amd/api.py
+++ b/rts_amd/api.py
@@ -675,11 +675,11 @@
 
 class Tracer:
 
-    def __init__(self, width, max_refl, max_refr=0, smooth=True, device=0, keep_all=False, count_traversal=False, device_build=None, pre_filter=True):
+    def __init__(self, width, max_refl, max_refr=0, smooth=True, device=0, keep_all=False, count_traversal=False, device_build=None, pre_filter=True, horizon=True):
         p = L.RtsParams(width, max_refl, max_refr, 1 if smooth else 0, device,
                         (L.RTS_FLAG_KEEP_ALL_RAYS if keep_all else 0) | (L.RTS_FLAG_COUNT_TRAVERSAL if count_traversal else 0) |
                         (0 if device_build is None else (L.RTS_FLAG_DEVICE_BUILD if device_build else L.RTS_FLAG_HOST_BUILD)) |
-                         (0 if pre_filter else L.RTS_FLAG_NO_PREFILTER))
+                         (0 if pre_filter else L.RTS_FLAG_NO_PREFILTER) | (0 if horizon else L.RTS_FLAG_NO_HORIZON))
         self.h = C.c_void_p()
         check(L.lib().rts_create(C.byref(p), C.byref(self.h)))
         self.width = width; self.max_refl = max_refl; self.depth = max_refl + (2 if max_refr else 0)
@@ -707,6 +707,16 @@
                                float(m.get("refl_coeff", 1.0)), float(m.get("refr_index", 1.0)))
         check(L.lib().rts_set_scene(self.h, arr, len(meshes)))
         self.n_targets = len(meshes)
+
+    def horizon(self, n_prims):
+        out = np.zeros((int(n_prims), 2), np.float32)
+        check(L.lib().rts_get_horizon(self.h, ptr(out), int(n_prims)))
+        return out
+
+    def walk_stats(self):
+        ls = (C.c_uint64 * 11)()
+        check(L.lib().rts_get_walk_stats(self.h, ls, 11))
+        return [int(v) for v in ls]
 
     def share_scene(self, other):
         check(L.lib().rts_share_scene(self.h, other.h))
diff --git a/rts_amd/csrc/rts_api.hip b/rts_amd/csrc/rts_api.hip
--- a/rts_amd/csrc/rts_api.hip
+++ b/rts_amd/csrc/rts_api.hip
@@ -316,6 +316,7 @@
     td.rinv[6] = (R[3]*R[7] - R[4]*R[6]) * id; td.rinv[7] = (R[1]*R[6] - R[0]*R[7]) * id; td.rinv[8] = (R[0]*R[4] - R[1]*R[3]) * id;
     td.px = m.position[0]; td.py = m.position[1]; td.pz = m.position[2];
     td.root = b.root;
+    { const RtsHorizonMesh& hz = c->scene->hz[t]; td.hz_h0 = (float)hz.h0 * 1.000001f; td.hz_rho = det > 0.0 ? (float)hz.rho * 0.999999f : 0.0f; }
     double cl[3], half2 = 0, wc[3], wmax = 0;
     for (int i = 0; i < 3; i++) { cl[i] = 0.5 * b.lo[i] + 0.5 * b.hi[i]; const double h = 0.5 * (b.hi[i] - b.lo[i]); half2 += h * h; }
     for (int i = 0; i < 3; i++) { wc[i] = R[3*i]*cl[0] + R[3*i + 1]*cl[1] + R[3*i + 2]*cl[2] + m.position[i]; wmax = std::max(wmax, std::fabs(wc[i])); }
@@ -498,6 +499,7 @@
     a.recv_records = c->d_recv.p; a.all_records = c->d_all.p; a.counters = c->p_counters; a.block_counters = c->d_block_counters.p; a.dir_hist = c->d_dir_hist.p;
     a.hit_prim = c->d_hit_prim.p; a.hit_t = c->d_hit_t.p; a.stack_ovf = c->d_stack_ovf.p; a.child = c->d_child.p;
     a.rx_window_screen = c->tune.rx_window_screen ? 1u : 0u;
+    a.horizon = (c->params.flags & RTS_FLAG_NO_HORIZON) ? 0u : 1u;
     a.coop_versions = c->tune.coop_versions ? 1u : 0u;
     a.tile_ctr = c->d_tile_ctr.p;
     return RTS_OK;
diff --git a/rts_amd/csrc/rts_bvh.hip b/rts_amd/csrc/rts_bvh.hip
--- a/rts_amd/csrc/rts_bvh.hip
+++ b/rts_amd/csrc/rts_bvh.hip
@@ -110,7 +110,8 @@
                                                 const uint32_t* __restrict__ prim_targ, RtsLeafTri* __restrict__ leaves, uint32_t n,
                                                 double ox, double oy, double oz, RtsMaskFrame f, uint32_t* __restrict__ mask,
                                                 const RtsTargetMotion* __restrict__ motion = nullptr, uint32_t prim_blocks = 0, const double* __restrict__ n_local = nullptr,
-                                                double* __restrict__ n_world = nullptr, const uint32_t* __restrict__ n_targ = nullptr, uint32_t n_normals = 0)
+                                                double* __restrict__ n_world = nullptr, const uint32_t* __restrict__ n_targ = nullptr, uint32_t n_normals = 0,
+                                                const float* __restrict__ horizon = nullptr)
 {
     __shared__ __attribute__((aligned(16))) uint32_t s_raw[MASK ? sizeof(RtsMaskLds) / 4 : 1];
     if (PLACE && blockIdx.x >= prim_blocks) {
@@ -137,7 +138,7 @@
             RtsLeafTri L;
             L.p0x = p[0]; L.p0y = p[1]; L.p0z = p[2]; L.e0x = e0.x; L.e0y = e0.y; L.e0z = e0.z; L.e1x = e1.x; L.e1y = e1.y; L.e1z = e1.z;
             L.nx = nn.x; L.ny = nn.y; L.nz = nn.z;
-            L.prim = g; L.targ = prim_targ[g]; L.pad[0] = 0u; L.pad[1] = 0u;
+            L.prim = g; L.targ = prim_targ[g]; L.hz[0] = horizon ? horizon[2*(size_t)g] : 1.0f; L.hz[1] = horizon ? horizon[2*(size_t)g+1] : 1.0f;
             leaves[g] = L;
         }
     }
@@ -155,9 +156,9 @@
     if (place && sc->n_prims) {
         const unsigned gp = blocks_for(sc->n_prims, 256), gn = blocks_for(sc->n_normals, 256);
         if (mask) k_leaves<true, true, true><<<gp + gn, 256, 0, st>>>(sc->d_prim_order.p, sc->d_tri_vidx.p, sc->d_verts_local.p, sc->d_prim_targ.p, c->d_leaves.p, sc->n_prims, lc.ox, lc.oy, lc.oz, f, pmask,
-                                                                     c->p_motion, gp, sc->d_normals_local.p, c->d_normals_world.p, sc->d_norm_targ.p, sc->n_normals);
+                                                                     c->p_motion, gp, sc->d_normals_local.p, c->d_normals_world.p, sc->d_norm_targ.p, sc->n_normals, sc->d_horizon.p);
         else k_leaves<true, false, true><<<gp + gn, 256, 0, st>>>(sc->d_prim_order.p, sc->d_tri_vidx.p, sc->d_verts_local.p, sc->d_prim_targ.p, c->d_leaves.p, sc->n_prims, lc.ox, lc.oy, lc.oz, f, nullptr,
-                                                                  c->p_motion, gp, sc->d_normals_local.p, c->d_normals_world.p, sc->d_norm_targ.p, sc->n_normals);
+                                                                  c->p_motion, gp, sc->d_normals_local.p, c->d_normals_world.p, sc->d_norm_targ.p, sc->n_normals, sc->d_horizon.p);
         c->verts_world_valid = false;
         RTS_HIP(hipGetLastError());
         return RTS_OK;
diff --git a/rts_amd/csrc/rts_horizon.hip b/rts_amd/csrc/rts_horizon.hip
--- /dev/null
+++ b/rts_amd/csrc/rts_horizon.hip
@@ -0,0 +1,137 @@
+#include <cmath>
+#include "rts_internal.h"
+#include "rts_ray_ops.h"
+
+#define RTS_HZ_BLOCK 64u
+#define RTS_HZ_WORK_CAP (1ull << 31)
+#define RTS_HZ_SLICES 8u
+
+struct RtsHzPrim { double cx, cy, cz, r, nx, ny, nz, d; };
+struct RtsHzBlk { double cx, cy, cz, r; uint32_t tlo, thi; };
+
+__global__ void k_hz_prims(const uint32_t* __restrict__ order, const uint32_t* __restrict__ tri_vidx, const double* __restrict__ verts, const uint32_t* __restrict__ prim_targ,
+                           uint32_t n, const RtsHorizonMesh* __restrict__ mesh, uint32_t* __restrict__ mesh_off, RtsHzPrim* __restrict__ hp, double* __restrict__ pv)
+{
+    const uint32_t i = blockIdx.x * blockDim.x + threadIdx.x;
+    if (i >= n) return;
+    const uint32_t g = order[i], t = prim_targ[g];
+    double p[9];
+    for (int k = 0; k < 3; k++) { const uint32_t v = tri_vidx[3 * (size_t)g + k]; for (int a = 0; a < 3; a++) p[3 * k + a] = verts[3 * (size_t)v + a]; }
+    for (int k = 0; k < 9; k++) pv[(size_t)i * 9 + k] = p[k];
+    dvec3 e0, e1, nn;
+    tri_terms(mk3(p[0], p[1], p[2]), mk3(p[3], p[4], p[5]), mk3(p[6], p[7], p[8]), e0, e1, nn);
+    const double nl = sqrt(nn.x * nn.x + nn.y * nn.y + nn.z * nn.z);
+    const double l0 = sqrt(e0.x * e0.x + e0.y * e0.y + e0.z * e0.z), l1 = sqrt(e1.x * e1.x + e1.y * e1.y + e1.z * e1.z);
+    const double e2x = p[6] - p[3], e2y = p[7] - p[4], e2z = p[8] - p[5], l2 = sqrt(e2x * e2x + e2y * e2y + e2z * e2z);
+    const double longest = fmax(l0, fmax(l1, l2));
+    const bool good = isfinite(nl) && isfinite(longest) && longest > 0.0 && nl / longest >= RTS_HZ_DEGEN * mesh[t].extent;
+    if (!good) atomicOr(&mesh_off[t], 1u);
+    RtsHzPrim q;
+    q.cx = (p[0] + p[3] + p[6]) / 3.0; q.cy = (p[1] + p[4] + p[7]) / 3.0; q.cz = (p[2] + p[5] + p[8]) / 3.0;
+    double r2 = 0.0;
+    for (int k = 0; k < 3; k++) { const double dx = p[3 * k] - q.cx, dy = p[3 * k + 1] - q.cy, dz = p[3 * k + 2] - q.cz; r2 = fmax(r2, dx * dx + dy * dy + dz * dz); }
+    q.r = sqrt(r2) * (1.0 + 1e-12);
+    const double inv = good ? 1.0 / nl : 0.0;
+    q.nx = nn.x * inv; q.ny = nn.y * inv; q.nz = nn.z * inv; q.d = q.nx * p[0] + q.ny * p[1] + q.nz * p[2];
+    hp[i] = q;
+}
+
+__global__ void k_hz_blocks(const uint32_t* __restrict__ order, const uint32_t* __restrict__ prim_targ, uint32_t n, uint32_t n_blocks, const RtsHzPrim* __restrict__ hp, RtsHzBlk* __restrict__ hb)
+{
+    const uint32_t b = blockIdx.x * blockDim.x + threadIdx.x;
+    if (b >= n_blocks) return;
+    const uint32_t i0 = b * RTS_HZ_BLOCK, i1 = min(n, i0 + RTS_HZ_BLOCK);
+    double cx = 0, cy = 0, cz = 0; uint32_t tlo = 0xffffffffu, thi = 0u;
+    for (uint32_t i = i0; i < i1; i++) { cx += hp[i].cx; cy += hp[i].cy; cz += hp[i].cz; const uint32_t t = prim_targ[order[i]]; tlo = min(tlo, t); thi = max(thi, t); }
+    const double m = 1.0 / (double)(i1 - i0); cx *= m; cy *= m; cz *= m;
+    double r = 0.0;
+    for (uint32_t i = i0; i < i1; i++) { const double dx = hp[i].cx - cx, dy = hp[i].cy - cy, dz = hp[i].cz - cz; r = fmax(r, sqrt(dx * dx + dy * dy + dz * dz) + hp[i].r); }
+    RtsHzBlk o; o.cx = cx; o.cy = cy; o.cz = cz; o.r = isfinite(r) ? r * (1.0 + 1e-12) : INFINITY; o.tlo = tlo; o.thi = thi;
+    hb[b] = o;
+}
+
+__device__ __forceinline__ double hz_raise(double s, double hmax, double gap, double h0)
+{
+    if (!(hmax <= h0)) s = (gap > 0.0) ? fmax(s, fmin(1.0, hmax / gap)) : 1.0;
+    return s;
+}
+
+__global__ void __launch_bounds__(256) k_hz_main(const uint32_t* __restrict__ order, const uint32_t* __restrict__ prim_targ, uint32_t n, uint32_t n_blocks, const RtsHorizonMesh* __restrict__ mesh,
+                                                 const uint32_t* __restrict__ mesh_off, const RtsHzPrim* __restrict__ hp, const RtsHzBlk* __restrict__ hb, const double* __restrict__ pv,
+                                                 uint32_t* __restrict__ horizon)
+{
+    const uint32_t i = blockIdx.x * blockDim.x + threadIdx.x, slice = blockIdx.y;
+    if (i >= n) return;
+    const uint32_t g = order[i], t = prim_targ[g];
+    double sp = 0.0, sm = 0.0;
+    if (mesh_off[t]) { sp = 1.0; sm = 1.0; }
+    else {
+        const RtsHzPrim T = hp[i];
+        const double h0 = RTS_HZ_H0 * mesh[t].extent, rho = RTS_HZ_RHO * mesh[t].extent;
+        for (uint32_t b = slice; b < n_blocks && !(sp >= 1.0 && sm >= 1.0); b += RTS_HZ_SLICES) {
+            const RtsHzBlk B = hb[b];
+            if (t < B.tlo || t > B.thi) continue;
+            const double hc = T.nx * B.cx + T.ny * B.cy + T.nz * B.cz - T.d;
+            const double dx = B.cx - T.cx, dy = B.cy - T.cy, dz = B.cz - T.cz;
+            const double gap = sqrt(dx * dx + dy * dy + dz * dz) - B.r - T.r - rho;
+            if (hz_raise(sp, hc + B.r, gap, h0) <= sp && hz_raise(sm, -hc + B.r, gap, h0) <= sm) continue;
+            const uint32_t j0 = b * RTS_HZ_BLOCK, j1 = min(n, j0 + RTS_HZ_BLOCK);
+            for (uint32_t j = j0; j < j1; j++) {
+                if (j == i || prim_targ[order[j]] != t) continue;
+                const RtsHzPrim U = hp[j];
+                const double* u = pv + (size_t)j * 9;
+                const double a0 = T.nx * u[0] + T.ny * u[1] + T.nz * u[2] - T.d, a1 = T.nx * u[3] + T.ny * u[4] + T.nz * u[5] - T.d, a2 = T.nx * u[6] + T.ny * u[7] + T.nz * u[8] - T.d;
+                const double ex = U.cx - T.cx, ey = U.cy - T.cy, ez = U.cz - T.cz;
+                const double pg = sqrt(ex * ex + ey * ey + ez * ez) - U.r - T.r - rho;
+                sp = hz_raise(sp, fmax(a0, fmax(a1, a2)), pg, h0);
+                sm = hz_raise(sm, fmax(-a0, fmax(-a1, -a2)), pg, h0);
+            }
+        }
+    }
+    float fp = (float)sp, fm = (float)sm;
+    if ((double)fp < sp) fp = __uint_as_float(__float_as_uint(fp) + 1u);
+    if ((double)fm < sm) fm = __uint_as_float(__float_as_uint(fm) + 1u);
+    atomicMax(&horizon[2 * (size_t)g], __float_as_uint(fminf(fp, 1.0f))); atomicMax(&horizon[2 * (size_t)g + 1], __float_as_uint(fminf(fm, 1.0f)));
+}
+
+int rts_horizon_build(RtsContext* c, RtsScene* ns, const RtsSceneFlat& flat)
+{
+    const uint32_t n = ns->n_prims, n_targets = (uint32_t)ns->meshes.size();
+    ns->hz.assign(n_targets, RtsHorizonMesh{0.0, 0.0, 0.0});
+    if (!n) return RTS_OK;
+    const uint32_t n_blocks = (n + RTS_HZ_BLOCK - 1u) / RTS_HZ_BLOCK;
+    std::vector<uint32_t> off(n_targets, 0u);
+    for (uint32_t t = 0; t < n_targets; t++) {
+        RtsBlasInfo b; rts_mesh_bounds(flat, t, &b);
+        double e2 = 0; for (int a = 0; a < 3; a++) e2 += (b.hi[a] - b.lo[a]) * (b.hi[a] - b.lo[a]);
+        const double E = std::sqrt(e2);
+        ns->hz[t].extent = E; ns->hz[t].h0 = RTS_HZ_H0 * E; ns->hz[t].rho = RTS_HZ_RHO * E;
+        if (!(E > 0.0) || !std::isfinite(E) || (unsigned long long)ns->meshes[t].n_tris * n_blocks > RTS_HZ_WORK_CAP) off[t] = 1u;
+    }
+    DevBuf<RtsHorizonMesh> d_mesh; DevBuf<uint32_t> d_off; DevBuf<RtsHzPrim> d_hp; DevBuf<RtsHzBlk> d_hb; DevBuf<double> d_pv;
+    RTS_HIP(d_mesh.reserve(n_targets)); RTS_HIP(d_off.reserve(n_targets)); RTS_HIP(d_hp.reserve(n)); RTS_HIP(d_hb.reserve(n_blocks)); RTS_HIP(d_pv.reserve((size_t)n * 9));
+    RTS_HIP(ns->d_horizon.reserve((size_t)n * 2));
+    RTS_HIP(hipStreamSynchronize(c->stream));
+    RTS_HIP(hipMemcpy(d_mesh.p, ns->hz.data(), sizeof(RtsHorizonMesh) * n_targets, hipMemcpyHostToDevice));
+    RTS_HIP(hipMemcpy(d_off.p, off.data(), sizeof(uint32_t) * n_targets, hipMemcpyHostToDevice));
+    k_hz_prims<<<(n + 255u) / 256u, 256, 0, c->stream>>>(ns->d_prim_order.p, ns->d_tri_vidx.p, ns->d_verts_local.p, ns->d_prim_targ.p, n, d_mesh.p, d_off.p, d_hp.p, d_pv.p);
+    k_hz_blocks<<<(n_blocks + 255u) / 256u, 256, 0, c->stream>>>(ns->d_prim_order.p, ns->d_prim_targ.p, n, n_blocks, d_hp.p, d_hb.p);
+    RTS_HIP(hipMemsetAsync(ns->d_horizon.p, 0, sizeof(float) * 2 * (size_t)n, c->stream));
+    k_hz_main<<<dim3((n + 255u) / 256u, RTS_HZ_SLICES), 256, 0, c->stream>>>(ns->d_prim_order.p, ns->d_prim_targ.p, n, n_blocks, d_mesh.p, d_off.p, d_hp.p, d_hb.p, d_pv.p, reinterpret_cast<uint32_t*>(ns->d_horizon.p));
+    RTS_HIP(hipGetLastError());
+    RTS_HIP(hipMemcpyAsync(off.data(), d_off.p, sizeof(uint32_t) * n_targets, hipMemcpyDeviceToHost, c->stream));
+    RTS_HIP(hipStreamSynchronize(c->stream));
+    for (uint32_t t = 0; t < n_targets; t++) if (off[t]) ns->hz[t].rho = 0.0;
+    return RTS_OK;
+}
+
+extern "C" int rts_get_horizon(RtsHandle c, float* out, uint32_t capacity_prims)
+{
+    CHECK_HANDLE(c);
+    if (!out) { rts_set_error("rts_get_horizon: null argument"); return RTS_ERR_INVALID; }
+    const RtsScene* sc = c->scene;
+    if (capacity_prims < sc->n_prims) { rts_set_error("rts_get_horizon: capacity too small (%u primitives)", sc->n_prims); return RTS_ERR_CAPACITY; }
+    RTS_HIP(hipStreamSynchronize(c->stream));
+    if (sc->n_prims) RTS_HIP(hipMemcpy(out, sc->d_horizon.p, sizeof(float) * 2 * (size_t)sc->n_prims, hipMemcpyDeviceToHost));
+    return RTS_OK;
+}
diff --git a/rts_amd/csrc/rts_internal.h b/rts_amd/csrc/rts_internal.h
--- a/rts_amd/csrc/rts_internal.h
+++ b/rts_amd/csrc/rts_internal.h
@@ -35,9 +35,14 @@
     double p0x, p0y, p0z, e0x, e0y, e0z, e1x, e1y, e1z, nx, ny, nz;
     uint32_t prim;
     uint32_t targ;
-    uint32_t pad[2];
+    float hz[2];
 };
 static_assert(sizeof(RtsLeafTri) == 112, "leaf size");
+#define RTS_HZ_H0 9.5367431640625e-07
+#define RTS_HZ_RHO 0.00390625
+#define RTS_HZ_DEGEN 9.5367431640625e-07
+#define RTS_HZ_MARGIN 0.00390625f
+struct RtsHorizonMesh { double extent, h0, rho; };
 static_assert(offsetof(RtsLeafTri, p0x) == 0 && offsetof(RtsLeafTri, p0z) == 16 && offsetof(RtsLeafTri, e0y) == 32 && offsetof(RtsLeafTri, e1x) == 48 &&
               offsetof(RtsLeafTri, e1z) == 64 && offsetof(RtsLeafTri, ny) == 80 && offsetof(RtsLeafTri, prim) == 96 && offsetof(RtsLeafTri, targ) == 100,
               "leaf record offsets of the walk step's decode");
@@ -51,6 +56,7 @@
     double rinv[9];
     double px, py, pz;
     double cx, cy, cz, r2;
+    float hz_h0, hz_rho;
     float ew;
     int32_t root;
 };
@@ -94,7 +100,7 @@
 #define RTS_OFF_HEAD (2 * RTS_TILE_CTRS_LAYOUT * RTS_TILE_CTR_STRIDE)
 #define RTS_OFF_LIVE (RTS_OFF_HEAD + 4)
 #define RTS_OFF_COUNTERS (RTS_OFF_HEAD + 8)
-#define RTS_OFF_BINS (RTS_OFF_COUNTERS + 32)
+#define RTS_OFF_BINS (RTS_OFF_COUNTERS + 48)
 #define RTS_OFF_TAKEN (RTS_OFF_BINS + RTS_TILE_BUCKETS)
 #define RTS_ZERO_WORDS (RTS_OFF_TAKEN + RTS_TILE_BUCKETS)
 #ifndef RTS_RX_LDS
@@ -165,6 +171,7 @@
     uint32_t pre_filter;
     const uint32_t* pmask;
     uint32_t stack_lds;
+    uint32_t horizon;
 };
 
 #define RTS_PIN_GROUPS 4096
@@ -173,7 +180,7 @@
     RtsLaunchConsts lc;
     RtsTargetMotion motion[256];
     RtsTargetDev td[256];
-    unsigned long long cnt[16];
+    unsigned long long cnt[24];
     uint32_t G, pad;
     double rcs[256];
     double gsum[5 * RTS_PIN_GROUPS]; uint64_t gkey[RTS_PIN_GROUPS]; uint64_t grow[RTS_PIN_GROUPS]; uint32_t gmin[RTS_PIN_GROUPS];
@@ -191,10 +198,12 @@
     DevBuf<RtsNode4> d_nodes4; DevBuf<uint32_t> d_leaf_prim;
     DevBuf<uint32_t> d_prim_order;
     DevBuf<RtsNode4> d_nodes4v;
+    DevBuf<float> d_horizon;
+    std::vector<RtsHorizonMesh> hz;
     double build_ms = 0; uint32_t builder = 0;
     size_t device_bytes() const {
         return d_tri_vidx.cap * 4 + d_tri_nidx.cap * 4 + d_vert_targ.cap * 4 + d_norm_targ.cap * 4 + d_prim_targ.cap * 4 + d_verts_local.cap * 8 +
-               d_normals_local.cap * 8 + (d_nodes4.cap + d_nodes4v.cap) * sizeof(RtsNode4) + d_leaf_prim.cap * 4 + d_prim_order.cap * 4;
+               d_normals_local.cap * 8 + (d_nodes4.cap + d_nodes4v.cap) * sizeof(RtsNode4) + d_leaf_prim.cap * 4 + d_prim_order.cap * 4 + d_horizon.cap * 4;
     }
 };
 
@@ -352,6 +361,7 @@
 
 int rts_sah_build(const double* verts, const uint32_t* tris, uint32_t n_tris, double split_budget, std::vector<RtsNode4>& nodes, std::vector<uint32_t>& leaf_prim, RtsBlasInfo& out);
 int rts_lbvh_build_device(RtsContext* c, RtsScene* ns, const RtsSceneFlat& flat, const RtsSceneTuning& tune);
+int rts_horizon_build(RtsContext* c, RtsScene* ns, const RtsSceneFlat& flat);
 int rts_scene_place(RtsContext* c, const RtsLaunchConsts& lc, bool place, uint32_t* pmask);
 int rts_tile_costs_flush(RtsContext* c);
 int rts_tile_records_masked(RtsContext* c, uint32_t* d_out, uint32_t n);
diff --git a/rts_amd/csrc/rts_results_api.hip b/rts_amd/csrc/rts_results_api.hip
--- a/rts_amd/csrc/rts_results_api.hip
+++ b/rts_amd/csrc/rts_results_api.hip
@@ -41,8 +41,8 @@
 {
     if (!c || !out) { rts_set_error("%s: null argument", who); return RTS_ERR_INVALID; }
     CHECK_CLOSED(c);
-    const int src[5] = {8, 9, 10, 11, 15};
-    for (uint32_t k = 0; k < n && k < 5u; k++) out[k] = c->pin.p->cnt[src[k]];
+    const int src[11] = {8, 9, 10, 11, 15, 16, 17, 18, 19, 20, 21};
+    for (uint32_t k = 0; k < n && k < 11u; k++) out[k] = c->pin.p->cnt[src[k]];
     return RTS_OK;
 }
 extern "C" int rts_get_lane_stats(RtsHandle c, uint64_t* out3) { return rts_walk_counters(c, "rts_get_lane_stats", out3, 3); }
diff --git a/rts_amd/csrc/rts_scene.hip b/rts_amd/csrc/rts_scene.hip
--- a/rts_amd/csrc/rts_scene.hip
+++ b/rts_amd/csrc/rts_scene.hip
@@ -164,6 +164,11 @@
     rts_tuning_read(&st, rts_env);
     { int rc = scene_build(c, ns.get(), meshes, flat, st); if (rc != RTS_OK) return rc; }
     { int rc = scene_finish(c, ns.get(), st); if (rc != RTS_OK) return rc; }
+    {
+        const auto t_hz0 = std::chrono::steady_clock::now();
+        int rc = rts_horizon_build(c, ns.get(), flat); if (rc != RTS_OK) return rc;
+        if (st.debug_build) fprintf(stderr, "[rts] horizon: %.2f ms\n", std::chrono::duration<double, std::milli>(std::chrono::steady_clock::now() - t_hz0).count());
+    }
     ns->build_ms = std::chrono::duration<double, std::milli>(std::chrono::steady_clock::now() - t_build0).count();
     return scene_swap(c, ns.release());
 }
@@ -198,6 +203,7 @@
     out->n_targets = (uint32_t)sc->meshes.size(); out->n_prims = sc->n_prims; out->n_nodes = sc->n_nodes; out->n_leaves = sc->n_leaves;
     out->handles_sharing = (uint32_t)sc->refs.load(); out->builder = sc->builder; out->build_ms = sc->build_ms;
     out->shared_device_bytes = sc->device_bytes(); out->version_bytes = sc->d_nodes4v.cap * sizeof(RtsNode4);
+    out->horizon_bytes = sc->d_horizon.cap * sizeof(float);
     out->handle_device_bytes = c->d_leaves.cap * sizeof(RtsLeafTri) + c->d_verts_world.cap * 8 + c->d_normals_world.cap * 8 + c->d_params.cap;
     return RTS_OK;
 }
diff --git a/rts_amd/csrc/rts_trace.hip b/rts_amd/csrc/rts_trace.hip
--- a/rts_amd/csrc/rts_trace.hip
+++ b/rts_amd/csrc/rts_trace.hip
@@ -284,6 +284,8 @@
 #define RTS_RXP_RW 15
 #define RTS_RXP_N 16
 struct RtsUnitLds { int32_t* stack; int32_t* exch; double* first; unsigned long long* path; uint32_t* n; const RtsRxDev* rx; const float (*rxp)[RTS_RXP_N]; uint32_t* lane_scratch; uint32_t* walk; };
+#define RTS_SKIP_SHIFT 23
+#define RTS_SHADED_MASK 0x007fffffu
 struct RtsRay { dvec3 dir, prev; double rayLength, power, doppler, refx, refy; uint32_t reflDepth, refrDepth; int received; bool end, chain_start; };
 
 template <bool KEEP_ALL, bool REFR, bool COOP, uint32_t CG = 64u>
@@ -461,6 +463,18 @@
             doppler += dot3(mk3(T.vx, T.vy, T.vz), sub3(k1, k0));
         }
         dir = widen3(nd);
+        if (!REFR) {
+            uint32_t skip = 0u;
+            if (a.horizon) {
+                const double dn = dir.x*L.nx + dir.y*L.ny + dir.z*L.nz, dl = sqrt(dir.x*dir.x + dir.y*dir.y + dir.z*dir.z), nl = sqrt(L.nx*L.nx + L.ny*L.ny + L.nz*L.nz);
+                const double c = fabs(dn) / (dl * nl), S = (double)(dn > 0.0 ? L.hz[0] : L.hz[1]);
+                const double ht = fabs((double)hit_t);
+                const double delta = ht * 0x1p-22 + (fmax(fmax(fabs(prev.x), fabs(prev.y)), fabs(prev.z)) + ht) * 0x1p-45;
+                const double reach = dl * (double)SCENE_EPS_R;
+                if ((c - delta / reach > S + (double)RTS_HZ_MARGIN) && (c * reach >= 2.0 * ((double)T.hz_h0 + delta)) && (4.0 * delta <= (double)T.hz_rho)) skip = L.targ + 1u;
+            }
+            atomicAnd(&s_n[RTS_BLOCK + tid], RTS_SHADED_MASK); if (skip) atomicOr(&s_n[RTS_BLOCK + tid], skip << RTS_SKIP_SHIFT);
+        }
         {
             const size_t plane = REFR ? (size_t)chain * (a.max_refl + 1) + reflDepth : (size_t)(reflDepth - 1);
             float* dh = a.dir_hist + plane * 3 * a.n_rays;
@@ -619,14 +633,14 @@
     dir = (may_target || may_rx) ? rts_primary_dir(lc, slot) : mk3(0.0, 0.0, 0.0);
     prev = origin;
     s_first[tid] = 0.0; s_first[RTS_BLOCK + tid] = 0.0; s_first[2 * RTS_BLOCK + tid] = 0.0;
-    s_path[tid] = 0ULL; s_path[RTS_BLOCK + tid] = 0ULL;
+    s_path[tid] = 0ULL; s_path[RTS_BLOCK + tid] = 0ULL; atomicAnd(&L_.n[RTS_BLOCK + tid], RTS_SHADED_MASK);
     rayLength = 0; power = 0; doppler = 0;
 }
 
 template <bool COUNT, bool KEEP_ALL, bool REFR, bool COOP, bool VERS = false>
 __device__ __forceinline__ void rts_trace_unit(const RtsTraceArgs& a, const RtsLaunchConsts& lc, const RtsUnitLds& L_, const uint32_t tid, const uint32_t gtid, const uint32_t lane,
                                                const uint32_t slot, const bool pre_on, const bool mask_on, const uint32_t D, const uint32_t max_refr, const dvec3& origin,
-                                               uint32_t& n_nodes, uint32_t& n_tris, bool& hard_overflow, unsigned long long (&lane_stats)[5],
+                                               uint32_t& n_nodes, uint32_t& n_tris, bool& hard_overflow, unsigned long long (&lane_stats)[11],
                                                const uint32_t pre = 0u)
 {
       int32_t* const s_stack = L_.stack; int32_t* const s_exch = L_.exch; double* const s_first = L_.first; unsigned long long* const s_path = L_.path; uint32_t* const s_n = L_.n;
@@ -669,11 +683,13 @@
             const bool primary = chain == 0 && chain_start;
             const bool may_hit = primary ? may_target : a.n_prims > 0;
             uint32_t steps = 0;
+            bool escaped = false;
             if (may_hit) {
                 float t_prune = RTS_DEFAULT_TMAX;
                 for (uint32_t targ = 0; targ < a.n_targets; targ++) {
                     const RtsTargetDev& TG = a.targets[targ];
                     if (TG.root < 0) continue;
+                    if (!REFR && (s_n[RTS_BLOCK + tid] >> RTS_SKIP_SHIFT) == targ + 1u) { if (COUNT) escaped = true; continue; }
                     {
                         const dvec3 q = mk3(TG.cx - prev.x, TG.cy - prev.y, TG.cz - prev.z);
                         const double qq = q.x*q.x + q.y*q.y + q.z*q.z, b = q.x*dir.x + q.y*dir.y + q.z*dir.z;
@@ -720,6 +736,15 @@
                 lane_stats[3] += (unsigned long long)__popcll(__ballot(steps > 0u));
                 lane_stats[4] += (unsigned long long)__popcll(__ballot(steps == 0u)) * smax;
             }
+            if (COUNT && escaped && (!COOP || (lane & (CG - 1u)) == 0u)) lane_stats[5] += 1ull;
+            if (COUNT && !COOP) {
+                const unsigned long long act_ = __ballot(true);
+                if (lane == (uint32_t)(__ffsll((long long)act_) - 1)) {
+                    const uint32_t smax_ = L_.lane_scratch[2u * (tid >> 6)];
+                    if (primary) { lane_stats[9] += smax_; lane_stats[10] += 1ull; }
+                    else { lane_stats[8] += 1ull; lane_stats[6] += smax_; if (smax_ == 0u) lane_stats[7] += 1ull; }
+                }
+            }
             if (COUNT && COOP && steps) lane_stats[3] += 1ull;
             {
                 const bool go_on_ = rts_shade<KEEP_ALL, REFR, COOP, CG>(a, L_, tid, gtid, lane, slot, chain, D, max_refr, origin, primary, may_rx, best_t, best_leaf, best_prim, tmin, S, pending, refr_code0);
@@ -795,7 +820,7 @@
     __shared__ uint32_t s_lane_scratch[COUNT ? 2 * (RTS_BLOCK / 64) : 1];
     __shared__ uint32_t s_walk[2 * (RTS_BLOCK / 64)];
     const RtsUnitLds ul = {s_stack, s_exch, s_first, s_path, s_n, s_rx, s_rxp, s_lane_scratch, s_walk};
-    unsigned long long lane_stats[5] = {0ull, 0ull, 0ull, 0ull, 0ull};
+    unsigned long long lane_stats[11] = {0ull, 0ull, 0ull, 0ull, 0ull, 0ull, 0ull, 0ull, 0ull, 0ull, 0ull};
 #define RTS_OPAQUE_S(x) ({ uint32_t o_ = (x); asm volatile("" : "+s"(o_)); o_; })
     uint32_t coop_x = 0, coop_sweep = 0, coop_len = 0;
     const uint32_t coop_P = COOP ? a.coop_spread : 1u, coop_G = RTS_XCD / coop_P;
@@ -931,8 +956,11 @@
     if (COUNT && !COOP && lane == 0 && lane_stats[0]) { atomicAdd(&a.counters[8], lane_stats[0]); atomicAdd(&a.counters[9], lane_stats[1]); atomicAdd(&a.counters[10], lane_stats[2]); }
     if (COUNT && (lane & (CG - 1u)) == 0u && lane_stats[3]) atomicAdd(&a.counters[11], lane_stats[3]);
     if (COUNT && !COOP && lane == 0 && lane_stats[4]) atomicAdd(&a.counters[15], lane_stats[4]);
+    if (COUNT && lane_stats[5]) atomicAdd(&a.counters[16], lane_stats[5]);
+    if (COUNT && !COOP && lane_stats[8]) { atomicAdd(&a.counters[17], lane_stats[6]); atomicAdd(&a.counters[18], lane_stats[7]); atomicAdd(&a.counters[19], lane_stats[8]); }
+    if (COUNT && !COOP && lane_stats[10]) { atomicAdd(&a.counters[20], lane_stats[9]); atomicAdd(&a.counters[21], lane_stats[10]); }
     const uint32_t tid_e = (wave_u << 6) | __builtin_amdgcn_mbcnt_hi(~0u, __builtin_amdgcn_mbcnt_lo(~0u, 0u));
-    unsigned long long n_seg = s_n[tid_e] & 0x003fffffu, n_shaded = s_n[RTS_BLOCK + tid_e], n_spill = s_n[2 * RTS_BLOCK + tid_e], n_nodes_w = n_nodes, n_tris_w = n_tris;
+    unsigned long long n_seg = s_n[tid_e] & 0x003fffffu, n_shaded = s_n[RTS_BLOCK + tid_e] & RTS_SHADED_MASK, n_spill = s_n[2 * RTS_BLOCK + tid_e], n_nodes_w = n_nodes, n_tris_w = n_tris;
     for (int off = 32; off > 0; off >>= 1) {
         n_seg += __shfl_down(n_seg, off); n_shaded += __shfl_down(n_shaded, off);
         if (COUNT) { n_nodes_w += __shfl_down(n_nodes_w, off); n_tris_w += __shfl_down(n_tris_w, off); }
@@ -962,7 +990,7 @@
 #define RTS_LD64(p) __hip_atomic_load((p), __ATOMIC_RELAXED, __HIP_MEMORY_SCOPE_AGENT)
     if (t == 7) { const unsigned long long h = head_count ? (unsigned long long)__hip_atomic_load(head_count, __ATOMIC_RELAXED, __HIP_MEMORY_SCOPE_AGENT) : 0ULL; counters[7] = h; host_cnt[7] = h; }
     if (t == 0) host_cnt[0] = RTS_LD64(&counters[0]);
-    if ((t >= 8 && t <= 12) || t == 14 || t == 15) host_cnt[t] = RTS_LD64(&counters[t]);
+    if ((t >= 8 && t <= 12) || (t >= 14 && t <= 21)) host_cnt[t] = RTS_LD64(&counters[t]);
     const unsigned int k = t & 7u, lane = t >> 3;
     unsigned long long v = 0;
     unsigned long long poisoned = 0;
```

After: 27010, median of 6. 9.2% higher.
